# albertgassol1/vf-nerf

Hardware: AMD Instinct MI355X
Metric: rays/sec (4096-ray chunk, 128 samples/ray) + PSNR vs ref (higher is better)
Workload: dtype f16x3+f32acc

## Files before the change

### vf_nerf_amd/csrc/vfn_common.h

```cpp
#pragma once
#include <hip/hip_runtime.h>
#include <stdarg.h>
#include <stdio.h>
#include "../../include/vfn.h"

void vfn_set_error(const char* fmt, ...);

#define VFN_REQUIRE(cond, ...)                 \
    do {                                       \
        if (!(cond)) {                         \
            vfn_set_error(__VA_ARGS__);        \
            return VFN_ERR_INVALID;            \
        }                                      \
    } while (0)

static inline int vfn_check_launch(const char* what) {
    hipError_t e = hipGetLastError();
    if (e != hipSuccess) {
        vfn_set_error("%s: HIP launch failed: %s", what, hipGetErrorString(e));
        return VFN_ERR_LAUNCH;
    }
    return VFN_OK;
}

__device__ __forceinline__ double vfn_pair_sqdist(double qx, double qy, double qz, double tx, double ty, double tz) {
    const double dx = qx - tx, dy = qy - ty, dz = qz - tz;
    return (dx * dx + dy * dy) + dz * dz;
}

int vfn_internal_raygen(const vfn_raygen_params* p, const float* uv, const float* pose, const float* intrinsics, const float* k_sign,
                        const float* t_vals, const float* far_per_ray, const float* u_coarse, int gen_u, long long u_base, uint64_t seed,
                        uint64_t offset, float* directions, float* ray_dirs, float* cam_loc, float* z_vals, float* points, void* stream);
int vfn_internal_density_fine(const vfn_density_params* dp, const float* normals_c, const float* ray_dirs, const float* z_c,
                              const float* density_scalars, const vfn_fine_params* fp, const float* directions, const float* cam_loc,
                              const float* far_per_ray, const float* u_fine, const float* u_add, int gen_fine, int gen_add,
                              long long fine_base, long long add_base, uint64_t seed, uint64_t offset, float* z_vals, float* points,
                              int32_t* src, float* new_points, int32_t* dst, int64_t new_row0, void* stream);
int vfn_internal_composite_gather(const vfn_density_params* dp, float* normals, const float* ray_dirs, const float* z_vals,
                                  const float* density_scalars, float* colors, const int32_t* src, const float* normals_c,
                                  const float* colors_c, int64_t n_stored_c, float* weights, float* rgb, float* depth, void* stream);

int vfn_internal_weight_grad_frag_batch(int32_t shape, int32_t dy_form, int32_t x_form, int32_t n, const void* const* dy, const void* const* x,
                                        float* const* dw_part, float* const* db_part, int64_t n_points, int32_t groups, void* stream);
int vfn_internal_weight_grad_frag_batch_dev(int32_t shape, int32_t dy_form, int32_t x_form, int32_t n, const void* const* dy, const void* const* x,
                                            float* const* dw_part, float* const* db_part, int64_t n_points, const int32_t* n_dev, int32_t groups,
                                            void* stream);

int vfn_internal_fused16_fwd_train_at(const vfn_net_geom* vf_geom, const void* vf_packed16, const vfn_net_geom* rn_geom,
                                      const void* rn_packed16, const float* points, const float* ray_dirs, int64_t n_points,
                                      const int32_t* n_dev, int32_t samples_per_ray, float* normals, float* colors, float* saved,
                                      float* save_aux_vf, float* save_aux_rn, uint32_t* save_masks, int32_t save_f16, int64_t ws_first,
                                      int64_t ws_points, int32_t colour_products, void* stream);
int vfn_internal_bwd_chain_bf16_ws_at(const vfn_net_geom* vf_geom, const void* vf_packed_bwd16, const float* vf_head_w,
                                      const vfn_net_geom* rn_geom, const void* rn_packed_bwd16, const float* rn_head_w,
                                      const float* feats, const uint32_t* masks, void* dy, int32_t dy_flags, const float* d_colors,
                                      const float* colors, const float* d_vec, const float* vec, const float* d_feats,
                                      int32_t vec_stride, int64_t n_points, const int32_t* n_dev, float* dz_rgb, float* dz_vec,
                                      int64_t ws_first, int64_t ws_points, void* stream);
int vfn_internal_net_weight_grads_frag_part(int32_t net_kind, const vfn_net_geom* geom, const vfn_wgrad_layer* layers, const void* saved,
                                            const void* dy, int64_t slot_bytes, int32_t dy_form, int32_t x_form, const float* feats,
                                            const float* aux, const float* dz_head, int64_t n_points, const int32_t* n_dev, uint32_t parts,
                                            int32_t accumulate, void* scratch, void* stream, int32_t stages = 3);

int vfn_internal_select_positive(const float* weights, const float* sigma, const float* z_vals, int n_rays, int n_samples, const float* points,
                                 const float* ray_dirs, int32_t* cnt, int32_t* off, int32_t* k_dev, int32_t* sel_sorted, float* pts_sel,
                                 float* dirs_sel, void* stream);
int vfn_internal_rows3_by_index(const float* a, const int32_t* index, const int32_t* k_dev, int64_t capacity, float* out, int gather, void* stream);
int vfn_internal_fused16_products_dev(const vfn_net_geom* vf_geom, const void* vf_packed16, const vfn_net_geom* rn_geom, const void* rn_packed16,
                                      const float* points, const float* ray_dirs, int64_t n_points, const int32_t* n_dev, int32_t samples_per_ray,
                                      const int32_t* out_index, int32_t colour_products, float* normals, float* colors, void* stream);
uint32_t* vfn_internal_f16x3_status();
struct VfnReportScope {
    VfnReportScope(uint32_t* status_word, uint64_t* clock_stamps, int64_t clock_slots);
    ~VfnReportScope();
    VfnReportScope(const VfnReportScope&) = delete;
    VfnReportScope& operator=(const VfnReportScope&) = delete;
    uint32_t* old_status; unsigned long long* old_clock; long long old_slots;
};
```

### vf_nerf_amd/csrc/vfn_mlp16.hip

```cpp
#include <string.h>
#include <utility>
#include "vfn_common.h"
#include "vfn_plan.h"

typedef _Float16 half8 __attribute__((ext_vector_type(8)));
typedef _Float16 half2v __attribute__((ext_vector_type(2)));
typedef float float2v __attribute__((ext_vector_type(2)));
typedef float f32x16 __attribute__((ext_vector_type(16)));
typedef float f32x4v __attribute__((ext_vector_type(4)));

constexpr float VFN16_WSCALE = 64.0f;
constexpr float VFN16_INV_WSCALE = 0.015625f;
constexpr float VFN16_XSCALE = 64.0f;
constexpr int VFN16_SAVE_AUX = 2;
constexpr int VFN16_HANDOVER_NUM = 8;
constexpr int VFN16_DMA_STEPS = 16;
constexpr int VFN16_EPI_PER_MFMA = 6;
constexpr int VFN16_EPI_PER_MFMA2 = 9;
#define VFN16_MAX_CHUNK_KB 39
#define VFN16_STATS_WORDS 64

struct Plan16 {
    int32_t n_hidden;
    int32_t feat_layer;
    int32_t multires;
    uint32_t total_kb;
    uint32_t head_off_kb;
    uint32_t off_kb[VFN_MAX_LAYERS];
    uint8_t act16[VFN_MAX_LAYERS];
    uint8_t aux16[VFN_MAX_LAYERS];
    uint8_t n_tiles[VFN_MAX_LAYERS];
};

static int make_plan16(int kind, const vfn_net_geom* g, VfnNetPlan* p32, Plan16* p, const char* what) {
    char err[256] = {0};
    int rc = vfn_make_plan(kind, g, p32, err, sizeof(err));
    if (rc != VFN_OK) { vfn_set_error("%s: %s", what, err); return rc; }
    memset(p, 0, sizeof(*p));
    p->n_hidden = p32->n_hidden; p->feat_layer = p32->feat_layer; p->multires = p32->multires;
    uint32_t off = 0;
    for (int h = 0; h < p32->n_hidden; ++h) {
        const VfnLayerPlan& lp = p32->hidden[h];
        if (lp.nkb_act % 2) { vfn_set_error("%s: act width not a multiple of 16", what); return VFN_ERR_UNSUPPORTED; }
        p->act16[h] = (uint8_t)(lp.nkb_act / 2);
        p->aux16[h] = lp.nkb_aux ? 3 : 0;
        p->n_tiles[h] = (uint8_t)lp.n_tiles;
        p->off_kb[h] = off;
        off += lp.n_tiles * (2u * (p->act16[h] + p->aux16[h]) + 1u);
    }
    p->head_off_kb = off;
    off += 2u * 16u + 1u;
    p->total_kb = off;
    return VFN_OK;
}

struct Pack16Entry {
    const float* w; const float* b; const float* bn_w; const float* bn_b; const float* bn_mean; const float* bn_var;
    uint32_t off_kb, n_chunks, act16, aux16;
    int32_t in_dim, row_off, n_rows, act_col_off, act_valid, aux_col_off, aux_valid;
    float scale;
};
struct Pack16Args {
    Pack16Entry e[VFN_MAX_LAYERS + 2];
    int32_t n_entries;
    uint32_t total_words;
    uint32_t* out;
    uint32_t* stats;
};

__device__ __forceinline__ float folded_weight(const Pack16Entry& e, int n, int col) {
    if (n >= e.n_rows || col < 0) return 0.f;
    const int row = e.row_off + n;
    float w = e.w[(size_t)row * e.in_dim + col];
    if (e.bn_w) w *= e.bn_w[row] / sqrtf(e.bn_var[row] + 1e-5f);
    return w * e.scale;
}

#define VFN16_STAT_WGS 32
__device__ __forceinline__ void pack16_entry_stats(const Pack16Args& a, int ei, int share) {
    __shared__ float s_max[4];
    const Pack16Entry& e = a.e[ei];
    const int ncol = e.act_valid + e.aux_valid;
    float m = 0.f;
    for (int n = share; n < e.n_rows; n += VFN16_STAT_WGS)
        for (int c = (int)threadIdx.x; c < ncol; c += (int)blockDim.x)
            m = fmaxf(m, fabsf(folded_weight(e, n, c < e.act_valid ? e.act_col_off + c : e.aux_col_off + (c - e.act_valid))));
#pragma unroll
    for (int o = 32; o > 0; o >>= 1) m = fmaxf(m, __shfl_xor(m, o, 64));
    if ((threadIdx.x & 63) == 0) s_max[threadIdx.x >> 6] = m;
    __syncthreads();
    if (threadIdx.x == 0) {
        const float wm = fmaxf(fmaxf(s_max[0], s_max[1]), fmaxf(s_max[2], s_max[3]));
        if (wm > 0.f) atomicMax(a.stats + ei, __builtin_bit_cast(uint32_t, wm));
    }
}

__global__ __launch_bounds__(256) void vfn_pack16_kernel(Pack16Args a) {
    if (blockIdx.x * blockDim.x >= a.total_words) {
        const int sidx = (int)(blockIdx.x - a.total_words / blockDim.x);
        if (a.stats) pack16_entry_stats(a, sidx / VFN16_STAT_WGS, sidx % VFN16_STAT_WGS);
        return;
    }
    const uint32_t idx = blockIdx.x * blockDim.x + threadIdx.x;
    int ei = 0;
    for (int i = 1; i < a.n_entries; ++i)
        if (idx >= a.e[i].off_kb * 256u) ei = i;
    const Pack16Entry& e = a.e[ei];
    const uint32_t nkb = e.act16 + e.aux16;
    const uint32_t wblocks = nkb * 2u;
    const uint32_t chunk_words = (wblocks + 1u) * 256u;
    const uint32_t local = idx - e.off_kb * 256u;
    const uint32_t ck = local / chunk_words, cw = local % chunk_words;
    uint32_t word = 0;
    if (cw < wblocks * 256u) {
        const uint32_t blk = cw >> 8, lane = (cw >> 2) & 63u, jp = cw & 3u;
        const uint32_t part = blk & 1u, kb = blk >> 1;
        const int g = (int)(lane >> 5);
        const int n = (int)(32u * ck + (lane & 31u));
        _Float16 halves[2];
        for (int q = 0; q < 2; ++q) {
            const int j = (int)(2u * jp) + q;
            int col = -1;
            if (kb < e.act16) {
                const int k = 16 * (int)kb + 8 * (j >> 2) + 4 * g + (j & 3);
                if (k < e.act_valid) col = e.act_col_off + k;
            } else {
                const int k = 16 * (int)(kb - e.act16) + 8 * g + j;
                if (k < e.aux_valid) col = e.aux_col_off + k;
            }
            const float w = folded_weight(e, n, col);
            const _Float16 hi = (_Float16)w;
            halves[q] = part ? (_Float16)(w - (float)hi) : hi;
        }
        word = (uint32_t)__builtin_bit_cast(unsigned short, halves[0]) |
               ((uint32_t)__builtin_bit_cast(unsigned short, halves[1]) << 16);
    } else {
        const uint32_t bi = cw - wblocks * 256u;
        if (bi < 32u) {
            const int hl = (int)(bi >> 4), r = (int)(bi & 15u);
            const int n = (int)(32u * ck) + (r & 3) + 8 * (r >> 2) + 4 * hl;
            float b = 0.f;
            if (n < e.n_rows) {
                const int row = e.row_off + n;
                b = e.b[row];
                if (e.bn_w) b = (b - e.bn_mean[row]) * (e.bn_w[row] / sqrtf(e.bn_var[row] + 1e-5f)) + e.bn_b[row];
            }
            word = __builtin_bit_cast(uint32_t, b * VFN16_WSCALE);
        }
    }
    a.out[idx] = word;
}

static int check_kind16(int net_kind, const Plan16& p, const char* what);

extern "C" int64_t vfn_pack16_size(int32_t net_kind, const vfn_net_geom* geom) {
    VfnNetPlan p32; Plan16 p;
    int rc = make_plan16(net_kind, geom, &p32, &p, "vfn_pack16_size");
    if (rc != VFN_OK) return rc;
    rc = check_kind16(net_kind, p, "vfn_pack16_size");
    if (rc != VFN_OK) return rc;
    return (int64_t)p.total_kb * 1024 + VFN16_STATS_WORDS * 4;
}

extern "C" int vfn_pack16_weights(int32_t net_kind, const vfn_net_geom* geom, const vfn_layer_params* layers,
                                   void* packed16, void* stream) {
    VfnNetPlan p32; Plan16 p;
    int rc = make_plan16(net_kind, geom, &p32, &p, "vfn_pack16_weights");
    if (rc != VFN_OK) return rc;
    rc = check_kind16(net_kind, p, "vfn_pack16_weights");
    if (rc != VFN_OK) return rc;
    VFN_REQUIRE(layers && packed16, "vfn_pack16_weights: NULL argument");
    Pack16Args a;
    memset(&a, 0, sizeof(a));
    const int L = geom->n_layers, pe_dim = p32.pe_dim, F = geom->feature_dims;
    auto fill = [&](Pack16Entry& e, int i) -> int {
        const vfn_layer_params& q = layers[i];
        VFN_REQUIRE(q.weight && q.bias, "vfn_pack16_weights: layer %d has NULL weight/bias", i);
        e.w = q.weight; e.b = q.bias;
        if (geom->has_bn[i]) {
            VFN_REQUIRE(q.bn_weight && q.bn_bias && q.bn_mean && q.bn_var, "vfn_pack16_weights: layer %d BatchNorm pointer NULL", i);
            e.bn_w = q.bn_weight; e.bn_b = q.bn_bias; e.bn_mean = q.bn_mean; e.bn_var = q.bn_var;
        }
        e.in_dim = geom->in_dims[i]; e.scale = 1.0f;
        return VFN_OK;
    };
    for (int h = 0; h < p.n_hidden; ++h) {
        const int i = p32.hidden[h].ref_layer;
        Pack16Entry& e = a.e[a.n_entries++];
        rc = fill(e, i);
        if (rc != VFN_OK) return rc;
        e.off_kb = p.off_kb[h]; e.n_chunks = p.n_tiles[h]; e.act16 = p.act16[h]; e.aux16 = p.aux16[h];
        const bool feat = p.feat_layer && h == p.n_hidden - 1;
        e.row_off = feat ? 3 : 0;
        e.n_rows = feat ? F : geom->out_dims[i];
        if (net_kind == VFN_NET_VF) {
            if (i == 0) { e.act_valid = 0; e.aux_col_off = 0; e.aux_valid = pe_dim; }
            else if (i == geom->skip_layer) {
                e.act_col_off = 0; e.act_valid = geom->out_dims[i - 1];
                e.aux_col_off = geom->out_dims[i - 1]; e.aux_valid = pe_dim;
                e.scale = 0.70710678118654752440f;
            } else { e.act_col_off = 0; e.act_valid = VFN_HIDDEN; }
        } else {
            if (i == 0) { e.act_col_off = 6 + pe_dim; e.act_valid = F; e.aux_col_off = 0; e.aux_valid = 6 + pe_dim; }
            else { e.act_col_off = 0; e.act_valid = VFN_HIDDEN; }
        }
    }
    {
        Pack16Entry& e = a.e[a.n_entries++];
        rc = fill(e, L - 1);
        if (rc != VFN_OK) return rc;
        e.off_kb = p.head_off_kb; e.n_chunks = 1; e.act16 = 16; e.aux16 = 0;
        e.row_off = 0; e.n_rows = 3; e.act_col_off = 0; e.act_valid = VFN_HIDDEN;
    }
    a.total_words = p.total_kb * 256u;
    a.out = (uint32_t*)packed16;
    a.stats = a.out + a.total_words;
    if (hipMemsetAsync(a.stats, 0, VFN16_STATS_WORDS * 4, (hipStream_t)stream) != hipSuccess) {
        vfn_set_error("vfn_pack16_weights: hipMemsetAsync failed");
        return VFN_ERR_LAUNCH;
    }
    hipLaunchKernelGGL(vfn_pack16_kernel, dim3(a.total_words / 256 + VFN16_STAT_WGS * a.n_entries), dim3(256), 0, (hipStream_t)stream, a);
    return vfn_check_launch("vfn_pack16_weights");
}

namespace {

enum : int { EPI_RELU = 0, EPI_TANH = 1, EPI_HEAD_TANH = 2, EPI_HEAD_SIGMOID = 3 };
enum : int { M16_FEAT = 1, M16_RENDER = 2, M16_TRAIN = 4, M16_BLKOUT = 8, M16_BLKIN = 16, M16_C2 = 32, M16_P1 = 64, M16_SF16 = 128,
             M16_VF_VEC = 0, M16_FUSED = M16_FEAT | M16_RENDER, M16_VF_BLK = M16_FEAT | M16_BLKOUT, M16_RN_BLK = M16_RENDER | M16_BLKIN,
             M16_VF_VEC_TRAIN = M16_TRAIN, M16_VF_FULL_TRAIN = M16_FEAT | M16_TRAIN, M16_FUSED_TRAIN = M16_FUSED | M16_TRAIN };

constexpr int VFN16_FDEPTH = 2;
#define VFN16_SLOT (VFN16_MAX_CHUNK_KB * 64)
#define VFN16_WAVES 4
#define VFN16_PTS 128

typedef __attribute__((address_space(3))) void lds_void;

constexpr int VF_ACT[9] = {0, 16, 16, 16, 14, 16, 16, 16, 16};
constexpr int VF_AUX[9] = {3, 0, 0, 0, 3, 0, 0, 0, 0};
constexpr int VF_TILES[9] = {8, 8, 8, 7, 8, 8, 8, 8, 8};
constexpr int RN_ACT[4] = {16, 16, 16, 16};
constexpr int RN_AUX[4] = {3, 0, 0, 0};
constexpr int RN_TILES[4] = {8, 8, 8, 8};
constexpr int HEAD_KB = 2 * 16 + 1;
constexpr int chunk_kb(int act, int aux) { return 2 * (act + aux) + 1; }
constexpr int vf_off_kb(int h) { int o = 0; for (int i = 0; i < h; ++i) o += VF_TILES[i] * chunk_kb(VF_ACT[i], VF_AUX[i]); return o; }
constexpr int rn_off_kb(int h) { int o = 0; for (int i = 0; i < h; ++i) o += RN_TILES[i] * chunk_kb(RN_ACT[i], RN_AUX[i]); return o; }

struct ChunkD { int net, off_kb, kb, aux; };
constexpr ChunkD chunk_of(int mode, int c) {
    if (!(mode & M16_BLKIN)) {
        const int vf_layers = (mode & M16_FEAT) ? 9 : 8;
        for (int h = 0; h < vf_layers; ++h) {
            if (c < VF_TILES[h]) return {0, vf_off_kb(h) + c * chunk_kb(VF_ACT[h], VF_AUX[h]), chunk_kb(VF_ACT[h], VF_AUX[h]), VF_AUX[h]};
            c -= VF_TILES[h];
        }
        if (c == 0) return {0, vf_off_kb(9), HEAD_KB, 0};
        c -= 1;
    }
    if (mode & M16_RENDER) {
        for (int h = 0; h < 4; ++h) {
            if (c < RN_TILES[h]) return {1, rn_off_kb(h) + c * chunk_kb(RN_ACT[h], RN_AUX[h]), chunk_kb(RN_ACT[h], RN_AUX[h]), RN_AUX[h]};
            c -= RN_TILES[h];
        }
        if (c == 0) return {1, rn_off_kb(4), HEAD_KB, 0};
    }
    return {0, 0, 0, 0};
}

constexpr int rn_first_chunk(int mode) { return (mode & M16_BLKIN) ? 0 : 72; }
constexpr bool chunk_two(int mode, int c) { return (mode & M16_C2) && !(mode & M16_BLKIN) && c >= 63 && c != 71; }
constexpr bool mode_one(int mode) { return (mode & M16_P1) != 0; }
constexpr int VFN16_P1_RING = 5;
#define VFN16_P1_SLOT_KB 20
constexpr int ring_of(int mode) { return mode_one(mode) ? VFN16_P1_RING : 3; }
constexpr int slot_u4(int mode) { return mode_one(mode) ? VFN16_P1_SLOT_KB * 64 : VFN16_MAX_CHUNK_KB * 64; }
constexpr int slot_base(int mode, int c) { return (c % ring_of(mode)) * slot_u4(mode); }
static_assert(VFN16_P1_RING * VFN16_P1_SLOT_KB <= 3 * VFN16_MAX_CHUNK_KB, "the single-product ring must fit into the split modes' ring");
constexpr int stores_of(int mode, int c) { return (c == 0 || ((mode & M16_RENDER) && c == rn_first_chunk(mode))) ? 0 : 4; }
constexpr int young_ops(int mode, int c) {
    const int ring = ring_of(mode);
    int n = 0;
    for (int k = (c - ring + 2 > 0 ? c - ring + 2 : 0); k < c; ++k) n += stores_of(mode, k);
    for (int j = 2; j <= ring - 2; ++j)
        if (c + j >= ring - 1 && chunk_of(mode, c + j).kb > 0) n += (((chunk_of(mode, c + j).kb - 1) / 2 + 1) / VFN16_WAVES);
    return n;
}

struct Mlp16Args {
    const uint4* vf_w;
    const uint4* rn_w;
    const float* points;
    const float* ray_dirs;
    float* out_vec;
    float* out_colors;
    long long n_points;
    int dirs_div;
    int vf_multires, rn_multires;
    uint32_t vf_bytes, rn_bytes;
    float* saved;
    float* save_aux_vf;
    float* save_aux_rn;
    uint32_t* save_masks;
    int save_f16;
    uint4* blk_out;
    const uint4* blk_in;
    const float* vec_in;
    const int* src;
    const int* out_index;
    long long ws_first, ws_points;
    uint32_t* status;
    const int* n_dev;
    unsigned long long* clock;
    long long clock_slots;
};

#define VFN16_CLAMP 60000.0f
constexpr int VFN16_CLAMP_BITS = 0x476a6000;
static_assert(__builtin_bit_cast(int, VFN16_CLAMP) == VFN16_CLAMP_BITS, "VFN16_CLAMP_BITS is VFN16_CLAMP as an integer");

struct X16 { half8 hi[16]; half8 lo[16]; };
struct A16 { half8 hi[3]; half8 lo[3]; };

struct Pipe16 {
    uint4* lds;
    __amdgpu_buffer_rsrc_t vf_w;
    __amdgpu_buffer_rsrc_t rn_w;
    float* saved;
    long long slot_floats;
    uint32_t slot_bytes;
    uint32_t save_voff;
    uint32_t save_voff16;
    uint32_t feat_voff;
    uint32_t st_tile, st_q;
    int save16;
    uint32_t* masks;
    uint32_t mask_bytes;
    uint32_t mask_voff;
    uint4* blk_out;
    uint32_t blk_bytes, blk_voff;
};

struct Carry16 {
    f32x16 pend;
    f32x16 bias;
    half8 fh0, fl0;
    uint32_t lm[4];
    unsigned long long sat;
};

template <int N, typename F, int... I>
__device__ __forceinline__ void static_for_impl(F&& f, std::integer_sequence<int, I...>) { (f(std::integral_constant<int, I>{}), ...); }
template <int N, typename F>
__device__ __forceinline__ void static_for(F&& f) { static_for_impl<N>(f, std::make_integer_sequence<int, N>{}); }

__device__ __forceinline__ void split2(float a, float b, _Float16& h0, _Float16& h1, _Float16& l0, _Float16& l1) {
    const float2v v = {a, b};
    const half2v hi = __builtin_convertvector(v, half2v);
    h0 = hi[0]; h1 = hi[1];
    const uint32_t hp = __builtin_bit_cast(uint32_t, hi);
    float r0, r1;
    asm("v_fma_mix_f32 %0, %1, -1.0, %2 op_sel_hi:[1,0,0]" : "=v"(r0) : "v"(hp), "v"(a));
    asm("v_fma_mix_f32 %0, %1, -1.0, %2 op_sel:[1,0,0] op_sel_hi:[1,0,0]" : "=v"(r1) : "v"(hp), "v"(b));
    const float2v r = {r0, r1};
    const half2v lo = __builtin_convertvector(r, half2v);
    l0 = lo[0]; l1 = lo[1];
}

__device__ __forceinline__ float tanh_exp(float v) { return 1.0f - 2.0f / (1.0f + expf(2.0f * v)); }

template <int NET, int OFF_KB, int LDS_U4>
__device__ __forceinline__ void dma_piece(const Pipe16& p, int blk, int lane, int dst_blk = -1) {
    __builtin_amdgcn_raw_ptr_buffer_load_lds(NET ? p.rn_w : p.vf_w, (lds_void*)(p.lds + LDS_U4 + (dst_blk < 0 ? blk : dst_blk) * 64), 16,
                                             lane * 16, (OFF_KB + blk) * 1024, 0, 0);
}
template <int MODE, int C>
__device__ __forceinline__ void dma_chunk(const Pipe16& p, int wave, int lane) {
    constexpr ChunkD d = chunk_of(MODE, C);
    if constexpr (mode_one(MODE)) {
        constexpr int NKB = (d.kb - 1) / 2;
#pragma unroll
        for (int i = 0; i * VFN16_WAVES < NKB + 1; ++i)
            if (wave + VFN16_WAVES * i < NKB + 1) dma_piece<d.net, d.off_kb, slot_base(MODE, C)>(p, 2 * (wave + VFN16_WAVES * i), lane, wave + VFN16_WAVES * i);
    } else {
#pragma unroll
    for (int i = 0; i * VFN16_WAVES < d.kb; ++i)
        if (wave + VFN16_WAVES * i < d.kb) dma_piece<d.net, d.off_kb, slot_base(MODE, C)>(p, wave + VFN16_WAVES * i, lane);
    }
}

template <int MODE, int C>
__device__ __forceinline__ void prefetch_chunk(Carry16& cy, const Pipe16& p, int lane) {
    constexpr ChunkD d = chunk_of(MODE, C);
    const uint4* cb = p.lds + slot_base(MODE, C);
    const f32x4v* bb = reinterpret_cast<const f32x4v*>(cb + (mode_one(MODE) ? (d.kb - 1) / 2 : d.kb - 1) * 64) + (lane >> 5) * 4;
    const f32x4v b0 = bb[0], b1 = bb[1], b2 = bb[2], b3 = bb[3];
#pragma unroll
    for (int q = 0; q < 4; ++q) { cy.bias[q] = b0[q]; cy.bias[4 + q] = b1[q]; cy.bias[8 + q] = b2[q]; cy.bias[12 + q] = b3[q]; }
    cy.fh0 = __builtin_bit_cast(half8, cb[0 * 64 + lane]);
    if (!chunk_two(MODE, C) && !mode_one(MODE)) cy.fl0 = __builtin_bit_cast(half8, cb[1 * 64 + lane]);
}

template <int EPI, bool KEEP, bool LO = true>
__device__ __forceinline__ void epi_pair(f32x16& pend, int& gmax, int pr, half8& hi, half8& lo, int j) {
    float v0 = pend[2 * pr], v1 = pend[2 * pr + 1];
    if (EPI != EPI_RELU) { v0 *= VFN16_INV_WSCALE; v1 *= VFN16_INV_WSCALE; }
    if (EPI == EPI_RELU) {
        const int b0 = __builtin_bit_cast(int, v0), b1 = __builtin_bit_cast(int, v1);
        gmax = pr == 0 ? max(b0, b1) : max(max(gmax, b0), b1);
        v0 = __builtin_amdgcn_fmed3f(v0, 0.f, VFN16_CLAMP); v1 = __builtin_amdgcn_fmed3f(v1, 0.f, VFN16_CLAMP);
    }
    else { v0 = tanh_exp(v0) * VFN16_XSCALE; v1 = tanh_exp(v1) * VFN16_XSCALE; }
    if constexpr (LO) {
        _Float16 h0, h1, l0, l1;
        split2(v0, v1, h0, h1, l0, l1);
        hi[j] = h0; hi[j + 1] = h1; lo[j] = l0; lo[j + 1] = l1;
    } else {
        const float2v v = {v0, v1};
        const half2v h = __builtin_convertvector(v, half2v);
        hi[j] = h[0]; hi[j + 1] = h[1];
    }
    if (KEEP) { pend[2 * pr] = v0 * (1.0f / VFN16_XSCALE); pend[2 * pr + 1] = v1 * (1.0f / VFN16_XSCALE); }
}

template <int SLOT, int TILE, bool SF16 = false>
__device__ __forceinline__ void save_group(const Pipe16& p, const f32x16& v, int q) {
    typedef unsigned int u32x4 __attribute__((ext_vector_type(4)));
    const __amdgpu_buffer_rsrc_t rs = __builtin_amdgcn_make_buffer_rsrc(p.saved + (long long)SLOT * p.slot_floats, 0,
                                                                        (int)p.slot_bytes, 0x00020000);
    const f32x4v g = {v[4 * q], v[4 * q + 1], v[4 * q + 2], v[4 * q + 3]};
    if constexpr (SF16 && SLOT != 8) {
        typedef _Float16 half4 __attribute__((ext_vector_type(4)));
        typedef unsigned int u32x2 __attribute__((ext_vector_type(2)));
        const half4 h = __builtin_convertvector(g, half4);
        __builtin_amdgcn_raw_buffer_store_b64(__builtin_bit_cast(u32x2, h), rs, (int)p.save_voff16, (TILE * 4096 + q * 1024) / 2, VFN16_SAVE_AUX);
        return;
    }
    if (SLOT == 8) {
        __builtin_amdgcn_raw_buffer_store_b128(__builtin_bit_cast(u32x4, g), rs, (int)p.feat_voff, (32 * TILE + 8 * q) * 4, 0);
    } else if (p.save16) {
        typedef _Float16 half4 __attribute__((ext_vector_type(4)));
        typedef unsigned int u32x2 __attribute__((ext_vector_type(2)));
        const half4 h = __builtin_convertvector(g, half4);
        if (p.st_q == 1024u) __builtin_amdgcn_raw_buffer_store_b64(__builtin_bit_cast(u32x2, h), rs, (int)p.save_voff16, (int)((TILE * p.st_tile + q * p.st_q) >> 1), VFN16_SAVE_AUX);
        else __builtin_amdgcn_raw_buffer_store_b64(__builtin_bit_cast(u32x2, h), rs, (int)p.save_voff16, (int)((TILE * p.st_tile + q * p.st_q) >> 1), 0);
    } else {
        if (p.st_q == 1024u) __builtin_amdgcn_raw_buffer_store_b128(__builtin_bit_cast(u32x4, g), rs, (int)p.save_voff, (int)(TILE * p.st_tile + q * p.st_q), VFN16_SAVE_AUX);
        else __builtin_amdgcn_raw_buffer_store_b128(__builtin_bit_cast(u32x4, g), rs, (int)p.save_voff, (int)(TILE * p.st_tile + q * p.st_q), 0);
    }
}

template <int TILE, int EPI>
__device__ __forceinline__ void collect_mask(Carry16& cy) {
    if constexpr (EPI == EPI_RELU) {
        typedef unsigned int u32x16 __attribute__((ext_vector_type(16)));
        const u32x16 u = __builtin_bit_cast(u32x16, cy.pend);
        unsigned b = 0;
#pragma unroll
        for (int r = 15; r >= 0; --r) b = __builtin_amdgcn_alignbit(b, u[r] + 0x7fffffffu, 31);
        cy.lm[TILE >> 1] |= b << (16 * (TILE & 1));
    }
}
template <int TILE, int EPI, int PART, int PARTS>
__device__ __forceinline__ void collect_mask_part(Carry16& cy, unsigned& b) {
    if constexpr (EPI == EPI_RELU) {
        typedef unsigned int u32x16 __attribute__((ext_vector_type(16)));
        const u32x16 u = __builtin_bit_cast(u32x16, cy.pend);
        constexpr int N = 16 / PARTS;
        if constexpr (PART == 0) b = 0;
#pragma unroll
        for (int r = 15 - PART * N; r > 15 - (PART + 1) * N; --r) b = __builtin_amdgcn_alignbit(b, u[r] + 0x7fffffffu, 31);
        if constexpr (PART == PARTS - 1) cy.lm[TILE >> 1] |= b << (16 * (TILE & 1));
    }
}
template <int SLOT>
__device__ __forceinline__ void store_mask(const Pipe16& p, Carry16& cy) {
    typedef unsigned int u32x4 __attribute__((ext_vector_type(4)));
    const __amdgpu_buffer_rsrc_t rs = __builtin_amdgcn_make_buffer_rsrc(
        reinterpret_cast<unsigned char*>(p.masks) + (size_t)SLOT * p.mask_bytes, 0, (int)p.mask_bytes, 0x00020000);
    const u32x4 w = {cy.lm[0], cy.lm[1], cy.lm[2], cy.lm[3]};
    __builtin_amdgcn_raw_buffer_store_b128(w, rs, (int)p.mask_voff, 0, 0);
    cy.lm[0] = 0; cy.lm[1] = 0; cy.lm[2] = 0; cy.lm[3] = 0;
}

template <int TILE>
__device__ __forceinline__ void store_blocks(const Pipe16& p, const X16& x) {
    typedef unsigned int u32x4 __attribute__((ext_vector_type(4)));
    const __amdgpu_buffer_rsrc_t rs = __builtin_amdgcn_make_buffer_rsrc(p.blk_out, 0, (int)p.blk_bytes, 0x00020000);
#pragma unroll
    for (int s = 0; s < 2; ++s) {
        __builtin_amdgcn_raw_buffer_store_b128(__builtin_bit_cast(u32x4, x.hi[2 * TILE + s]), rs, (int)p.blk_voff, (2 * TILE + s) * 2048, 0);
        __builtin_amdgcn_raw_buffer_store_b128(__builtin_bit_cast(u32x4, x.lo[2 * TILE + s]), rs, (int)p.blk_voff, (2 * TILE + s) * 2048 + 1024, 0);
    }
}

template <int MODE, int C0, int ACT, int AUX, int NCH, int EPI, int PEPI, int PKB, int SLOT = -1, int PSLOT = -1, bool BLK = false,
          bool PBLK = false>
__device__ __forceinline__ void layer16(const X16& xin, const A16& aux, X16& xout, X16& xpend, Carry16& cy, float (&head)[3],
                                       const Pipe16& p, int wave, int lane) {
    constexpr int NKB = ACT + AUX;
    constexpr int E = NKB / 2 > 0 ? NKB / 2 : 1;
    constexpr int H = NKB * VFN16_HANDOVER_NUM / 16 > 0 ? NKB * VFN16_HANDOVER_NUM / 16 : 1;
    constexpr int PMAX = (VFN16_MAX_CHUNK_KB + VFN16_WAVES - 1) / VFN16_WAVES;
    constexpr int DSPAN = NKB - H > 0 ? NKB - H : 1;
    constexpr int DSTEPS = DSPAN < VFN16_DMA_STEPS ? DSPAN : VFN16_DMA_STEPS;
    static_assert(PEPI < 0 || PKB >= E, "the pending tile must be complete before it is read");
    constexpr bool TRAIN = (MODE & M16_TRAIN) != 0;
    constexpr int DEND = NKB - 4 > H + 1 ? NKB - 4 : (H + 1 < NKB ? H + 1 : NKB - 1);
    constexpr int SSTEPS = NKB - DEND > 0 ? NKB - DEND : 1;
    constexpr int DST = TRAIN ? (DEND - H > 0 ? DEND - H : 1) : DSTEPS;
    constexpr int MPARTS = (TRAIN && E <= H) ? (DEND - H >= 4 ? 4 : (DEND - H >= 2 ? 2 : (DEND - H >= 1 ? 1 : 0))) : 0;
    static_for<NCH>([&](auto ich) {
        constexpr int ch = decltype(ich)::value;
        constexpr int C = C0 + ch;
        constexpr int RING = ring_of(MODE);
        constexpr ChunkD dcur = chunk_of(MODE, C), dnext = chunk_of(MODE, C + 1), ddma = chunk_of(MODE, C + RING - 1);
        static_assert(dcur.kb == 2 * NKB + 1, "layer shape and chunk table disagree");
        constexpr bool P1 = mode_one(MODE);
        constexpr bool W2 = chunk_two(MODE, C);
        constexpr bool D2 = chunk_two(MODE, C + RING - 1) || P1;
        constexpr int DNKB = (ddma.kb - 1) / 2;
        constexpr int DPIECES = P1 ? DNKB + 1 : (D2 ? DNKB + ddma.aux + 1 : ddma.kb);
        auto piece_blk = [&](int idx) -> int {
            if (P1) return idx < DNKB ? 2 * idx : 2 * DNKB;
            if (!D2) return idx;
            if (ddma.aux == 0) return 2 * idx;
            return idx < DNKB ? 2 * idx : (idx < DNKB + ddma.aux ? 2 * (idx - ddma.aux) + 1 : 2 * DNKB);
        };
        constexpr int PM = D2 ? (DPIECES + VFN16_WAVES - 1) / VFN16_WAVES : PMAX;
        const uint4* cb = p.lds + slot_base(MODE, C);
        constexpr int FB = P1 ? 1 : 2;
        f32x16 acc = cy.bias;
        half8 fh[VFN16_FDEPTH], fl[VFN16_FDEPTH];
        fh[0] = cy.fh0;
        if (!P1 && (!W2 || ACT == 0)) fl[0] = cy.fl0;
        half8 ehi[2], elo[2];
        [[maybe_unused]] int gmax = 0;
        [[maybe_unused]] unsigned mbits = 0;
#pragma unroll
        for (int st = 0; st < NKB; ++st) {
            constexpr int AHEAD = VFN16_FDEPTH - 1;
            if (st + AHEAD < NKB) {
                fh[(st + AHEAD) % VFN16_FDEPTH] = __builtin_bit_cast(half8, cb[(FB * (st + AHEAD)) * 64 + lane]);
                if (!P1 && (!W2 || st + AHEAD >= ACT)) fl[(st + AHEAD) % VFN16_FDEPTH] = __builtin_bit_cast(half8, cb[(2 * (st + AHEAD) + 1) * 64 + lane]);
            }
            const half8 a_hi = fh[st % VFN16_FDEPTH];
            const half8 x_hi = st < ACT ? xin.hi[st < ACT ? st : 0] : aux.hi[st >= ACT ? st - ACT : 0];
            const half8 x_lo = st < ACT ? xin.lo[st < ACT ? st : 0] : aux.lo[st >= ACT ? st - ACT : 0];
            acc = __builtin_amdgcn_mfma_f32_32x32x16_f16(a_hi, x_hi, acc, 0, 0, 0);
            if constexpr (!P1) {
                acc = __builtin_amdgcn_mfma_f32_32x32x16_f16(a_hi, x_lo, acc, 0, 0, 0);
                if (!W2 || st >= ACT) acc = __builtin_amdgcn_mfma_f32_32x32x16_f16(fl[st % VFN16_FDEPTH], x_hi, acc, 0, 0, 0);
            }
            if (st < E && (ch > 0 || PEPI >= 0)) {
#pragma unroll
                for (int pr = st * 8 / E; pr < (st + 1) * 8 / E; ++pr) {
                    const int sblk = pr >> 2, j = (pr & 3) * 2;
                    if (ch > 0) epi_pair<EPI, TRAIN, !P1>(cy.pend, gmax, pr, ehi[sblk], elo[sblk], j);
                    else epi_pair<(PEPI >= 0 ? PEPI : 0), TRAIN, !P1>(cy.pend, gmax, pr, ehi[sblk], elo[sblk], j);
                    if (pr == 7 && (ch > 0 ? EPI : PEPI) == EPI_RELU) cy.sat |= __builtin_amdgcn_ballot_w64(gmax >= VFN16_CLAMP_BITS);
                    if ((pr & 3) == 3) {
                        asm volatile("" : "+a"(ehi[sblk]));
                        if constexpr (!P1) asm volatile("" : "+a"(elo[sblk]));
                        if (ch > 0) { xout.hi[2 * (ch > 0 ? ch - 1 : 0) + sblk] = ehi[sblk]; if constexpr (!P1) xout.lo[2 * (ch > 0 ? ch - 1 : 0) + sblk] = elo[sblk]; }
                        else { xpend.hi[PKB + sblk] = ehi[sblk]; if constexpr (!P1) xpend.lo[PKB + sblk] = elo[sblk]; }
                    }
                }
                if constexpr (!P1) {
                __builtin_amdgcn_sched_group_barrier(0x100, W2 ? 1 : 2, 0);
                __builtin_amdgcn_sched_group_barrier(0x008, 1, 0);
                __builtin_amdgcn_sched_group_barrier(0x002, W2 ? VFN16_EPI_PER_MFMA2 : VFN16_EPI_PER_MFMA, 0);
                __builtin_amdgcn_sched_group_barrier(0x008, 1, 0);
                __builtin_amdgcn_sched_group_barrier(0x002, W2 ? VFN16_EPI_PER_MFMA2 : VFN16_EPI_PER_MFMA, 0);
                if (!W2) {
                    __builtin_amdgcn_sched_group_barrier(0x008, 1, 0);
                    __builtin_amdgcn_sched_group_barrier(0x002, VFN16_EPI_PER_MFMA, 0);
                }
                }
            }
            if (st == H - 1 && dnext.kb > 0) {
                if constexpr (P1 && TRAIN) {
                    constexpr int young = young_ops(MODE, C);
                    static_assert(young < 64, "vmcnt is a 6-bit field");
                    if constexpr (young == 0) asm volatile("s_waitcnt vmcnt(0)" ::: "memory");
                    else asm volatile("s_waitcnt vmcnt(%0)" :: "n"(young) : "memory");
                } else
                if (TRAIN && C > 0 && (ch == 0 || ch > 1 || PEPI >= 0)) asm volatile("s_waitcnt vmcnt(4)" ::: "memory");
                else asm volatile("s_waitcnt vmcnt(0)" ::: "memory");
                __builtin_amdgcn_s_barrier();
            }
            if (st >= H && st < H + DST && ddma.kb > 0) {
#pragma unroll
                for (int i = (st - H) * PM / DST; i < (st - H + 1) * PM / DST; ++i) {
                    if (VFN16_WAVES * i + VFN16_WAVES <= DPIECES) dma_piece<ddma.net, ddma.off_kb, slot_base(MODE, C + RING - 1)>(p, piece_blk(wave + VFN16_WAVES * i), lane, P1 ? wave + VFN16_WAVES * i : -1);
                    else if (VFN16_WAVES * i < DPIECES) {
                        const int idx = min(wave + VFN16_WAVES * i, DPIECES - 1);
                        dma_piece<ddma.net, ddma.off_kb, slot_base(MODE, C + RING - 1)>(p, piece_blk(idx), lane, P1 ? idx : -1);
                    }
                }
            }
            if (TRAIN && MPARTS > 0 && st >= H && st < H + MPARTS && (ch > 0 || PEPI >= 0)) {
                static_for<MPARTS>([&](auto ip) {
                    constexpr int part = decltype(ip)::value;
                    if (st - H == part) {
                        if (ch > 0) collect_mask_part<(ch > 0 ? ch - 1 : 0), EPI, part, (MPARTS > 0 ? MPARTS : 1)>(cy, mbits);
                        else collect_mask_part<PKB / 2, (PEPI >= 0 ? PEPI : 0), part, (MPARTS > 0 ? MPARTS : 1)>(cy, mbits);
                    }
                });
            }
            if (TRAIN && st >= DEND && st < DEND + SSTEPS && (ch > 0 || PEPI >= 0)) {
                if (st == DEND) {
                    if constexpr (MPARTS > 0) {
                        if (ch == 0) store_mask<(PSLOT >= 0 ? PSLOT : 0)>(p, cy);
                    } else {
                        if (ch > 0) collect_mask<(ch > 0 ? ch - 1 : 0), EPI>(cy);
                        else { collect_mask<PKB / 2, (PEPI >= 0 ? PEPI : 0)>(cy); store_mask<(PSLOT >= 0 ? PSLOT : 0)>(p, cy); }
                    }
                }
#pragma unroll
                for (int q = (st - DEND) * 4 / SSTEPS; q < (st - DEND + 1) * 4 / SSTEPS; ++q) {
                    if (ch > 0) save_group<(SLOT >= 0 ? SLOT : 0), (ch > 0 ? ch - 1 : 0), (MODE & M16_SF16) != 0>(p, cy.pend, q);
                    else save_group<(PSLOT >= 0 ? PSLOT : 0), PKB / 2, (MODE & M16_SF16) != 0>(p, cy.pend, q);
                }
            }
            if (st == H && ((BLK && ch > 0) || (PBLK && ch == 0))) {
                if (ch > 0) store_blocks<(ch > 0 ? ch - 1 : 0)>(p, xout);
                else store_blocks<PKB / 2>(p, xpend);
            }
            if (st == NKB - 1 && dnext.kb > 0) prefetch_chunk<MODE, (dnext.kb > 0 ? C + 1 : C)>(cy, p, lane);
            __builtin_amdgcn_sched_barrier(0);
        }
        if (EPI == EPI_RELU || EPI == EPI_TANH) {
            cy.pend = acc;
        } else {
#pragma unroll
            for (int c = 0; c < 3; ++c) {
                const float v = acc[c] * VFN16_INV_WSCALE;
                head[c] = (EPI == EPI_HEAD_TANH) ? tanh_exp(v) : 1.0f / (1.0f + expf(-v));
            }
        }
    });
}

__device__ __forceinline__ float enc_value(const float (&x)[3], const float (&sn)[18], const float (&cs)[18], int multires, int k) {
    if (k < 3) return x[k];
    const int idx = k - 3, oct = idx / 6, rem = idx - 6 * oct;
    if (oct >= multires) return 0.f;
    return rem < 3 ? sn[3 * oct + rem] : cs[3 * oct + rem - 3];
}

template <typename F>
__device__ __forceinline__ void build_aux(A16& aux, int g, F col, float& ain) {
#pragma unroll
    for (int s = 0; s < 3; ++s) {
        half8 hi, lo;
#pragma unroll
        for (int j = 0; j < 8; j += 2) {
            float v0, v1;
            if (g == 0) { v0 = col(16 * s + j); v1 = col(16 * s + j + 1); }
            else { v0 = col(16 * s + 8 + j); v1 = col(16 * s + 8 + j + 1); }
            v0 *= VFN16_XSCALE; v1 *= VFN16_XSCALE;
            v0 = fminf(fmaxf(v0, -VFN16_CLAMP), VFN16_CLAMP); v1 = fminf(fmaxf(v1, -VFN16_CLAMP), VFN16_CLAMP);
            ain = fmaxf(ain, fmaxf(fabsf(v0), fabsf(v1)));
            _Float16 h0, h1, l0, l1;
            split2(v0, v1, h0, h1, l0, l1);
            hi[j] = h0; hi[j + 1] = h1; lo[j] = l0; lo[j + 1] = l1;
        }
        aux.hi[s] = hi; aux.lo[s] = lo;
    }
}

template <typename F>
__device__ __forceinline__ void save_aux(float* dst, long long m, int g, F col) {
#pragma unroll
    for (int s = 0; s < 3; ++s)
#pragma unroll
        for (int h = 0; h < 2; ++h) {
            const int c0 = 16 * s + 8 * g + 4 * h;
            if (c0 + 4 <= VFN_AUX_K) {
                f32x4v v;
                if (g == 0) { v = f32x4v{col(16 * s + 4 * h), col(16 * s + 4 * h + 1), col(16 * s + 4 * h + 2), col(16 * s + 4 * h + 3)}; }
                else { v = f32x4v{col(16 * s + 8 + 4 * h), col(16 * s + 8 + 4 * h + 1), col(16 * s + 8 + 4 * h + 2), col(16 * s + 8 + 4 * h + 3)}; }
                *reinterpret_cast<f32x4v*>(dst + m * VFN_AUX_K + c0) = v;
            }
        }
}

__device__ __forceinline__ void load_aux(A16& ax, const float* park) {
    const half8* pk = reinterpret_cast<const half8*>(park + 8);
#pragma unroll
    for (int q = 0; q < 3; ++q) { ax.hi[q] = pk[2 * q]; ax.lo[q] = pk[2 * q + 1]; }
}

__device__ __forceinline__ void encode_sincos(const float (&x)[3], int multires, int g, float (&sn)[18], float (&cs)[18]) {
#pragma unroll
    for (int j = 0; j < 3; ++j)
#pragma unroll
        for (int c = 0; c < 3; ++c) {
            float s = 0.f, k = 0.f;
            if (2 * j < multires) {
                sincosf(x[c] * (g ? (float)(2 << (2 * j)) : (float)(1 << (2 * j))), &s, &k);
                if (2 * j + g >= multires) { s = 0.f; k = 0.f; }
            }
            const float so = __shfl_xor(s, 32, 64), ko = __shfl_xor(k, 32, 64);
            sn[6 * j + c] = g ? so : s;          cs[6 * j + c] = g ? ko : k;
            sn[6 * j + 3 + c] = g ? s : so;      cs[6 * j + 3 + c] = g ? k : ko;
        }
}

template <int MODE>
__device__ __forceinline__ void render_aux(const Mlp16Args& a, A16& aux, const float (&xr)[3], const float (&dr)[3], const float (&nrm)[3],
                                           long long m, bool in, int g, float& ain) {
    const int rn_multires = a.rn_multires;
    float sn[18], cs[18];
    encode_sincos(dr, rn_multires, g, sn, cs);
    const int ncol = 6 + 6 * rn_multires;
    auto rn_col = [&](int k) -> float {
        if (k < 3) return xr[k];
        if (k >= ncol) return k < ncol + 3 ? nrm[k - ncol] : 0.f;
        return enc_value(dr, sn, cs, rn_multires, k - 3);
    };
    build_aux(aux, g, rn_col, ain);
    if ((MODE & M16_TRAIN) && in) save_aux(a.save_aux_rn, m, g, rn_col);
}

template <int MODE>
__device__ __forceinline__ void render_tail(const Mlp16Args& a, const Pipe16& p, Carry16& cy, X16& xa, X16& xb, const A16& aux,
                                            const float (&nrm)[3], long long m, bool in, int wave, int lane) {
    constexpr int R = EPI_RELU, NONE = -1;
    constexpr int C0 = rn_first_chunk(MODE);
    float rgb[3] = {0.f, 0.f, 0.f};
    layer16<MODE, C0 + 0, 16, 3, 8, R, NONE, 0, 9, -1>(xb, aux, xa, xb, cy, rgb, p, wave, lane);
    layer16<MODE, C0 + 8, 16, 0, 8, R, R, 14, 10, 9>(xa, aux, xb, xa, cy, rgb, p, wave, lane);
    layer16<MODE, C0 + 16, 16, 0, 8, R, R, 14, 11, 10>(xb, aux, xa, xb, cy, rgb, p, wave, lane);
    layer16<MODE, C0 + 24, 16, 0, 8, R, R, 14, 12, 11>(xa, aux, xb, xa, cy, rgb, p, wave, lane);
    layer16<MODE, C0 + 32, 16, 0, 1, EPI_HEAD_SIGMOID, R, 14, -1, 12>(xb, aux, xa, xb, cy, rgb, p, wave, lane);
    const long long mo = m;
    if (in && (threadIdx.x & 32) == 0) {
        a.out_vec[mo * 3 + 0] = nrm[0]; a.out_vec[mo * 3 + 1] = nrm[1]; a.out_vec[mo * 3 + 2] = nrm[2];
        a.out_colors[mo * 3 + 0] = rgb[0]; a.out_colors[mo * 3 + 1] = rgb[1]; a.out_colors[mo * 3 + 2] = rgb[2];
    }
}

__device__ __forceinline__ void report_range(const Mlp16Args& a, unsigned long long sat, float ain) {
    if (a.status) {
        const unsigned bits = (sat != 0ull ? 1u : 0u) | (ain >= VFN16_CLAMP ? 2u : 0u);
        if (bits) atomicOr(a.status, bits);
    }
}

template <int MODE>
__global__ __launch_bounds__(256, 1) void vfn_mlp16_kernel(const Mlp16Args a) {
    __shared__ __attribute__((aligned(16))) uint4 s_ring[3 * VFN16_SLOT + 256 * 8];
    float* s_park = reinterpret_cast<float*>(s_ring + 3 * VFN16_SLOT) + threadIdx.x * 32;
    const int tid = threadIdx.x;
    const int lane = tid & 63;
    const int wave = __builtin_amdgcn_readfirstlane(tid >> 6);
    const int g = lane >> 5;
    unsigned long long ck_t0 = 0ull, ck_r0 = 0ull;
    if constexpr ((MODE & M16_RENDER) != 0 && (MODE & M16_BLKIN) == 0 && (MODE & M16_TRAIN) == 0) {
        if (a.clock) { ck_t0 = __builtin_amdgcn_s_memtime(); ck_r0 = __builtin_amdgcn_s_memrealtime(); }
    }
    const long long m = (long long)blockIdx.x * VFN16_PTS + wave * 32 + (lane & 31);
    long long n_live = a.n_points;
    if (a.n_dev) {
        const long long nd = (long long)*a.n_dev;
        n_live = nd < n_live ? nd : n_live;
        if ((long long)blockIdx.x * VFN16_PTS >= n_live) return;
    }
    const bool in = m < n_live;

    if constexpr ((MODE & M16_BLKIN) != 0) {
        const int dpos = in ? a.src[m] : -1;
        const bool live = dpos >= 0;
        float xr[3] = {0.f, 0.f, 0.f}, dr[3] = {0.f, 0.f, 0.f}, nrm[3] = {0.f, 0.f, 0.f};
        if (live) {
            const long long di = dpos / a.dirs_div;
#pragma unroll
            for (int c = 0; c < 3; ++c) { xr[c] = a.points[(long long)dpos * 3 + c]; dr[c] = a.ray_dirs[di * 3 + c]; nrm[c] = a.vec_in[m * 3 + c]; }
        }
        Pipe16 p;
        p.lds = s_ring;
        p.vf_w = __builtin_amdgcn_make_buffer_rsrc(const_cast<uint4*>(a.rn_w), 0, (int)a.rn_bytes, 0x00020000);
        p.rn_w = p.vf_w;
        p.saved = nullptr; p.slot_floats = 0; p.slot_bytes = 0; p.save_voff = 0; p.blk_out = nullptr; p.blk_bytes = 0; p.blk_voff = 0;
        p.masks = nullptr; p.mask_bytes = 0; p.mask_voff = 0; p.save16 = 0; p.save_voff16 = 0; p.feat_voff = 0; p.st_tile = 0; p.st_q = 0;
        dma_chunk<MODE, 0>(p, wave, lane);
        dma_chunk<MODE, 1>(p, wave, lane);
        X16 xa, xb;
        A16 aux;
        float ain_blk = 0.f;
        {
            typedef unsigned int u32x4 __attribute__((ext_vector_type(4)));
            const __amdgpu_buffer_rsrc_t rs_blk = __builtin_amdgcn_make_buffer_rsrc(
                const_cast<uint4*>(a.blk_in), 0, (int)(((a.n_points + 31) & ~31ll) * 1024), 0x00020000);
            const unsigned goff = in ? (unsigned)((m >> 5) * 32768 + lane * 16) : 0xfffffff0u;
            u32x4 q[32];
#pragma unroll
            for (int i = 0; i < 32; ++i) q[i] = __builtin_amdgcn_raw_buffer_load_b128(rs_blk, goff, i * 1024, 0);
            render_aux<MODE>(a, aux, xr, dr, nrm, -1, false, g, ain_blk);
#pragma unroll
            for (int t = 0; t < 8; ++t) {
                half8 h0 = __builtin_bit_cast(half8, q[4 * t + 0]), l0 = __builtin_bit_cast(half8, q[4 * t + 1]);
                half8 h1 = __builtin_bit_cast(half8, q[4 * t + 2]), l1 = __builtin_bit_cast(half8, q[4 * t + 3]);
                asm volatile("" : "+a"(h0)); asm volatile("" : "+a"(l0)); asm volatile("" : "+a"(h1)); asm volatile("" : "+a"(l1));
                xb.hi[2 * t] = h0; xb.lo[2 * t] = l0; xb.hi[2 * t + 1] = h1; xb.lo[2 * t + 1] = l1;
            }
        }
        asm volatile("s_waitcnt vmcnt(0)" ::: "memory");
        __builtin_amdgcn_s_barrier();
        Carry16 cy;
#pragma unroll
        for (int q = 0; q < 16; ++q) cy.pend[q] = 0.f;
        cy.lm[0] = 0; cy.lm[1] = 0; cy.lm[2] = 0; cy.lm[3] = 0; cy.sat = 0ull;
        prefetch_chunk<MODE, 0>(cy, p, lane);
        render_tail<MODE>(a, p, cy, xa, xb, aux, nrm, live ? (long long)dpos : -1, live, wave, lane);
        report_range(a, cy.sat, ain_blk);
    } else {
    float x[3] = {0.f, 0.f, 0.f};
    if (in) { x[0] = a.points[m * 3 + 0]; x[1] = a.points[m * 3 + 1]; x[2] = a.points[m * 3 + 2]; }
    float d[3] = {0.f, 0.f, 0.f};
    int out_row = -1;
    if ((MODE & M16_RENDER) && in) {
        const long long di = m / a.dirs_div;
        d[0] = a.ray_dirs[di * 3 + 0]; d[1] = a.ray_dirs[di * 3 + 1]; d[2] = a.ray_dirs[di * 3 + 2];
        if (a.out_index) out_row = a.out_index[m];
    }
    asm volatile("s_waitcnt vmcnt(0)" ::: "memory");
    if (MODE & M16_RENDER) {
        s_park[0] = x[0]; s_park[1] = x[1]; s_park[2] = x[2];
        s_park[4] = d[0]; s_park[5] = d[1]; s_park[6] = d[2];
    }

    Pipe16 p;
    p.lds = s_ring;
    p.vf_w = __builtin_amdgcn_make_buffer_rsrc(const_cast<uint4*>(a.vf_w), 0, (int)a.vf_bytes, 0x00020000);
    p.rn_w = __builtin_amdgcn_make_buffer_rsrc(const_cast<uint4*>((MODE & M16_RENDER) ? a.rn_w : a.vf_w), 0,
                                               (int)((MODE & M16_RENDER) ? a.rn_bytes : a.vf_bytes), 0x00020000);
    const bool frag = (a.save_f16 & 2) != 0;
    const long long mw = m + a.ws_first;
    p.slot_floats = frag ? ((a.ws_points + 31) >> 5) * 8192 : a.ws_points * 256;
    p.saved = a.saved + a.ws_first * 256;
    {
        const long long left = p.slot_floats * 4 - a.ws_first * 1024;
        p.slot_bytes = (uint32_t)(left < 0x7fffffffll ? left : 0x7fffffffll);
    }
    p.save_voff = !in ? (frag ? 0xc0000000u : 0xfffffff0u) : (frag ? (uint32_t)((m >> 5) * 32768 + lane * 16) : (uint32_t)(m * 1024 + g * 16));
    p.save_voff16 = !in ? (frag ? 0xc0000000u : 0xfffffff0u) : (frag ? (uint32_t)((m >> 5) * 32768 + lane * 8) : (uint32_t)(m * 1024 + g * 8));
    p.feat_voff = in ? (uint32_t)(m * 1024 + g * 16) : 0xfffffff0u;
    p.st_tile = frag ? 4096u : 128u; p.st_q = frag ? 1024u : 32u;
    p.masks = a.save_masks; p.mask_bytes = (uint32_t)(a.ws_points * 32); p.mask_voff = in ? (uint32_t)((2 * mw + g) * 16) : 0xfffffff0u;
    p.save16 = a.save_f16 & 1;
    p.blk_out = a.blk_out; p.blk_bytes = (uint32_t)(((a.n_points + 31) & ~31ll) * 1024);
    p.blk_voff = (uint32_t)((m >> 5) * 32768 + lane * 16);
    dma_chunk<MODE, 0>(p, wave, lane);
    dma_chunk<MODE, 1>(p, wave, lane);
    if constexpr (mode_one(MODE)) static_for<VFN16_P1_RING - 3>([&](auto ic) { dma_chunk<MODE, 2 + decltype(ic)::value>(p, wave, lane); });

    const int vf_multires = a.vf_multires;
    A16 aux;
    float ain = 0.f;
    {
        float sn[18], cs[18];
        encode_sincos(x, vf_multires, g, sn, cs);
        build_aux(aux, g, [&](int k) { return enc_value(x, sn, cs, vf_multires, k); }, ain);
        if ((MODE & M16_TRAIN) && in) save_aux(a.save_aux_vf, mw, g, [&](int k) { return enc_value(x, sn, cs, vf_multires, k); });
        half8* pk = reinterpret_cast<half8*>(s_park + 8);
#pragma unroll
        for (int q = 0; q < 3; ++q) { pk[2 * q] = aux.hi[q]; pk[2 * q + 1] = aux.lo[q]; }
    }
    asm volatile("s_waitcnt vmcnt(0)" ::: "memory");
    __builtin_amdgcn_s_barrier();
    Carry16 cy;
#pragma unroll
    for (int q = 0; q < 16; ++q) cy.pend[q] = 0.f;
    cy.lm[0] = 0; cy.lm[1] = 0; cy.lm[2] = 0; cy.lm[3] = 0; cy.sat = 0ull;
    prefetch_chunk<MODE, 0>(cy, p, lane);

    X16 xa, xb;
    float vec[3] = {0.f, 0.f, 0.f};
    constexpr int R = EPI_RELU, T = EPI_TANH, NONE = -1;
    layer16<MODE, 0, 0, 3, 8, R, NONE, 0, 0, -1>(xa, aux, xb, xb, cy, vec, p, wave, lane);
    layer16<MODE, 8, 16, 0, 8, R, R, 14, 1, 0>(xb, aux, xa, xb, cy, vec, p, wave, lane);
    layer16<MODE, 16, 16, 0, 8, R, R, 14, 2, 1>(xa, aux, xb, xa, cy, vec, p, wave, lane);
    layer16<MODE, 24, 16, 0, 7, R, R, 14, 3, 2>(xb, aux, xa, xb, cy, vec, p, wave, lane);
    { A16 ax; load_aux(ax, s_park); layer16<MODE, 31, 14, 3, 8, R, R, 12, 4, 3>(xa, ax, xb, xa, cy, vec, p, wave, lane); }
    layer16<MODE, 39, 16, 0, 8, R, R, 14, 5, 4>(xb, aux, xa, xb, cy, vec, p, wave, lane);
    layer16<MODE, 47, 16, 0, 8, R, R, 14, 6, 5>(xa, aux, xb, xa, cy, vec, p, wave, lane);
    layer16<MODE, 55, 16, 0, 8, R, R, 14, 7, 6>(xb, aux, xa, xb, cy, vec, p, wave, lane);
    if constexpr (!(MODE & M16_FEAT)) {
        layer16<MODE, 63, 16, 0, 1, EPI_HEAD_TANH, R, 14, -1, 7>(xa, aux, xb, xa, cy, vec, p, wave, lane);
        if (in && g == 0) { a.out_vec[m * 3 + 0] = vec[0]; a.out_vec[m * 3 + 1] = vec[1]; a.out_vec[m * 3 + 2] = vec[2]; }
        report_range(a, cy.sat, ain);
    } else {
    constexpr bool BO = (MODE & M16_BLKOUT) != 0;
    layer16<MODE, 63, 16, 0, 8, T, R, 14, 8, 7, BO, false>(xa, aux, xb, xa, cy, vec, p, wave, lane);
    layer16<MODE, 71, 16, 0, 1, EPI_HEAD_TANH, T, 14, -1, 8, false, BO>(xa, aux, xb, xb, cy, vec, p, wave, lane);
    if constexpr (!(MODE & M16_RENDER)) {
        if (in && g == 0) { a.out_vec[m * 3 + 0] = vec[0]; a.out_vec[m * 3 + 1] = vec[1]; a.out_vec[m * 3 + 2] = vec[2]; }
        report_range(a, cy.sat, ain);
    } else {
    float nrm[3];
#pragma unroll
    for (int c = 0; c < 3; ++c) nrm[c] = __shfl(vec[c], lane & 31, 64);
    const float xr[3] = {s_park[0], s_park[1], s_park[2]};
    const float dr[3] = {s_park[4], s_park[5], s_park[6]};
    A16 raux;
    render_aux<MODE>(a, raux, xr, dr, nrm, (MODE & M16_TRAIN) ? mw : m, in, g, ain);
    render_tail<MODE>(a, p, cy, xa, xb, raux, nrm, a.out_index ? (long long)out_row : m, a.out_index ? out_row >= 0 : in, wave, lane);
    report_range(a, cy.sat, ain);
    if constexpr ((MODE & M16_TRAIN) == 0) {
        if (a.clock && threadIdx.x == 0 && (long long)blockIdx.x < a.clock_slots) {
            const unsigned long long t1 = __builtin_amdgcn_s_memtime(), r1 = __builtin_amdgcn_s_memrealtime();
            a.clock[2 * blockIdx.x] = t1 - ck_t0; a.clock[2 * blockIdx.x + 1] = r1 - ck_r0;
        }
    }
    }
    }
    }
}

int check_vf16(const Plan16& vf, const char* what) {
    bool ok = vf.feat_layer == 1 && vf.n_hidden == 9 && (int)vf.head_off_kb == vf_off_kb(9);
    for (int h = 0; ok && h < 9; ++h)
        ok = vf.act16[h] == VF_ACT[h] && vf.aux16[h] == VF_AUX[h] && vf.n_tiles[h] == VF_TILES[h] && (int)vf.off_kb[h] == vf_off_kb(h);
    if (!ok) { vfn_set_error("%s: the f16x3 kernels are specialised for the shipped vector-field network shape", what); return VFN_ERR_UNSUPPORTED; }
    return VFN_OK;
}
int check_rn16(const Plan16& rn, const char* what) {
    bool ok = rn.n_hidden == 4 && (int)rn.head_off_kb == rn_off_kb(4);
    for (int h = 0; ok && h < 4; ++h)
        ok = rn.act16[h] == RN_ACT[h] && rn.aux16[h] == RN_AUX[h] && rn.n_tiles[h] == RN_TILES[h] && (int)rn.off_kb[h] == rn_off_kb(h);
    if (!ok) { vfn_set_error("%s: the f16x3 kernels are specialised for the shipped rendering network shape", what); return VFN_ERR_UNSUPPORTED; }
    return VFN_OK;
}

}

static int check_kind16(int net_kind, const Plan16& p, const char* what) {
    return net_kind == VFN_NET_VF ? check_vf16(p, what) : check_rn16(p, what);
}

static thread_local uint32_t* t_status_word = nullptr;

uint32_t* vfn_internal_f16x3_status() { return t_status_word; }

extern "C" int vfn_f16x3_set_status(uint32_t* status_word) {
    t_status_word = status_word;
    return VFN_OK;
}

static thread_local unsigned long long* t_clock_probe = nullptr;
static thread_local long long t_clock_slots = 0;

extern "C" int vfn_f16x3_set_clock_probe(uint64_t* stamps, int64_t slots) {
    VFN_REQUIRE(slots >= 0 && (stamps || slots == 0), "vfn_f16x3_set_clock_probe: %lld slots without a buffer", (long long)slots);
    t_clock_probe = reinterpret_cast<unsigned long long*>(stamps);
    t_clock_slots = stamps ? slots : 0;
    return VFN_OK;
}

VfnReportScope::VfnReportScope(uint32_t* status_word, uint64_t* clock_stamps, int64_t clock_slots)
    : old_status(t_status_word), old_clock(t_clock_probe), old_slots(t_clock_slots) {
    if (status_word) t_status_word = status_word;
    if (clock_stamps && clock_slots > 0) { t_clock_probe = reinterpret_cast<unsigned long long*>(clock_stamps); t_clock_slots = clock_slots; }
}
VfnReportScope::~VfnReportScope() { t_status_word = old_status; t_clock_probe = old_clock; t_clock_slots = old_slots; }

extern "C" int vfn_vf_mlp16_fwd(const vfn_net_geom* geom, const void* packed16, const float* points, int64_t n_points,
                                 float* out_vec, void* stream) {
    Mlp16Args a = {};
    VfnNetPlan p32; Plan16 vf;
    int rc = make_plan16(VFN_NET_VF, geom, &p32, &vf, "vfn_vf_mlp16_fwd");
    if (rc != VFN_OK) return rc;
    rc = check_vf16(vf, "vfn_vf_mlp16_fwd");
    if (rc != VFN_OK) return rc;
    if (n_points <= 0) return VFN_OK;
    VFN_REQUIRE(packed16 && points && out_vec, "vfn_vf_mlp16_fwd: NULL argument");
    a.vf_w = (const uint4*)packed16; a.points = points; a.out_vec = out_vec; a.n_points = n_points; a.dirs_div = 1;
    a.vf_multires = vf.multires; a.vf_bytes = vf.total_kb * 1024u;
    a.status = t_status_word;
    a.clock = t_clock_probe; a.clock_slots = t_clock_slots;
    const long long blocks = (n_points + VFN16_PTS - 1) / VFN16_PTS;
    hipLaunchKernelGGL(vfn_mlp16_kernel<M16_VF_VEC>, dim3((unsigned)blocks), dim3(256), 0, (hipStream_t)stream, a);
    return vfn_check_launch("vfn_vf_mlp16_fwd");
}

static int launch_fused16(const char* what, const vfn_net_geom* vf_geom, const void* vf_packed16, const vfn_net_geom* rn_geom,
                          const void* rn_packed16, const float* points, const float* ray_dirs, int64_t n_points,
                          int32_t samples_per_ray, const int32_t* out_index, bool scatter, int32_t colour_products, float* normals,
                          float* colors, void* stream, const int32_t* n_dev = nullptr) {
    Mlp16Args a = {};
    a.n_dev = n_dev;
    VfnNetPlan p32; Plan16 vf, rn;
    VFN_REQUIRE(vf_geom && rn_geom, "%s: NULL argument", what);
    int rc = make_plan16(VFN_NET_VF, vf_geom, &p32, &vf, what);
    if (rc != VFN_OK) return rc;
    rc = make_plan16(VFN_NET_RENDER, rn_geom, &p32, &rn, what);
    if (rc != VFN_OK) return rc;
    rc = check_vf16(vf, what);
    if (rc != VFN_OK) return rc;
    rc = check_rn16(rn, what);
    if (rc != VFN_OK) return rc;
    VFN_REQUIRE(vf_geom->feature_dims == VFN_HIDDEN && rn_geom->feature_dims == VFN_HIDDEN, "%s: both nets need feature_dims == %d", what, VFN_HIDDEN);
    VFN_REQUIRE(colour_products == 2 || colour_products == 3, "%s: colour_products must be 2 or 3 (got %d)", what, colour_products);
    if (n_points <= 0) return VFN_OK;
    VFN_REQUIRE(vf_packed16 && rn_packed16 && points && ray_dirs && normals && colors && (out_index || !scatter), "%s: NULL argument", what);
    VFN_REQUIRE(samples_per_ray > 0, "%s: samples_per_ray must be > 0", what);
    a.vf_w = (const uint4*)vf_packed16; a.rn_w = (const uint4*)rn_packed16; a.points = points; a.ray_dirs = ray_dirs;
    a.out_vec = normals; a.out_colors = colors; a.out_index = out_index; a.n_points = n_points; a.dirs_div = samples_per_ray;
    a.vf_multires = vf.multires; a.rn_multires = rn.multires; a.vf_bytes = vf.total_kb * 1024u; a.rn_bytes = rn.total_kb * 1024u;
    a.status = t_status_word;
    a.clock = t_clock_probe; a.clock_slots = t_clock_slots;
    const long long blocks = (n_points + VFN16_PTS - 1) / VFN16_PTS;
    if (colour_products == 2) hipLaunchKernelGGL(vfn_mlp16_kernel<M16_FUSED | M16_C2>, dim3((unsigned)blocks), dim3(256), 0, (hipStream_t)stream, a);
    else hipLaunchKernelGGL(vfn_mlp16_kernel<M16_FUSED>, dim3((unsigned)blocks), dim3(256), 0, (hipStream_t)stream, a);
    return vfn_check_launch(what);
}

extern "C" int vfn_vf_render_fused16_fwd(const vfn_net_geom* vf_geom, const void* vf_packed16, const vfn_net_geom* rn_geom,
                                          const void* rn_packed16, const float* points, const float* ray_dirs,
                                          int64_t n_points, int32_t samples_per_ray, float* normals, float* colors,
                                          void* stream) {
    return launch_fused16("vfn_vf_render_fused16_fwd", vf_geom, vf_packed16, rn_geom, rn_packed16, points, ray_dirs, n_points, samples_per_ray,
                          nullptr, false, 3, normals, colors, stream);
}

extern "C" int vfn_vf_render_fused16_scatter(const vfn_net_geom* vf_geom, const void* vf_packed16, const vfn_net_geom* rn_geom,
                                          const void* rn_packed16, const float* points, const float* ray_dirs,
                                          int64_t n_points, int32_t samples_per_ray, const int32_t* out_index, float* normals,
                                          float* colors, void* stream) {
    return launch_fused16("vfn_vf_render_fused16_scatter", vf_geom, vf_packed16, rn_geom, rn_packed16, points, ray_dirs, n_points,
                          samples_per_ray, out_index, true, 3, normals, colors, stream);
}

extern "C" int vfn_vf_render_fused16_products(const vfn_net_geom* vf_geom, const void* vf_packed16, const vfn_net_geom* rn_geom,
                                              const void* rn_packed16, const float* points, const float* ray_dirs, int64_t n_points,
                                              int32_t samples_per_ray, const int32_t* out_index, int32_t colour_products,
                                              float* normals, float* colors, void* stream) {
    return launch_fused16("vfn_vf_render_fused16_products", vf_geom, vf_packed16, rn_geom, rn_packed16, points, ray_dirs, n_points,
                          samples_per_ray, out_index, false, colour_products, normals, colors, stream);
}

int vfn_internal_fused16_products_dev(const vfn_net_geom* vf_geom, const void* vf_packed16, const vfn_net_geom* rn_geom, const void* rn_packed16,
                                      const float* points, const float* ray_dirs, int64_t n_points, const int32_t* n_dev, int32_t samples_per_ray,
                                      const int32_t* out_index, int32_t colour_products, float* normals, float* colors, void* stream) {
    return launch_fused16("vfn_render_fwd (colour branch on the selected samples)", vf_geom, vf_packed16, rn_geom, rn_packed16, points, ray_dirs,
                          n_points, samples_per_ray, out_index, false, colour_products, normals, colors, stream, n_dev);
}

extern "C" int vfn_vf_feat16_fwd(const vfn_net_geom* geom, const void* packed16, const float* points, int64_t n_points,
                                 float* out_vec, void* out_blocks, void* stream) {
    Mlp16Args a = {};
    VfnNetPlan p32; Plan16 vf;
    int rc = make_plan16(VFN_NET_VF, geom, &p32, &vf, "vfn_vf_feat16_fwd");
    if (rc != VFN_OK) return rc;
    rc = check_vf16(vf, "vfn_vf_feat16_fwd");
    if (rc != VFN_OK) return rc;
    if (n_points <= 0) return VFN_OK;
    VFN_REQUIRE(packed16 && points && out_vec && out_blocks, "vfn_vf_feat16_fwd: NULL argument");
    VFN_REQUIRE(n_points < (1ll << 22), "vfn_vf_feat16_fwd: at most 4194303 points per launch (32-bit block offsets)");
    a.vf_w = (const uint4*)packed16; a.points = points; a.out_vec = out_vec; a.n_points = n_points; a.dirs_div = 1;
    a.vf_multires = vf.multires; a.vf_bytes = vf.total_kb * 1024u; a.blk_out = (uint4*)out_blocks;
    a.status = t_status_word;
    a.clock = t_clock_probe; a.clock_slots = t_clock_slots;
    const long long blocks = (n_points + VFN16_PTS - 1) / VFN16_PTS;
    hipLaunchKernelGGL(vfn_mlp16_kernel<M16_VF_BLK>, dim3((unsigned)blocks), dim3(256), 0, (hipStream_t)stream, a);
    return vfn_check_launch("vfn_vf_feat16_fwd");
}

extern "C" int vfn_render16_from_blocks(const vfn_net_geom* rn_geom, const void* rn_packed16, const void* blocks, const float* vecs,
                                        const int32_t* dst, const float* points, const float* ray_dirs, int64_t n_points,
                                        int32_t samples_per_ray, float* normals, float* colors, void* stream) {
    Mlp16Args a = {};
    VfnNetPlan p32; Plan16 rn;
    int rc = make_plan16(VFN_NET_RENDER, rn_geom, &p32, &rn, "vfn_render16_from_blocks");
    if (rc != VFN_OK) return rc;
    rc = check_rn16(rn, "vfn_render16_from_blocks");
    if (rc != VFN_OK) return rc;
    VFN_REQUIRE(rn_geom->feature_dims == VFN_HIDDEN, "vfn_render16_from_blocks: feature_dims must be %d", VFN_HIDDEN);
    if (n_points <= 0) return VFN_OK;
    VFN_REQUIRE(rn_packed16 && blocks && vecs && dst && points && ray_dirs && normals && colors, "vfn_render16_from_blocks: NULL argument");
    VFN_REQUIRE(samples_per_ray > 0, "vfn_render16_from_blocks: samples_per_ray must be > 0");
    a.rn_w = (const uint4*)rn_packed16; a.vf_w = a.rn_w; a.points = points; a.ray_dirs = ray_dirs; a.out_vec = normals; a.out_colors = colors;
    a.n_points = n_points; a.dirs_div = samples_per_ray; a.rn_multires = rn.multires; a.rn_bytes = rn.total_kb * 1024u; a.vf_bytes = a.rn_bytes;
    a.blk_in = (const uint4*)blocks; a.vec_in = vecs; a.src = dst;
    a.status = t_status_word;
    a.clock = t_clock_probe; a.clock_slots = t_clock_slots;
    const long long nblocks = (n_points + VFN16_PTS - 1) / VFN16_PTS;
    hipLaunchKernelGGL(vfn_mlp16_kernel<M16_RN_BLK>, dim3((unsigned)nblocks), dim3(256), 0, (hipStream_t)stream, a);
    return vfn_check_launch("vfn_render16_from_blocks");
}

extern "C" int vfn_vf_mlp16_fwd_train(const vfn_net_geom* geom, const void* packed16, const float* points, int64_t n_points,
                                      int32_t with_features, float* out_vec, float* saved, float* save_aux_vf, uint32_t* save_masks,
                                      int32_t save_f16, void* stream) {
    return vfn_vf_mlp16_fwd_train_at(geom, packed16, points, n_points, with_features, out_vec, saved, save_aux_vf, save_masks, save_f16, 0, n_points,
                                     stream);
}

extern "C" int vfn_vf_mlp16_fwd_train_at(const vfn_net_geom* geom, const void* packed16, const float* points, int64_t n_points,
                                         int32_t with_features, float* out_vec, float* saved, float* save_aux_vf, uint32_t* save_masks,
                                         int32_t save_f16, int64_t ws_first, int64_t ws_points, void* stream) {
    Mlp16Args a = {};
    VfnNetPlan p32; Plan16 vf;
    int rc = make_plan16(VFN_NET_VF, geom, &p32, &vf, "vfn_vf_mlp16_fwd_train");
    if (rc != VFN_OK) return rc;
    rc = check_vf16(vf, "vfn_vf_mlp16_fwd_train");
    if (rc != VFN_OK) return rc;
    if (n_points <= 0) return VFN_OK;
    VFN_REQUIRE(packed16 && points && out_vec && saved && save_aux_vf && save_masks, "vfn_vf_mlp16_fwd_train: NULL argument");
    VFN_REQUIRE(ws_first >= 0 && ws_first + n_points <= ws_points, "vfn_vf_mlp16_fwd_train: points %lld .. %lld outside a workspace of %lld",
                (long long)ws_first, (long long)(ws_first + n_points), (long long)ws_points);
    VFN_REQUIRE(!(save_f16 & 2) || ws_first % 32 == 0, "vfn_vf_mlp16_fwd_train: ws_first must be a multiple of 32 in fragment order");
    VFN_REQUIRE(n_points < (1ll << 21) && ws_points < (1ll << 26), "vfn_vf_mlp16_fwd_train: at most 2097151 points per launch (32-bit slot offsets) and 67108863 per "
                "workspace (got %lld in %lld)", (long long)n_points, (long long)ws_points);
    a.vf_w = (const uint4*)packed16; a.points = points; a.out_vec = out_vec; a.n_points = n_points; a.dirs_div = 1;
    a.vf_multires = vf.multires; a.vf_bytes = vf.total_kb * 1024u; a.saved = saved; a.save_aux_vf = save_aux_vf;
    a.save_masks = save_masks; a.save_f16 = save_f16 & 3;
    a.ws_first = ws_first; a.ws_points = ws_points;
    a.status = t_status_word;
    a.clock = t_clock_probe; a.clock_slots = t_clock_slots;
    const long long blocks = (n_points + VFN16_PTS - 1) / VFN16_PTS;
    if (save_f16 & 4) {
        VFN_REQUIRE(!with_features, "vfn_vf_mlp16_fwd_train: the single-product forward computes the vector columns only");
        hipLaunchKernelGGL(vfn_mlp16_kernel<M16_VF_VEC_TRAIN | M16_P1>, dim3((unsigned)blocks), dim3(256), 0, (hipStream_t)stream, a);
    }
    else if (with_features && (save_f16 & 3) == 3) hipLaunchKernelGGL(vfn_mlp16_kernel<M16_VF_FULL_TRAIN | M16_SF16>, dim3((unsigned)blocks), dim3(256), 0, (hipStream_t)stream, a);
    else if (with_features) hipLaunchKernelGGL(vfn_mlp16_kernel<M16_VF_FULL_TRAIN>, dim3((unsigned)blocks), dim3(256), 0, (hipStream_t)stream, a);
    else if ((save_f16 & 3) == 3) hipLaunchKernelGGL(vfn_mlp16_kernel<M16_VF_VEC_TRAIN | M16_SF16>, dim3((unsigned)blocks), dim3(256), 0, (hipStream_t)stream, a);
    else hipLaunchKernelGGL(vfn_mlp16_kernel<M16_VF_VEC_TRAIN>, dim3((unsigned)blocks), dim3(256), 0, (hipStream_t)stream, a);
    return vfn_check_launch("vfn_vf_mlp16_fwd_train");
}

extern "C" int vfn_vf_render_fused16_fwd_train(const vfn_net_geom* vf_geom, const void* vf_packed16, const vfn_net_geom* rn_geom,
                                               const void* rn_packed16, const float* points, const float* ray_dirs,
                                               int64_t n_points, int32_t samples_per_ray, float* normals, float* colors,
                                               float* saved, float* save_aux_vf, float* save_aux_rn, uint32_t* save_masks,
                                               int32_t save_f16, void* stream) {
    return vfn_vf_render_fused16_fwd_train_at(vf_geom, vf_packed16, rn_geom, rn_packed16, points, ray_dirs, n_points, samples_per_ray, normals, colors,
                                              saved, save_aux_vf, save_aux_rn, save_masks, save_f16, 0, n_points, 3, stream);
}

extern "C" int vfn_vf_render_fused16_fwd_train_at(const vfn_net_geom* vf_geom, const void* vf_packed16, const vfn_net_geom* rn_geom,
                                                  const void* rn_packed16, const float* points, const float* ray_dirs,
                                                  int64_t n_points, int32_t samples_per_ray, float* normals, float* colors,
                                                  float* saved, float* save_aux_vf, float* save_aux_rn, uint32_t* save_masks,
                                                  int32_t save_f16, int64_t ws_first, int64_t ws_points, int32_t colour_products,
                                                  void* stream) {
    return vfn_internal_fused16_fwd_train_at(vf_geom, vf_packed16, rn_geom, rn_packed16, points, ray_dirs, n_points, nullptr, samples_per_ray, normals,
                                             colors, saved, save_aux_vf, save_aux_rn, save_masks, save_f16, ws_first, ws_points, colour_products, stream);
}

int vfn_internal_fused16_fwd_train_at(const vfn_net_geom* vf_geom, const void* vf_packed16, const vfn_net_geom* rn_geom,
                                      const void* rn_packed16, const float* points, const float* ray_dirs, int64_t n_points,
                                      const int32_t* n_dev, int32_t samples_per_ray, float* normals, float* colors, float* saved,
                                      float* save_aux_vf, float* save_aux_rn, uint32_t* save_masks, int32_t save_f16, int64_t ws_first,
                                      int64_t ws_points, int32_t colour_products, void* stream) {
    Mlp16Args a = {};
    a.n_dev = n_dev;
    VfnNetPlan p32; Plan16 vf, rn;
    int rc = make_plan16(VFN_NET_VF, vf_geom, &p32, &vf, "vfn_vf_render_fused16_fwd_train");
    if (rc != VFN_OK) return rc;
    rc = make_plan16(VFN_NET_RENDER, rn_geom, &p32, &rn, "vfn_vf_render_fused16_fwd_train");
    if (rc != VFN_OK) return rc;
    rc = check_vf16(vf, "vfn_vf_render_fused16_fwd_train");
    if (rc != VFN_OK) return rc;
    rc = check_rn16(rn, "vfn_vf_render_fused16_fwd_train");
    if (rc != VFN_OK) return rc;
    if (n_points <= 0) return VFN_OK;
    VFN_REQUIRE(vf_packed16 && rn_packed16 && points && ray_dirs && normals && colors && saved && save_aux_vf && save_aux_rn && save_masks,
                "vfn_vf_render_fused16_fwd_train: NULL argument");
    VFN_REQUIRE(samples_per_ray > 0, "vfn_vf_render_fused16_fwd_train: samples_per_ray must be > 0");
    VFN_REQUIRE(ws_first >= 0 && ws_first + n_points <= ws_points, "vfn_vf_render_fused16_fwd_train: points %lld .. %lld outside a workspace of %lld",
                (long long)ws_first, (long long)(ws_first + n_points), (long long)ws_points);
    VFN_REQUIRE(!(save_f16 & 2) || ws_first % 32 == 0, "vfn_vf_render_fused16_fwd_train: ws_first must be a multiple of 32 in fragment order");
    VFN_REQUIRE(n_points < (1ll << 21) && ws_points < (1ll << 26), "vfn_vf_render_fused16_fwd_train: at most 2097151 points per launch (32-bit slot offsets) and 67108863 per "
                "workspace (got %lld in %lld)", (long long)n_points, (long long)ws_points);
    a.ws_first = ws_first; a.ws_points = ws_points;
    a.vf_w = (const uint4*)vf_packed16; a.rn_w = (const uint4*)rn_packed16; a.points = points; a.ray_dirs = ray_dirs;
    a.out_vec = normals; a.out_colors = colors; a.n_points = n_points; a.dirs_div = samples_per_ray;
    a.vf_multires = vf.multires; a.rn_multires = rn.multires; a.vf_bytes = vf.total_kb * 1024u; a.rn_bytes = rn.total_kb * 1024u;
    a.saved = saved; a.save_aux_vf = save_aux_vf; a.save_aux_rn = save_aux_rn; a.save_masks = save_masks; a.save_f16 = save_f16 & 3;
    a.status = t_status_word;
    a.clock = t_clock_probe; a.clock_slots = t_clock_slots;
    const long long blocks = (n_points + VFN16_PTS - 1) / VFN16_PTS;
    VFN_REQUIRE(colour_products >= 1 && colour_products <= 3, "vfn_vf_render_fused16_fwd_train: colour_products must be 1, 2 or 3 (got %d)", colour_products);
    if (colour_products == 1) hipLaunchKernelGGL(vfn_mlp16_kernel<M16_FUSED_TRAIN | M16_P1>, dim3((unsigned)blocks), dim3(256), 0, (hipStream_t)stream, a);
    else if (colour_products == 2) hipLaunchKernelGGL(vfn_mlp16_kernel<M16_FUSED_TRAIN | M16_C2>, dim3((unsigned)blocks), dim3(256), 0, (hipStream_t)stream, a);
    else if ((save_f16 & 3) == 3) hipLaunchKernelGGL(vfn_mlp16_kernel<M16_FUSED_TRAIN | M16_SF16>, dim3((unsigned)blocks), dim3(256), 0, (hipStream_t)stream, a);
    else hipLaunchKernelGGL(vfn_mlp16_kernel<M16_FUSED_TRAIN>, dim3((unsigned)blocks), dim3(256), 0, (hipStream_t)stream, a);
    return vfn_check_launch("vfn_vf_render_fused16_fwd_train");
}
```

### vf_nerf_amd/csrc/vfn_rays.hip

```cpp
#pragma clang fp contract(off)
#include <string.h>
#include "vfn_common.h"

namespace {

__device__ __forceinline__ bool argmax_takes(float ob, int oi, float best, int besti) {
    if (ob != ob) return best == best || oi < besti;
    return best == best && (ob > best || (ob == best && oi < besti));
}

constexpr int WAVE = 64;
constexpr int RAYS_PER_BLOCK = 4;
constexpr int MAX_SAMPLES = 512;

__device__ __forceinline__ float wave_sum(float v) {
#pragma unroll
    for (int o = 32; o > 0; o >>= 1) v += __shfl_xor(v, o, WAVE);
    return v;
}

__device__ __forceinline__ void philox_round(uint32_t (&c)[4], uint32_t (&k)[2]) {
    const uint64_t p0 = (uint64_t)0xD2511F53u * c[0];
    const uint64_t p1 = (uint64_t)0xCD9E8D57u * c[2];
    const uint32_t n0 = (uint32_t)(p1 >> 32) ^ c[1] ^ k[0];
    const uint32_t n1 = (uint32_t)p1;
    const uint32_t n2 = (uint32_t)(p0 >> 32) ^ c[3] ^ k[1];
    const uint32_t n3 = (uint32_t)p0;
    c[0] = n0; c[1] = n1; c[2] = n2; c[3] = n3;
    k[0] += 0x9E3779B9u; k[1] += 0xBB67AE85u;
}

struct PhiloxStream { unsigned long long seed, offset; };
__device__ __forceinline__ float philox_uniform(const PhiloxStream& ps, long long e) {
    const unsigned long long ctr = ps.offset + (unsigned long long)(e >> 2);
    uint32_t c[4] = {(uint32_t)ctr, (uint32_t)(ctr >> 32), 0u, 0u};
    uint32_t k[2] = {(uint32_t)ps.seed, (uint32_t)(ps.seed >> 32)};
#pragma unroll
    for (int r = 0; r < 10; ++r) philox_round(c, k);
    const int i = (int)(e & 3);
    const uint32_t v = i == 0 ? c[0] : (i == 1 ? c[1] : (i == 2 ? c[2] : c[3]));
    return (float)(v >> 8) * (1.0f / 16777216.0f);
}

constexpr int K1_RAYS = 16;

struct RaygenArgs {
    vfn_raygen_params p;
    const float* uv;
    const float* pose;
    const float* K;
    const float* t_vals;
    const float* far_per_ray;
    const float* u;
    float* directions;
    float* ray_dirs;
    float* cam_loc;
    float* z_vals;
    float* points;
    int gen_u;
    long long u_base;
    PhiloxStream ps;
    const float* k_sign;
};

__device__ __forceinline__ float coarse_z(float near, float far, float t) { return near * (1.0f - t) + far * t; }

__global__ __launch_bounds__(256) void vfn_raygen_kernel(const RaygenArgs a) {
    __shared__ float s_ray[K1_RAYS][8];
    const int tid = threadIdx.x;
    const int ray0 = blockIdx.x * K1_RAYS;
    const int n = a.p.n_rays;
    if (tid < K1_RAYS && ray0 + tid < n) {
        const int r = ray0 + tid;
        float P[3][4];
        if (a.p.pose_is_quat) {
            const float* q7 = a.pose + (size_t)r * 7;
            float q0 = q7[0], q1 = q7[1], q2 = q7[2], q3 = q7[3];
            const float nq = fmaxf(sqrtf(q0 * q0 + q1 * q1 + q2 * q2 + q3 * q3), 1e-12f);
            const float qr = q0 / nq, qi = q1 / nq, qj = q2 / nq, qk = q3 / nq;
            P[0][0] = 1 - 2 * (qj * qj + qk * qk); P[0][1] = 2 * (qj * qi - qk * qr); P[0][2] = 2 * (qi * qk + qr * qj);
            P[1][0] = 2 * (qj * qi + qk * qr); P[1][1] = 1 - 2 * (qi * qi + qk * qk); P[1][2] = 2 * (qj * qk - qi * qr);
            P[2][0] = 2 * (qk * qi - qj * qr); P[2][1] = 2 * (qj * qk + qi * qr); P[2][2] = 1 - 2 * (qi * qi + qj * qj);
            P[0][3] = q7[4]; P[1][3] = q7[5]; P[2][3] = q7[6];
        } else {
            const float* m = a.pose + (size_t)r * 16;
#pragma unroll
            for (int i = 0; i < 3; ++i)
#pragma unroll
                for (int j = 0; j < 4; ++j) P[i][j] = m[i * 4 + j];
        }
        const float* Kr = a.K + (size_t)r * 16;
        const float fx = Kr[0], sk = Kr[1], cx = Kr[2], fy = Kr[5], cy = Kr[6];
        const float fy0 = (a.k_sign ? a.k_sign : a.K)[5];
        const float zs = (fy0 > 0.f) ? 1.f : ((fy0 < 0.f) ? -1.f : 0.f);
        const float u = a.uv[(size_t)r * 2 + 0], v = a.uv[(size_t)r * 2 + 1];
        const float za = fabsf(zs);
        const float x = (u - cx + cy * sk / fy - sk * v / fy) / fx * za;
        const float y = (v - cy) / fy * za;
        float w[3];
#pragma unroll
        for (int i = 0; i < 3; ++i) w[i] = ((P[i][0] * x + P[i][1] * y) + P[i][2] * zs) + P[i][3];
        const float cam[3] = {P[0][3], P[1][3], P[2][3]};
        float d[3] = {w[0] - cam[0], w[1] - cam[1], w[2] - cam[2]};
        const float nd = fmaxf(sqrtf(d[0] * d[0] + d[1] * d[1] + d[2] * d[2]), 1e-12f);
#pragma unroll
        for (int i = 0; i < 3; ++i) {
            a.directions[(size_t)r * 3 + i] = d[i];
            a.ray_dirs[(size_t)r * 3 + i] = d[i] / nd;
            a.cam_loc[(size_t)r * 3 + i] = cam[i];
            s_ray[tid][i] = d[i];
            s_ray[tid][3 + i] = cam[i];
        }
        s_ray[tid][6] = a.far_per_ray ? a.far_per_ray[r] : a.p.far;
    }
    __syncthreads();
    const int S = a.p.n_samples;
    const int total = K1_RAYS * S;
    for (int idx = tid; idx < total; idx += blockDim.x) {
        const int lr = idx / S, s = idx - lr * S;
        const int r = ray0 + lr;
        if (r >= n) break;
        const float near = a.p.near, far = s_ray[lr][6];
        float z = coarse_z(near, far, a.t_vals[s]);
        if (a.u || a.gen_u) {
            const float zl = (s > 0) ? coarse_z(near, far, a.t_vals[s - 1]) : z;
            const float zu = (s < S - 1) ? coarse_z(near, far, a.t_vals[s + 1]) : z;
            const float upper = (s < S - 1) ? 0.5f * (zu + z) : z;
            const float lower = (s > 0) ? 0.5f * (z + zl) : z;
            z = lower + (upper - lower) * (a.gen_u ? philox_uniform(a.ps, a.u_base + (long long)r * S + s) : a.u[(size_t)r * S + s]);
        }
        const size_t o = (size_t)r * S + s;
        a.z_vals[o] = z;
        a.points[o * 3 + 0] = s_ray[lr][3] + z * s_ray[lr][0];
        a.points[o * 3 + 1] = s_ray[lr][4] + z * s_ray[lr][1];
        a.points[o * 3 + 2] = s_ray[lr][5] + z * s_ray[lr][2];
    }
}

struct DensityArgs {
    vfn_density_params p;
    const float* normals;
    const float* ray_dirs;
    const float* z_vals;
    const float* scalars;
    const float* colors;
    float* sigma;
    float* weights;
    long long* argmax;
    float* rgb;
    float* depth;
    const int* src;
    const float* normals_c;
    const float* colors_c;
    int n_stored_c;
};

__device__ __forceinline__ float laplace_cdf(float x, float beta, float scale, float mean) {
    const float a = x - mean;
    const float sg = (a > 0.f) ? 1.f : ((a < 0.f) ? -1.f : 0.f);
    const float t = 1.0f - expf(-fabsf(a) / beta);
    return scale * (0.5f + (0.5f * sg) * t);
}

__device__ __forceinline__ float dot3(const float* a, const float* b) { return (a[0] * b[0] + a[1] * b[1]) + a[2] * b[2]; }

__device__ __forceinline__ int density_ray(const DensityArgs& a, float* su, int ray, int lane) {
    const int S = a.p.n_samples;
    float* sz = su + (size_t)S * 3;
    float* se = sz + S;

    const float* nrm = a.normals + (size_t)ray * S * 3;
    for (int j = lane; j < S; j += WAVE) {
        if (a.src) {
            const int row = a.src[(size_t)ray * S + j];
            if (row < a.n_stored_c) {
                float* no = const_cast<float*>(nrm) + j * 3;
                float* co = const_cast<float*>(a.colors) + ((size_t)ray * S + j) * 3;
#pragma unroll
                for (int c = 0; c < 3; ++c) { no[c] = a.normals_c[(size_t)row * 3 + c]; co[c] = a.colors_c[(size_t)row * 3 + c]; }
            }
        }
        const float x = nrm[j * 3 + 0], y = nrm[j * 3 + 1], z = nrm[j * 3 + 2];
        const float nn = fmaxf(sqrtf((x * x + y * y) + z * z), 1e-8f);
        su[j * 3 + 0] = x / nn; su[j * 3 + 1] = y / nn; su[j * 3 + 2] = z / nn;
        sz[j] = a.z_vals[(size_t)ray * S + j];
    }
    float d[3] = {a.ray_dirs[(size_t)ray * 3 + 0], a.ray_dirs[(size_t)ray * 3 + 1], a.ray_dirs[(size_t)ray * 3 + 2]};
    {
        const float nd = fmaxf(sqrtf((d[0] * d[0] + d[1] * d[1]) + d[2] * d[2]), 1e-8f);
        d[0] /= nd; d[1] /= nd; d[2] /= nd;
    }
    const float beta = fminf(fmaxf(a.scalars[0], a.p.beta_min), a.p.beta_max);
    const float mean = fminf(fmaxf(a.scalars[1], a.p.mean_min), a.p.mean_max);
    const float scale = fmaxf(fabsf(a.scalars[2]), a.p.scale_min);
    const float cdf_cut = laplace_cdf(a.p.cutoff, beta, scale, mean);
    __builtin_amdgcn_wave_barrier();
    __builtin_amdgcn_fence(__ATOMIC_RELEASE, "wavefront");

    const int W = a.p.n_window;
    const int start = (int)((W + 1) / 2.0 + 1);
    const float wgt = 1.0f / (float)W;
    float wnorm = 0.f;
    for (int i = 0; i < W; ++i) wnorm += fabsf(wgt);
    const int L = S - 1;
    const int lo = start, hi = L - start;

    for (int j = lane; j < S; j += WAVE) {
        float sg = 0.f;
        if (j < L) {
            const float* uj = su + j * 3;
            float c = dot3(uj, su + (j + 1) * 3);
            if (j >= lo && j < hi) {
                c = c * wgt / wnorm;
                for (int i = 1; i < start - 1; ++i) {
                    const float f = dot3(uj, su + (j + 1 + i) * 3);
                    const float b = dot3(uj, su + (j - i) * 3);
                    c = (c + f * wgt / wnorm) + b * wgt / wnorm;
                }
            }
            const float c_ray = dot3(uj, d);
            sg = fmaxf(laplace_cdf(-c, beta, scale, mean) - cdf_cut, 0.f);
            if (c_ray < a.p.dir_to_normal_th && c < 0.f) sg = 0.f;
        }
        if (a.sigma) a.sigma[(size_t)ray * S + j] = sg;
        const float delta = (j < L) ? (sz[j + 1] - sz[j]) : 1e10f;
        se[j] = delta * sg;
    }
    __builtin_amdgcn_wave_barrier();
    __builtin_amdgcn_fence(__ATOMIC_ACQ_REL, "wavefront");

    const int C = (S + WAVE - 1) / WAVE;
    const int j0 = lane * C;
    double tot = 0.0;
    for (int i = 0; i < C; ++i) { const int j = j0 + i; if (j < S) tot += (double)se[j]; }
    double incl = tot;
#pragma unroll
    for (int o = 1; o < WAVE; o <<= 1) {
        const double up = __shfl_up(incl, o, WAVE);
        if (lane >= o) incl += up;
    }
    double run = incl - tot;
    float wsum_l = 0.f;
    for (int i = 0; i < C; ++i) {
        const int j = j0 + i;
        if (j < S) {
            const float e = se[j];
            const float T = expf(-(float)run);
            const float w = (1.0f - expf(-e)) * T;
            run += (double)e;
            se[j] = w;
            wsum_l += w;
        }
    }
    const float wsum = wave_sum(wsum_l);
    const float den = wsum + 1e-5f;
    __builtin_amdgcn_wave_barrier();
    __builtin_amdgcn_fence(__ATOMIC_ACQ_REL, "wavefront");

    float best = -INFINITY;
    int besti = 0x7fffffff;
    float acc[4] = {0.f, 0.f, 0.f, 0.f};
    const float* col = a.colors ? a.colors + (size_t)ray * S * 3 : nullptr;
    for (int j = lane; j < S; j += WAVE) {
        float w = se[j];
        if (a.p.normalize) w = w / den;
        if (a.weights) a.weights[(size_t)ray * S + j] = w;
        if (argmax_takes(w, j, best, besti)) { best = w; besti = j; }
        if (col) {
            acc[0] += w * col[j * 3 + 0]; acc[1] += w * col[j * 3 + 1]; acc[2] += w * col[j * 3 + 2];
            acc[3] += w * sz[j];
        }
    }
#pragma unroll
    for (int o = 32; o > 0; o >>= 1) {
        const float ob = __shfl_xor(best, o, WAVE);
        const int oi = __shfl_xor(besti, o, WAVE);
        if (argmax_takes(ob, oi, best, besti)) { best = ob; besti = oi; }
    }
    besti = (besti == 0x7fffffff) ? 0 : besti;
    if (a.argmax && lane == 0) a.argmax[ray] = besti;
    if (col) {
#pragma unroll
        for (int c = 0; c < 4; ++c) acc[c] = wave_sum(acc[c]);
        if (lane == 0) {
            a.rgb[(size_t)ray * 3 + 0] = acc[0]; a.rgb[(size_t)ray * 3 + 1] = acc[1]; a.rgb[(size_t)ray * 3 + 2] = acc[2];
            a.depth[ray] = acc[3];
        }
    }
    return besti;
}

__global__ __launch_bounds__(256) void vfn_density_kernel(const DensityArgs a) {
    extern __shared__ __attribute__((aligned(16))) float dsm[];
    const int wv = threadIdx.x >> 6, lane = threadIdx.x & 63;
    const int ray = blockIdx.x * RAYS_PER_BLOCK + wv;
    if (ray >= a.p.n_rays) return;
    (void)density_ray(a, dsm + (size_t)wv * a.p.n_samples * 5, ray, lane);
}

constexpr int MAX_SAMPLES_BWD = 256;

struct DensityBwdArgs {
    vfn_density_params p;
    const float* normals;
    const float* ray_dirs;
    const float* z_vals;
    const float* scalars;
    const float* colors;
    const float* d_rgb;
    const float* d_depth;
    const float* d_weights;
    const float* d_sigma;
    float* d_normals;
    float* d_colors;
    float* d_scalars;
};

__device__ __forceinline__ double wave_excl_scan_d(double v, int lane) {
    double incl = v;
#pragma unroll
    for (int o = 1; o < WAVE; o <<= 1) {
        const double up = __shfl_up(incl, o, WAVE);
        if (lane >= o) incl += up;
    }
    return incl - v;
}

__device__ __forceinline__ void density_bwd_ray(const DensityBwdArgs& a, float* bsm, int wv, int lane, int ray, float& gb_out, float& gm_out,
                                                float& gs_out) {
    const int S = a.p.n_samples;
    float* su = bsm + (size_t)wv * S * 12;
    float* sinv = su + (size_t)S * 3;
    float* sz = sinv + S;
    float* sc = sz + S;
    float* se = sc + S;
    float* sT = se + S;
    float* sw = sT + S;
    float* sg = sw + S;
    float* sact = sg + S;
    float* sdl = sact + S;

    const float* nrm = a.normals + (size_t)ray * S * 3;
    for (int j = lane; j < S; j += WAVE) {
        const float x = nrm[j * 3 + 0], y = nrm[j * 3 + 1], z = nrm[j * 3 + 2];
        const float nn = fmaxf(sqrtf((x * x + y * y) + z * z), 1e-8f);
        su[j * 3 + 0] = x / nn; su[j * 3 + 1] = y / nn; su[j * 3 + 2] = z / nn;
        sinv[j] = 1.0f / nn;
        sz[j] = a.z_vals[(size_t)ray * S + j];
    }
    float d[3] = {a.ray_dirs[(size_t)ray * 3 + 0], a.ray_dirs[(size_t)ray * 3 + 1], a.ray_dirs[(size_t)ray * 3 + 2]};
    {
        const float nd = fmaxf(sqrtf((d[0] * d[0] + d[1] * d[1]) + d[2] * d[2]), 1e-8f);
        d[0] /= nd; d[1] /= nd; d[2] /= nd;
    }
    const float braw = a.scalars[0], mraw = a.scalars[1], sraw = a.scalars[2];
    const float beta = fminf(fmaxf(braw, a.p.beta_min), a.p.beta_max);
    const float mean = fminf(fmaxf(mraw, a.p.mean_min), a.p.mean_max);
    const float scale = fmaxf(fabsf(sraw), a.p.scale_min);
    const float cdf_cut = laplace_cdf(a.p.cutoff, beta, scale, mean);
    __builtin_amdgcn_wave_barrier();

    const int W = a.p.n_window;
    const int start = (int)((W + 1) / 2.0 + 1);
    const float wgt = 1.0f / (float)W;
    float wnorm = 0.f;
    for (int i = 0; i < W; ++i) wnorm += fabsf(wgt);
    const float coef = wgt / wnorm;
    const int L = S - 1;
    const int lo = start, hi = L - start;

    for (int j = lane; j < S; j += WAVE) {
        float sgm = 0.f, c = 1.f, act = 0.f;
        if (j < L) {
            const float* uj = su + j * 3;
            c = dot3(uj, su + (j + 1) * 3);
            if (j >= lo && j < hi) {
                c = c * wgt / wnorm;
                for (int i = 1; i < start - 1; ++i) {
                    const float f = dot3(uj, su + (j + 1 + i) * 3);
                    const float b = dot3(uj, su + (j - i) * 3);
                    c = (c + f * wgt / wnorm) + b * wgt / wnorm;
                }
            }
            const float c_ray = dot3(uj, d);
            const float raw = laplace_cdf(-c, beta, scale, mean) - cdf_cut;
            const bool masked = (c_ray < a.p.dir_to_normal_th && c < 0.f);
            if (raw > 0.f && !masked) { sgm = raw; act = 1.f; }
        }
        sc[j] = c;
        sact[j] = act;
        const float delta = (j < L) ? (sz[j + 1] - sz[j]) : 1e10f;
        sdl[j] = delta;
        se[j] = delta * sgm;
    }
    __builtin_amdgcn_wave_barrier();

    const int C = (S + WAVE - 1) / WAVE;
    const int j0 = lane * C;
    double tot = 0.0;
    for (int i = 0; i < C; ++i) { const int j = j0 + i; if (j < S) tot += (double)se[j]; }
    double run = wave_excl_scan_d(tot, lane);
    float wsum_l = 0.f;
    for (int i = 0; i < C; ++i) {
        const int j = j0 + i;
        if (j < S) {
            const float e = se[j];
            const float T = expf(-(float)run);
            const float w = (1.0f - expf(-e)) * T;
            run += (double)e;
            sT[j] = T; sw[j] = w;
            wsum_l += w;
        }
    }
    const float wsum = wave_sum(wsum_l);
    const float den = a.p.normalize ? (wsum + 1e-5f) : 1.0f;
    __builtin_amdgcn_wave_barrier();

    float drgb[3] = {0.f, 0.f, 0.f}, ddep = 0.f;
    if (a.d_rgb) { drgb[0] = a.d_rgb[(size_t)ray * 3 + 0]; drgb[1] = a.d_rgb[(size_t)ray * 3 + 1]; drgb[2] = a.d_rgb[(size_t)ray * 3 + 2]; }
    if (a.d_depth) ddep = a.d_depth[ray];
    const float* col = a.colors ? a.colors + (size_t)ray * S * 3 : nullptr;
    float dot_l = 0.f;
    for (int j = lane; j < S; j += WAVE) {
        const float w = sw[j] / den;
        float g = ddep * sz[j];
        if (col) g += (drgb[0] * col[j * 3 + 0] + drgb[1] * col[j * 3 + 1]) + drgb[2] * col[j * 3 + 2];
        if (a.d_weights) g += a.d_weights[(size_t)ray * S + j];
        if (a.d_colors) {
            float* dc = a.d_colors + ((size_t)ray * S + j) * 3;
            dc[0] = w * drgb[0]; dc[1] = w * drgb[1]; dc[2] = w * drgb[2];
        }
        sg[j] = g;
        dot_l += g * w;
    }
    const float gdot = wave_sum(dot_l);
    __builtin_amdgcn_wave_barrier();
    double qtot = 0.0;
    for (int i = 0; i < C; ++i) {
        const int j = j0 + i;
        if (j < S) {
            const float gh = a.p.normalize ? (sg[j] - gdot) / den : sg[j];
            sg[j] = gh;
            qtot += (double)(gh * sw[j]);
        }
    }
    const double qpre = wave_excl_scan_d(qtot, lane);
    double qall = qtot;
#pragma unroll
    for (int o = 32; o > 0; o >>= 1) qall += __shfl_xor(qall, o, WAVE);
    double qrun = qpre;
    float gb = 0.f, gm = 0.f, gs = 0.f;
    const float Ec = expf(-fabsf(a.p.cutoff - mean) / beta);
    const float ac = a.p.cutoff - mean;
    const float Fcut = cdf_cut / scale;
    for (int i = 0; i < C; ++i) {
        const int j = j0 + i;
        if (j < S) {
            const float gh = sg[j];
            qrun += (double)(gh * sw[j]);
            const float suffix = (float)(qall - qrun);
            float gc = 0.f;
            if (j < L && sact[j] != 0.f) {
                const float e = se[j];
                const float de = gh * sT[j] * expf(-e) - suffix;
                const float dsig = sdl[j] * de + (a.d_sigma ? a.d_sigma[(size_t)ray * S + j] : 0.f);
                const float x = -sc[j];
                const float ax = x - mean;
                const float E = expf(-fabsf(ax) / beta);
                const float sgx = (ax > 0.f) ? 1.f : ((ax < 0.f) ? -1.f : 0.f);
                const float Fx = 0.5f + 0.5f * sgx * (1.0f - E);
                gc = -dsig * scale * 0.5f * E / beta;
                gs += dsig * (Fx - Fcut);
                gm += dsig * scale * (-0.5f * E / beta + 0.5f * Ec / beta);
                gb += dsig * scale * (-0.5f * ax * E + 0.5f * ac * Ec) / (beta * beta);
            }
            sg[j] = gc;
        }
    }
    __builtin_amdgcn_wave_barrier();
    gb_out = wave_sum(gb); gm_out = wave_sum(gm); gs_out = wave_sum(gs);
    for (int j = lane; j < S; j += WAVE) {
        float du[3] = {0.f, 0.f, 0.f};
        if (j < L) {
            const float gcj = sg[j];
            if (gcj != 0.f) {
                if (j >= lo && j < hi) {
                    for (int t = 1; t <= start - 1; ++t) { const float* un = su + (j + t) * 3; du[0] += coef * gcj * un[0]; du[1] += coef * gcj * un[1]; du[2] += coef * gcj * un[2]; }
                    for (int t = 1; t <= start - 2; ++t) { const float* un = su + (j - t) * 3; du[0] += coef * gcj * un[0]; du[1] += coef * gcj * un[1]; du[2] += coef * gcj * un[2]; }
                } else {
                    const float* un = su + (j + 1) * 3;
                    du[0] += gcj * un[0]; du[1] += gcj * un[1]; du[2] += gcj * un[2];
                }
            }
        }
        for (int i = max(0, j - (start - 1)); i <= min(L - 1, j + (start - 2)); ++i) {
            if (i == j) continue;
            const float gci = sg[i];
            if (gci == 0.f) continue;
            const bool interior = (i >= lo && i < hi);
            const int off = j - i;
            float wgt_ij = 0.f;
            if (interior) { if ((off >= 1 && off <= start - 1) || (off <= -1 && off >= -(start - 2))) wgt_ij = coef; }
            else if (off == 1) wgt_ij = 1.f;
            if (wgt_ij != 0.f) { const float* ui = su + i * 3; du[0] += wgt_ij * gci * ui[0]; du[1] += wgt_ij * gci * ui[1]; du[2] += wgt_ij * gci * ui[2]; }
        }
        const float* uj = su + j * 3;
        const float inv = sinv[j];
        float dn[3];
        if (inv >= 1e8f * 0.999f) {
            dn[0] = du[0] * inv; dn[1] = du[1] * inv; dn[2] = du[2] * inv;
        } else {
            const float pr = (du[0] * uj[0] + du[1] * uj[1]) + du[2] * uj[2];
            dn[0] = (du[0] - pr * uj[0]) * inv; dn[1] = (du[1] - pr * uj[1]) * inv; dn[2] = (du[2] - pr * uj[2]) * inv;
        }
        float* o = a.d_normals + ((size_t)ray * S + j) * 3;
        o[0] += dn[0]; o[1] += dn[1]; o[2] += dn[2];
    }
}

__global__ __launch_bounds__(1024) void vfn_density_bwd_kernel(const DensityBwdArgs a) {
    extern __shared__ __attribute__((aligned(16))) float bsm[];
    __shared__ float s_red[16][3];
    const int wv = threadIdx.x >> 6, lane = threadIdx.x & 63, waves = blockDim.x >> 6;
    const int ray = blockIdx.x * waves + wv;
    float gb = 0.f, gm = 0.f, gs = 0.f;
    if (ray < a.p.n_rays) density_bwd_ray(a, bsm, wv, lane, ray, gb, gm, gs);
    if (!a.d_scalars) return;
    if (lane == 0) { s_red[wv][0] = gb; s_red[wv][1] = gm; s_red[wv][2] = gs; }
    __syncthreads();
    if (threadIdx.x < 3) {
        float v = 0.f;
        for (int w = 0; w < waves; ++w) v += s_red[w][threadIdx.x];
        const float braw = a.scalars[0], mraw = a.scalars[1], sraw = a.scalars[2];
        if (threadIdx.x == 0 && braw >= a.p.beta_min && braw <= a.p.beta_max) atomicAdd(a.d_scalars + 0, v);
        if (threadIdx.x == 1 && mraw >= a.p.mean_min && mraw <= a.p.mean_max) atomicAdd(a.d_scalars + 1, v);
        if (threadIdx.x == 2 && fabsf(sraw) >= a.p.scale_min) atomicAdd(a.d_scalars + 2, (sraw >= 0.f) ? v : -v);
    }
}

struct FineArgs {
    vfn_fine_params p;
    const float* z_coarse;
    const long long* argmax;
    const float* directions;
    const float* cam_loc;
    const float* far_per_ray;
    const float* u_fine;
    const float* u_add;
    float* z_vals;
    float* points;
    int* src;
    float* new_points;
    int* dst;
    int new_row0;
    int gen_fine, gen_add;
    long long fine_base, add_base;
    PhiloxStream ps;
};

__device__ __forceinline__ void fine_ray(const FineArgs& a, float* sv, int ray, int lane, long long imax) {
    const int Sc = a.p.n_coarse, Nf = a.p.n_fine, St = Sc + Nf;
    float* so = sv + St;
    const float* zc = a.z_coarse + (size_t)ray * Sc;
    for (int j = lane; j < Sc; j += WAVE) sv[j] = zc[j];
    const float near = a.p.near;
    const float far = a.far_per_ray ? a.far_per_ray[ray] : a.p.far;
    if (imax > 0) {
        const float zstar = zc[imax];
        const float base = zstar - a.p.half_range;
        const float step = a.p.window_step;
        for (int k = lane; k < Nf; k += WAVE) {
            float z = base + step * (float)k;
            if (a.u_fine || a.gen_fine) {
                const float zl = base + step * (float)(k - 1);
                const float zu = base + step * (float)(k + 1);
                const float upper = (k < Nf - 1) ? 0.5f * (zu + z) : z;
                const float lower = (k > 0) ? 0.5f * (z + zl) : z;
                z = lower + (upper - lower) * (a.gen_fine ? philox_uniform(a.ps, a.fine_base + (long long)ray * Nf + k) : a.u_fine[(size_t)ray * Nf + k]);
            }
            sv[Sc + k] = z;
        }
    } else {
        const float span = a.far_per_ray ? (far - near) : a.p.span;
        for (int k = lane; k < Nf; k += WAVE)
            sv[Sc + k] = (a.gen_add ? philox_uniform(a.ps, a.add_base + (long long)ray * Nf + k) : a.u_add[(size_t)ray * Nf + k]) * span + near;
    }
    __builtin_amdgcn_wave_barrier();
    __builtin_amdgcn_fence(__ATOMIC_ACQ_REL, "wavefront");
    for (int i = lane; i < St; i += WAVE) {
        const float v = sv[i];
        int rank = 0;
        for (int j = 0; j < St; ++j) {
            const float o = sv[j];
            rank += (o < v || (o == v && j < i)) ? 1 : 0;
        }
        so[rank] = v;
        const int row = i < Sc ? ray * Sc + i : a.new_row0 + ray * Nf + (i - Sc);
        if (a.src) a.src[(size_t)ray * St + rank] = row;
        if (a.dst) a.dst[row] = ray * St + rank;
    }
    __builtin_amdgcn_wave_barrier();
    __builtin_amdgcn_fence(__ATOMIC_ACQ_REL, "wavefront");
    const float dx = a.directions[(size_t)ray * 3 + 0], dy = a.directions[(size_t)ray * 3 + 1], dz = a.directions[(size_t)ray * 3 + 2];
    const float ox = a.cam_loc[(size_t)ray * 3 + 0], oy = a.cam_loc[(size_t)ray * 3 + 1], oz = a.cam_loc[(size_t)ray * 3 + 2];
    for (int j = lane; j < St; j += WAVE) {
        const float z = so[j];
        const size_t o = (size_t)ray * St + j;
        a.z_vals[o] = z;
        a.points[o * 3 + 0] = ox + z * dx;
        a.points[o * 3 + 1] = oy + z * dy;
        a.points[o * 3 + 2] = oz + z * dz;
    }
    if (a.new_points) {
        for (int k = lane; k < Nf; k += WAVE) {
            const float z = sv[Sc + k];
            const size_t o = (size_t)ray * Nf + k;
            a.new_points[o * 3 + 0] = ox + z * dx;
            a.new_points[o * 3 + 1] = oy + z * dy;
            a.new_points[o * 3 + 2] = oz + z * dz;
        }
    }
}

__global__ __launch_bounds__(256) void vfn_fine_kernel(const FineArgs a) {
    extern __shared__ __attribute__((aligned(16))) float fsm[];
    const int wv = threadIdx.x >> 6, lane = threadIdx.x & 63;
    const int ray = blockIdx.x * RAYS_PER_BLOCK + wv;
    if (ray >= a.p.n_rays) return;
    fine_ray(a, fsm + (size_t)wv * (a.p.n_coarse + a.p.n_fine) * 2, ray, lane, a.argmax[ray]);
}

__global__ __launch_bounds__(256) void vfn_density_fine_kernel(const DensityArgs d, const FineArgs f) {
    extern __shared__ __attribute__((aligned(16))) float dfm[];
    const int wv = threadIdx.x >> 6, lane = threadIdx.x & 63;
    const int ray = blockIdx.x * RAYS_PER_BLOCK + wv;
    if (ray >= d.p.n_rays) return;
    const int per_wave = max(d.p.n_samples * 5, (f.p.n_coarse + f.p.n_fine) * 2);
    float* lds = dfm + (size_t)wv * per_wave;
    const int imax = density_ray(d, lds, ray, lane);
    __builtin_amdgcn_wave_barrier();
    __builtin_amdgcn_fence(__ATOMIC_ACQ_REL, "wavefront");
    fine_ray(f, lds, ray, lane, (long long)imax);
}

__global__ void vfn_uniform_kernel(float* out, long long n, unsigned long long seed, unsigned long long offset) {
    const long long g = (long long)blockIdx.x * blockDim.x + threadIdx.x;
    const long long base = g * 4;
    if (base >= n) return;
    const unsigned long long ctr = offset + (unsigned long long)g;
    uint32_t c[4] = {(uint32_t)ctr, (uint32_t)(ctr >> 32), 0u, 0u};
    uint32_t k[2] = {(uint32_t)seed, (uint32_t)(seed >> 32)};
#pragma unroll
    for (int r = 0; r < 10; ++r) philox_round(c, k);
#pragma unroll
    for (int i = 0; i < 4; ++i)
        if (base + i < n) out[base + i] = (float)(c[i] >> 8) * (1.0f / 16777216.0f);
}

struct ShellArgs {
    const float* u;
    const float* centroid;
    float* points;
    float* gt;
    long long n;
    float r_min, r_max;
    int inward;
    unsigned long long seed, offset;
};

__global__ void vfn_sphere_shell_kernel(const ShellArgs a) {
    const long long i = (long long)blockIdx.x * blockDim.x + threadIdx.x;
    if (i >= a.n) return;
    float u0, u1, u2;
    if (a.u) { u0 = a.u[i * 3 + 0]; u1 = a.u[i * 3 + 1]; u2 = a.u[i * 3 + 2]; }
    else {
        const unsigned long long ctr = a.offset + (unsigned long long)i;
        uint32_t c[4] = {(uint32_t)ctr, (uint32_t)(ctr >> 32), 0u, 0u};
        uint32_t k[2] = {(uint32_t)a.seed, (uint32_t)(a.seed >> 32)};
#pragma unroll
        for (int r = 0; r < 10; ++r) philox_round(c, k);
        u0 = (float)(c[0] >> 8) * (1.0f / 16777216.0f);
        u1 = (float)(c[1] >> 8) * (1.0f / 16777216.0f);
        u2 = (float)(c[2] >> 8) * (1.0f / 16777216.0f);
    }
    const float phi = 6.283185307179586f * u0;
    const float ct = 2.0f * u1 - 1.0f;
    const float st = sqrtf(fmaxf(0.f, 1.0f - ct * ct));
    const float r = cbrtf(u2) * (a.r_max - a.r_min) + a.r_min;
    float sp, cp;
    sincosf(phi, &sp, &cp);
    const float cx = a.centroid[0], cy = a.centroid[1], cz = a.centroid[2];
    const float px = r * st * cp + cx, py = r * st * sp + cy, pz = r * ct + cz;
    a.points[i * 3 + 0] = px; a.points[i * 3 + 1] = py; a.points[i * 3 + 2] = pz;
    float dx = px - cx, dy = py - cy, dz = pz - cz;
    if (a.inward) { dx = -dx; dy = -dy; dz = -dz; }
    const float inv = 1.0f / fmaxf(sqrtf(dx * dx + dy * dy + dz * dz), 1e-12f);
    a.gt[i * 3 + 0] = dx * inv; a.gt[i * 3 + 1] = dy * inv; a.gt[i * 3 + 2] = dz * inv;
}


__global__ __launch_bounds__(256) void vfn_scatter_rows3_kernel(const float* a, const float* b, const int* index, long long n,
                                                                 float* out_a, float* out_b) {
    const long long r = (long long)blockIdx.x * 256 + threadIdx.x;
    if (r >= n) return;
    const int d = index[r];
    if (d < 0) return;
#pragma unroll
    for (int c = 0; c < 3; ++c) {
        out_a[(long long)d * 3 + c] = a[r * 3 + c];
        if (b) out_b[(long long)d * 3 + c] = b[r * 3 + c];
    }
}

struct UniformSampleArgs {
    const float* directions;
    const float* cam_loc;
    const float* t_vals;
    const float* far_per_ray;
    const float* u;
    float* z_vals;
    float* points;
    int n_rays, n_samples;
    float near, far;
};

__global__ __launch_bounds__(256) void vfn_uniform_sample_kernel(const UniformSampleArgs a) {
    const long long idx = (long long)blockIdx.x * blockDim.x + threadIdx.x;
    const int S = a.n_samples;
    if (idx >= (long long)a.n_rays * S) return;
    const int r = (int)(idx / S), s = (int)(idx - (long long)r * S);
    const float near = a.near, far = a.far_per_ray ? a.far_per_ray[r] : a.far;
    float z = coarse_z(near, far, a.t_vals[s]);
    if (a.u) {
        const float zl = (s > 0) ? coarse_z(near, far, a.t_vals[s - 1]) : z;
        const float zu = (s < S - 1) ? coarse_z(near, far, a.t_vals[s + 1]) : z;
        const float upper = (s < S - 1) ? 0.5f * (zu + z) : z;
        const float lower = (s > 0) ? 0.5f * (z + zl) : z;
        z = lower + (upper - lower) * a.u[idx];
    }
    a.z_vals[idx] = z;
    if (a.points) {
        a.points[idx * 3 + 0] = a.cam_loc[(size_t)r * 3 + 0] + z * a.directions[(size_t)r * 3 + 0];
        a.points[idx * 3 + 1] = a.cam_loc[(size_t)r * 3 + 1] + z * a.directions[(size_t)r * 3 + 1];
        a.points[idx * 3 + 2] = a.cam_loc[(size_t)r * 3 + 2] + z * a.directions[(size_t)r * 3 + 2];
    }
}

__global__ __launch_bounds__(256) void vfn_rows_argmax_kernel(const float* w, int n_rows, int n_cols, long long* out) {
    const int wv = threadIdx.x >> 6, lane = threadIdx.x & 63;
    const int row = blockIdx.x * RAYS_PER_BLOCK + wv;
    if (row >= n_rows) return;
    float best = -INFINITY;
    int besti = 0x7fffffff;
    for (int j = lane; j < n_cols; j += WAVE) {
        const float v = w[(size_t)row * n_cols + j];
        if (argmax_takes(v, j, best, besti)) { best = v; besti = j; }
    }
#pragma unroll
    for (int o = 32; o > 0; o >>= 1) {
        const float ob = __shfl_xor(best, o, WAVE);
        const int oi = __shfl_xor(besti, o, WAVE);
        if (argmax_takes(ob, oi, best, besti)) { best = ob; besti = oi; }
    }
    if (lane == 0) out[row] = (besti == 0x7fffffff) ? 0 : besti;
}

__global__ __launch_bounds__(256) void vfn_merge_sort_depths_kernel(const float* z, const float* extra, int n_rays, int s, int e, int p2,
                                                                    const float* directions, const float* cam_loc, float* z_out, float* points) {
    extern __shared__ float sbuf[];
    const int wv = threadIdx.x >> 6, lane = threadIdx.x & 63;
    const int ray = blockIdx.x * RAYS_PER_BLOCK + wv;
    const bool live = ray < n_rays;
    float* buf = sbuf + wv * p2;
    const int tot = s + e;
    for (int i = lane; i < p2; i += WAVE)
        buf[i] = !live || i >= tot ? __builtin_nanf("") : (i < s ? z[(size_t)ray * s + i] : extra[(size_t)ray * e + (i - s)]);
    __syncthreads();
    for (int k = 2; k <= p2; k <<= 1)
        for (int j = k >> 1; j > 0; j >>= 1) {
            for (int i = lane; i < p2; i += WAVE) {
                const int q = i ^ j;
                if (q > i) {
                    const float a = buf[i], b = buf[q];
                    const bool a_gt_b = (a != a && b == b) || a > b;
                    const bool up = (i & k) == 0;
                    if (a_gt_b == up && (a_gt_b || (b != b && a == a) || b > a)) { buf[i] = b; buf[q] = a; }
                }
            }
            __syncthreads();
        }
    if (!live) return;
    for (int i = lane; i < tot; i += WAVE) {
        const float zz = buf[i];
        const size_t idx = (size_t)ray * tot + i;
        z_out[idx] = zz;
        if (points) {
            points[idx * 3 + 0] = cam_loc[(size_t)ray * 3 + 0] + zz * directions[(size_t)ray * 3 + 0];
            points[idx * 3 + 1] = cam_loc[(size_t)ray * 3 + 1] + zz * directions[(size_t)ray * 3 + 1];
            points[idx * 3 + 2] = cam_loc[(size_t)ray * 3 + 2] + zz * directions[(size_t)ray * 3 + 2];
        }
    }
}

}

extern "C" int vfn_uniform_sample(int32_t n_rays, int32_t n_samples, float near, float far, const float* directions,
                                  const float* cam_loc, const float* t_vals, const float* far_per_ray, const float* u,
                                  float* z_vals, float* points, void* stream) {
    if (n_rays == 0) return VFN_OK;
    VFN_REQUIRE(n_rays > 0 && n_samples >= 1, "vfn_uniform_sample: bad sizes (n_rays=%d, n_samples=%d)", n_rays, n_samples);
    VFN_REQUIRE(t_vals && z_vals && (!points || (directions && cam_loc)), "vfn_uniform_sample: NULL argument");
    UniformSampleArgs a{directions, cam_loc, t_vals, far_per_ray, u, z_vals, points, n_rays, n_samples, near, far};
    const long long total = (long long)n_rays * n_samples;
    hipLaunchKernelGGL(vfn_uniform_sample_kernel, dim3((unsigned)((total + 255) / 256)), dim3(256), 0, (hipStream_t)stream, a);
    return vfn_check_launch("vfn_uniform_sample");
}

extern "C" int vfn_merge_sort_depths(const float* z_vals, const float* extra, int32_t n_rays, int32_t n_samples, int32_t n_extra,
                                     const float* directions, const float* cam_loc, float* z_out, float* points, void* stream) {
    if (n_rays == 0) return VFN_OK;
    VFN_REQUIRE(n_rays > 0 && n_samples >= 0 && n_extra >= 0 && n_samples + n_extra >= 1 && n_samples + n_extra <= 2048,
                "vfn_merge_sort_depths: bad sizes (n_rays=%d, n_samples=%d, n_extra=%d; at most 2048 depths per ray)", n_rays, n_samples, n_extra);
    VFN_REQUIRE((z_vals || n_samples == 0) && (extra || n_extra == 0) && z_out && (!points || (directions && cam_loc)),
                "vfn_merge_sort_depths: NULL argument");
    int p2 = 2;
    while (p2 < n_samples + n_extra) p2 <<= 1;
    hipLaunchKernelGGL(vfn_merge_sort_depths_kernel, dim3((unsigned)((n_rays + RAYS_PER_BLOCK - 1) / RAYS_PER_BLOCK)), dim3(256),
                       (size_t)RAYS_PER_BLOCK * p2 * sizeof(float), (hipStream_t)stream, z_vals, extra, (int)n_rays, (int)n_samples, (int)n_extra, p2,
                       directions, cam_loc, z_out, points);
    return vfn_check_launch("vfn_merge_sort_depths");
}

extern "C" int vfn_rows_argmax(const float* w, int32_t n_rows, int32_t n_cols, int64_t* out, void* stream) {
    if (n_rows == 0) return VFN_OK;
    VFN_REQUIRE(w && out && n_rows > 0 && n_cols >= 1, "vfn_rows_argmax: bad argument");
    hipLaunchKernelGGL(vfn_rows_argmax_kernel, dim3((unsigned)((n_rows + RAYS_PER_BLOCK - 1) / RAYS_PER_BLOCK)), dim3(256), 0,
                       (hipStream_t)stream, w, (int)n_rows, (int)n_cols, (long long*)out);
    return vfn_check_launch("vfn_rows_argmax");
}

extern "C" int vfn_raygen_uniform(const vfn_raygen_params* p, const float* uv, const float* pose, const float* intrinsics,
                                  const float* t_vals, const float* far_per_ray, const float* u_coarse, float* directions,
                                  float* ray_dirs, float* cam_loc, float* z_vals, float* points, void* stream) {
    if (p && p->n_rays == 0) return VFN_OK;
    VFN_REQUIRE(p && uv && pose && intrinsics && t_vals && directions && ray_dirs && cam_loc && z_vals && points,
                "vfn_raygen_uniform: NULL argument");
    VFN_REQUIRE(p->n_rays >= 0 && p->n_samples >= 1, "vfn_raygen_uniform: bad sizes (n_rays=%d, n_samples=%d)", p->n_rays,
                p->n_samples);
    if (p->n_rays == 0) return VFN_OK;
    RaygenArgs a{*p, uv, pose, intrinsics, t_vals, far_per_ray, u_coarse, directions, ray_dirs, cam_loc, z_vals, points};
    const unsigned blocks = (unsigned)((p->n_rays + K1_RAYS - 1) / K1_RAYS);
    hipLaunchKernelGGL(vfn_raygen_kernel, dim3(blocks), dim3(256), 0, (hipStream_t)stream, a);
    return vfn_check_launch("vfn_raygen_uniform");
}

extern "C" int vfn_ray_density_weights(const vfn_density_params* p, const float* normals, const float* ray_dirs,
                                       const float* z_vals, const float* density_scalars, const float* colors, float* sigma,
                                       float* weights, int64_t* argmax, float* rgb, float* depth, void* stream) {
    if (p && p->n_rays <= 0) return VFN_OK;
    VFN_REQUIRE(p && normals && ray_dirs && z_vals && density_scalars, "vfn_ray_density_weights: NULL argument");
    VFN_REQUIRE(p->n_samples >= 2 && p->n_samples <= MAX_SAMPLES, "vfn_ray_density_weights: n_samples=%d outside [2,%d]",
                p->n_samples, MAX_SAMPLES);
    VFN_REQUIRE(p->n_window >= 1, "vfn_ray_density_weights: n_window must be >= 1");
    VFN_REQUIRE(!colors || (rgb && depth), "vfn_ray_density_weights: colors given but rgb/depth NULL");
    if (p->n_rays <= 0) return VFN_OK;
    DensityArgs a{*p, normals, ray_dirs, z_vals, density_scalars, colors, sigma, weights, (long long*)argmax, rgb, depth};
    const unsigned blocks = (unsigned)((p->n_rays + RAYS_PER_BLOCK - 1) / RAYS_PER_BLOCK);
    const size_t shmem = (size_t)RAYS_PER_BLOCK * p->n_samples * 5 * sizeof(float);
    hipLaunchKernelGGL(vfn_density_kernel, dim3(blocks), dim3(256), shmem, (hipStream_t)stream, a);
    return vfn_check_launch("vfn_ray_density_weights");
}

extern "C" int vfn_range_fine_sample(const vfn_fine_params* p, const float* z_coarse, const int64_t* argmax,
                                     const float* directions, const float* cam_loc, const float* far_per_ray,
                                     const float* u_fine, const float* u_add, float* z_vals, float* points, void* stream) {
    return vfn_range_fine_sample_indexed(p, z_coarse, argmax, directions, cam_loc, far_per_ray, u_fine, u_add, z_vals, points,
                                         nullptr, nullptr, nullptr, p ? (int64_t)p->n_rays * p->n_coarse : 0, stream);
}

extern "C" int vfn_range_fine_sample_indexed(const vfn_fine_params* p, const float* z_coarse, const int64_t* argmax,
                                             const float* directions, const float* cam_loc, const float* far_per_ray,
                                             const float* u_fine, const float* u_add, float* z_vals, float* points,
                                             int32_t* src, float* new_points, int32_t* dst, int64_t new_row0, void* stream) {
    if (p && p->n_rays <= 0) return VFN_OK;
    VFN_REQUIRE(p && z_coarse && argmax && directions && cam_loc && u_add && z_vals && points,
                "vfn_range_fine_sample: NULL argument (u_add is always required, ray_sampler.py:292)");
    VFN_REQUIRE(p->n_coarse >= 1 && p->n_fine >= 2 && p->n_coarse + p->n_fine <= MAX_SAMPLES,
                "vfn_range_fine_sample: bad sizes (n_coarse=%d, n_fine=%d)", p->n_coarse, p->n_fine);
    VFN_REQUIRE((long long)p->n_rays * (p->n_coarse + p->n_fine) < (1ll << 31), "vfn_range_fine_sample: more than 2^31 samples");
    VFN_REQUIRE(new_row0 >= (long long)p->n_rays * p->n_coarse && new_row0 + (long long)p->n_rays * p->n_fine < (1ll << 31),
                "vfn_range_fine_sample_indexed: new_row0=%lld must not overlap the proposal rows", (long long)new_row0);
    FineArgs a{*p, z_coarse, (const long long*)argmax, directions, cam_loc, far_per_ray, u_fine, u_add, z_vals, points, src, new_points,
               dst, (int)new_row0};
    const unsigned blocks = (unsigned)((p->n_rays + RAYS_PER_BLOCK - 1) / RAYS_PER_BLOCK);
    const size_t shmem = (size_t)RAYS_PER_BLOCK * (p->n_coarse + p->n_fine) * 2 * sizeof(float);
    hipLaunchKernelGGL(vfn_fine_kernel, dim3(blocks), dim3(256), shmem, (hipStream_t)stream, a);
    return vfn_check_launch("vfn_range_fine_sample");
}

int vfn_internal_raygen(const vfn_raygen_params* p, const float* uv, const float* pose, const float* intrinsics, const float* k_sign,
                        const float* t_vals, const float* far_per_ray, const float* u_coarse, int gen_u, long long u_base, uint64_t seed,
                        uint64_t offset, float* directions, float* ray_dirs, float* cam_loc, float* z_vals, float* points, void* stream) {
    RaygenArgs a{*p, uv, pose, intrinsics, t_vals, far_per_ray, u_coarse, directions, ray_dirs, cam_loc, z_vals, points};
    a.gen_u = gen_u; a.u_base = u_base; a.ps = PhiloxStream{seed, offset}; a.k_sign = k_sign;
    const unsigned blocks = (unsigned)((p->n_rays + K1_RAYS - 1) / K1_RAYS);
    hipLaunchKernelGGL(vfn_raygen_kernel, dim3(blocks), dim3(256), 0, (hipStream_t)stream, a);
    return vfn_check_launch("vfn_render_fwd (rays)");
}

int vfn_internal_density_fine(const vfn_density_params* dp, const float* normals_c, const float* ray_dirs, const float* z_c,
                              const float* density_scalars, const vfn_fine_params* fp, const float* directions, const float* cam_loc,
                              const float* far_per_ray, const float* u_fine, const float* u_add, int gen_fine, int gen_add,
                              long long fine_base, long long add_base, uint64_t seed, uint64_t offset, float* z_vals, float* points,
                              int32_t* src, float* new_points, int32_t* dst, int64_t new_row0, void* stream) {
    VFN_REQUIRE(dp->n_samples >= 2 && dp->n_samples <= MAX_SAMPLES && fp->n_coarse + fp->n_fine <= MAX_SAMPLES && fp->n_fine >= 2 &&
                dp->n_window >= 1, "vfn_render_fwd: sample counts outside what the per-ray kernels support (n_coarse=%d, n_fine=%d)",
                fp->n_coarse, fp->n_fine);
    VFN_REQUIRE((long long)fp->n_rays * (fp->n_coarse + fp->n_fine) < (1ll << 31), "vfn_render_fwd: more than 2^31 samples");
    DensityArgs d{*dp, normals_c, ray_dirs, z_c, density_scalars, nullptr, nullptr, nullptr, nullptr, nullptr, nullptr};
    FineArgs f{*fp, z_c, nullptr, directions, cam_loc, far_per_ray, u_fine, u_add, z_vals, points, src, new_points, dst, (int)new_row0};
    f.gen_fine = gen_fine; f.gen_add = gen_add; f.fine_base = fine_base; f.add_base = add_base; f.ps = PhiloxStream{seed, offset};
    const unsigned blocks = (unsigned)((dp->n_rays + RAYS_PER_BLOCK - 1) / RAYS_PER_BLOCK);
    const int per_wave = dp->n_samples * 5 > (fp->n_coarse + fp->n_fine) * 2 ? dp->n_samples * 5 : (fp->n_coarse + fp->n_fine) * 2;
    hipLaunchKernelGGL(vfn_density_fine_kernel, dim3(blocks), dim3(256), (size_t)RAYS_PER_BLOCK * per_wave * sizeof(float),
                       (hipStream_t)stream, d, f);
    return vfn_check_launch("vfn_render_fwd (proposal weights + fine sampler)");
}

int vfn_internal_composite_gather(const vfn_density_params* dp, float* normals, const float* ray_dirs, const float* z_vals,
                                  const float* density_scalars, float* colors, const int32_t* src, const float* normals_c,
                                  const float* colors_c, int64_t n_stored_c, float* weights, float* rgb, float* depth, void* stream) {
    VFN_REQUIRE(dp->n_samples >= 2 && dp->n_samples <= MAX_SAMPLES, "vfn_render_fwd: n_samples=%d outside [2,%d]", dp->n_samples, MAX_SAMPLES);
    DensityArgs a{*dp, normals, ray_dirs, z_vals, density_scalars, colors, nullptr, weights, nullptr, rgb, depth};
    a.src = src; a.normals_c = normals_c; a.colors_c = colors_c; a.n_stored_c = (int)n_stored_c;
    const unsigned blocks = (unsigned)((dp->n_rays + RAYS_PER_BLOCK - 1) / RAYS_PER_BLOCK);
    hipLaunchKernelGGL(vfn_density_kernel, dim3(blocks), dim3(256), (size_t)RAYS_PER_BLOCK * dp->n_samples * 5 * sizeof(float),
                       (hipStream_t)stream, a);
    return vfn_check_launch("vfn_render_fwd (composite)");
}

namespace {
__device__ __forceinline__ bool sel_predicate(const float* w, const float* sigma, const float* z, int ray, int S, int j, int lane, double& carry) {
    const size_t i = (size_t)ray * S + j;
    const bool in = j < S;
    const bool pos = in && w[i] > 0.f;
    if (!sigma) return pos;
    const float sg = in ? sigma[i] : 0.f;
    const float delta = !in ? 0.f : (j < S - 1 ? z[i + 1] - z[i] : 1e10f);
    const double e = (double)(sg * delta);
    double incl = e;
#pragma unroll
    for (int o = 1; o < 64; o <<= 1) {
        const double up = __shfl_up(incl, o, 64);
        if (lane >= o) incl += up;
    }
    const double before = carry + (incl - e);
    carry += __shfl(incl, 63, 64);
    return pos || (in && sg > 0.f && delta > 0.f && before < 110.0);
}

__global__ void vfn_sel_count_kernel(const float* w, const float* sigma, const float* z, int n_rays, int S, int32_t* cnt) {
    const int ray = blockIdx.x * 4 + (threadIdx.x >> 6), lane = threadIdx.x & 63;
    if (ray >= n_rays) return;
    int c = 0;
    double carry = 0.0;
    for (int j0 = 0; j0 < S; j0 += 64) c += sel_predicate(w, sigma, z, ray, S, j0 + lane, lane, carry) ? 1 : 0;
#pragma unroll
    for (int o = 32; o > 0; o >>= 1) c += __shfl_xor(c, o, 64);
    if (lane == 0) cnt[ray] = c;
}

__global__ __launch_bounds__(256) void vfn_sel_scan_kernel(const int32_t* cnt, int n, int32_t* off, int32_t* k_dev) {
    __shared__ int s_sum[256];
    const int t = threadIdx.x;
    const int per = (n + 255) / 256, lo = t * per, hi = min(n, lo + per);
    int sum = 0;
    for (int i = lo; i < hi; ++i) sum += cnt[i];
    s_sum[t] = sum;
    __syncthreads();
    for (int o = 1; o < 256; o <<= 1) {
        const int v = t >= o ? s_sum[t - o] : 0;
        __syncthreads();
        s_sum[t] += v;
        __syncthreads();
    }
    int run = s_sum[t] - sum;
    for (int i = lo; i < hi; ++i) { off[i] = run; run += cnt[i]; }
    if (t == 255) k_dev[0] = s_sum[255];
}

__global__ void vfn_sel_compact_kernel(const float* w, const float* sigma, const float* z, int n_rays, int S, const int32_t* off, const float* points,
                                       const float* ray_dirs, int32_t* sel_sorted, float* pts_sel, float* dirs_sel) {
    const int ray = blockIdx.x * 4 + (threadIdx.x >> 6), lane = threadIdx.x & 63;
    if (ray >= n_rays) return;
    int base = off[ray];
    const float dx = ray_dirs[(size_t)ray * 3 + 0], dy = ray_dirs[(size_t)ray * 3 + 1], dz = ray_dirs[(size_t)ray * 3 + 2];
    double carry = 0.0;
    for (int j0 = 0; j0 < S; j0 += 64) {
        const int j = j0 + lane;
        const bool sel = sel_predicate(w, sigma, z, ray, S, j, lane, carry);
        const unsigned long long mask = __ballot(sel);
        if (sel) {
            const int k = base + __popcll(mask & ((1ull << lane) - 1ull));
            const size_t i = (size_t)ray * S + j;
            sel_sorted[k] = (int32_t)i;
            pts_sel[(size_t)k * 3 + 0] = points[i * 3 + 0]; pts_sel[(size_t)k * 3 + 1] = points[i * 3 + 1]; pts_sel[(size_t)k * 3 + 2] = points[i * 3 + 2];
            dirs_sel[(size_t)k * 3 + 0] = dx; dirs_sel[(size_t)k * 3 + 1] = dy; dirs_sel[(size_t)k * 3 + 2] = dz;
        }
        base += __popcll(mask);
    }
}

__global__ void vfn_sel_rows3_kernel(const float* a, const int32_t* index, const int32_t* k_dev, float* out, int gather) {
    const long long k = (long long)blockIdx.x * blockDim.x + threadIdx.x;
    if (k >= (long long)*k_dev) return;
    const size_t i = (size_t)index[k];
    const size_t from = gather ? i : (size_t)k, to = gather ? (size_t)k : i;
    out[to * 3 + 0] = a[from * 3 + 0]; out[to * 3 + 1] = a[from * 3 + 1]; out[to * 3 + 2] = a[from * 3 + 2];
}

}

int vfn_internal_select_positive(const float* weights, const float* sigma, const float* z_vals, int n_rays, int n_samples, const float* points,
                                 const float* ray_dirs, int32_t* cnt, int32_t* off, int32_t* k_dev, int32_t* sel_sorted, float* pts_sel,
                                 float* dirs_sel, void* stream) {
    VFN_REQUIRE((sigma == nullptr) == (z_vals == nullptr), "vfn_internal_select_positive: sigma and z_vals come together");
    VFN_REQUIRE(weights && points && ray_dirs && cnt && off && k_dev && sel_sorted && pts_sel && dirs_sel && n_rays > 0 && n_samples > 0,
                "vfn_internal_select_positive: bad argument");
    hipStream_t s = (hipStream_t)stream;
    const unsigned blocks = (unsigned)((n_rays + 3) / 4);
    hipLaunchKernelGGL(vfn_sel_count_kernel, dim3(blocks), dim3(256), 0, s, weights, sigma, z_vals, n_rays, n_samples, cnt);
    hipLaunchKernelGGL(vfn_sel_scan_kernel, dim3(1), dim3(256), 0, s, cnt, n_rays, off, k_dev);
    hipLaunchKernelGGL(vfn_sel_compact_kernel, dim3(blocks), dim3(256), 0, s, weights, sigma, z_vals, n_rays, n_samples, off, points, ray_dirs,
                       sel_sorted, pts_sel, dirs_sel);
    return vfn_check_launch("sample selection (w > 0)");
}

extern "C" int vfn_select_samples(const float* weights, const float* sigma, const float* z_vals, int32_t n_rays, int32_t n_samples, const float* points,
                                  const float* ray_dirs, int32_t* scratch, int32_t* count, int32_t* index, float* points_sel, float* dirs_sel,
                                  void* stream) {
    VFN_REQUIRE(scratch && count, "vfn_select_samples: NULL scratch / count");
    return vfn_internal_select_positive(weights, sigma, z_vals, n_rays, n_samples, points, ray_dirs, scratch, scratch + n_rays, count, index, points_sel,
                                        dirs_sel, stream);
}

int vfn_internal_rows3_by_index(const float* a, const int32_t* index, const int32_t* k_dev, int64_t capacity, float* out, int gather, void* stream) {
    VFN_REQUIRE(a && index && k_dev && out && capacity >= 0, "vfn_internal_rows3_by_index: bad argument");
    if (capacity == 0) return VFN_OK;
    hipLaunchKernelGGL(vfn_sel_rows3_kernel, dim3((unsigned)((capacity + 255) / 256)), dim3(256), 0, (hipStream_t)stream, a, index, k_dev, out, gather);
    return vfn_check_launch("selected rows scatter / gather");
}

extern "C" int vfn_scatter_rows3(const float* a, const float* b, const int32_t* index, int64_t n_rows, float* out_a, float* out_b,
                                 void* stream) {
    VFN_REQUIRE(n_rows >= 0 && (n_rows == 0 || (a && index && out_a && (!b || out_b))), "vfn_scatter_rows3: NULL argument");
    if (n_rows == 0) return VFN_OK;
    hipLaunchKernelGGL(vfn_scatter_rows3_kernel, dim3((unsigned)((n_rows + 255) / 256)), dim3(256), 0, (hipStream_t)stream, a, b, index,
                       (long long)n_rows, out_a, out_b);
    return vfn_check_launch("vfn_scatter_rows3");
}

extern "C" int vfn_fill_uniform(float* out, int64_t n, uint64_t seed, uint64_t offset, void* stream) {
    VFN_REQUIRE(out || n == 0, "vfn_fill_uniform: NULL output");
    if (n <= 0) return VFN_OK;
    const long long groups = (n + 3) / 4;
    const unsigned blocks = (unsigned)((groups + 255) / 256);
    hipLaunchKernelGGL(vfn_uniform_kernel, dim3(blocks), dim3(256), 0, (hipStream_t)stream, out, (long long)n,
                       (unsigned long long)seed, (unsigned long long)offset);
    return vfn_check_launch("vfn_fill_uniform");
}

static int bwd_rays_per_block(int n_samples) {
    int rpb = 16;
    while (rpb > 1 && (size_t)rpb * n_samples * 12 * sizeof(float) > 60 * 1024) rpb >>= 1;
    return rpb;
}

extern "C" int vfn_ray_density_weights_bwd(const vfn_density_params* p, const float* normals, const float* ray_dirs,
                                           const float* z_vals, const float* density_scalars, const float* colors,
                                           const float* d_rgb, const float* d_depth, const float* d_weights,
                                           float* d_normals, float* d_colors, float* d_scalars, void* stream) {
    if (p && p->n_rays <= 0) return VFN_OK;
    VFN_REQUIRE(p && normals && ray_dirs && z_vals && density_scalars && d_normals, "vfn_ray_density_weights_bwd: NULL argument");
    VFN_REQUIRE(p->n_samples >= 2 && p->n_samples <= MAX_SAMPLES_BWD,
                "vfn_ray_density_weights_bwd: n_samples=%d outside [2,%d]", p->n_samples, MAX_SAMPLES_BWD);
    VFN_REQUIRE(p->n_window >= 1, "vfn_ray_density_weights_bwd: n_window must be >= 1");
    VFN_REQUIRE(!(d_rgb && !colors), "vfn_ray_density_weights_bwd: d_rgb given without colors");
    if (p->n_rays <= 0) return VFN_OK;
    DensityBwdArgs a{*p, normals, ray_dirs, z_vals, density_scalars, colors, d_rgb, d_depth, d_weights, nullptr, d_normals, d_colors, d_scalars};
    const int rpb = bwd_rays_per_block(p->n_samples);
    const unsigned blocks = (unsigned)((p->n_rays + rpb - 1) / rpb);
    const size_t shmem = (size_t)rpb * p->n_samples * 12 * sizeof(float);
    hipLaunchKernelGGL(vfn_density_bwd_kernel, dim3(blocks), dim3(64 * rpb), shmem, (hipStream_t)stream, a);
    return vfn_check_launch("vfn_ray_density_weights_bwd");
}

extern "C" int vfn_ray_density_sigma_bwd(const vfn_density_params* p, const float* normals, const float* ray_dirs,
                                         const float* z_vals, const float* density_scalars, const float* d_sigma,
                                         float* d_normals, float* d_scalars, void* stream) {
    if (p && p->n_rays <= 0) return VFN_OK;
    VFN_REQUIRE(p && normals && ray_dirs && z_vals && density_scalars && d_sigma && d_normals, "vfn_ray_density_sigma_bwd: NULL argument");
    VFN_REQUIRE(p->n_samples >= 2 && p->n_samples <= MAX_SAMPLES_BWD,
                "vfn_ray_density_sigma_bwd: n_samples=%d outside [2,%d]", p->n_samples, MAX_SAMPLES_BWD);
    VFN_REQUIRE(p->n_window >= 1, "vfn_ray_density_sigma_bwd: n_window must be >= 1");
    DensityBwdArgs a{*p, normals, ray_dirs, z_vals, density_scalars, nullptr, nullptr, nullptr, nullptr, d_sigma, d_normals, nullptr, d_scalars};
    const int rpb = bwd_rays_per_block(p->n_samples);
    const unsigned blocks = (unsigned)((p->n_rays + rpb - 1) / rpb);
    const size_t shmem = (size_t)rpb * p->n_samples * 12 * sizeof(float);
    hipLaunchKernelGGL(vfn_density_bwd_kernel, dim3(blocks), dim3(64 * rpb), shmem, (hipStream_t)stream, a);
    return vfn_check_launch("vfn_ray_density_sigma_bwd");
}

extern "C" int vfn_sample_sphere_shell(int64_t n, float r_min, float r_max, const float* centroid, int32_t inward, const float* u,
                                       uint64_t seed, uint64_t offset, float* points, float* gt, void* stream) {
    if (n <= 0) return VFN_OK;
    VFN_REQUIRE(centroid && points && gt, "vfn_sample_sphere_shell: NULL argument");
    VFN_REQUIRE(r_max >= r_min && r_min >= 0.f, "vfn_sample_sphere_shell: need 0 <= r_min <= r_max (got %g, %g)", (double)r_min, (double)r_max);
    ShellArgs a{u, centroid, points, gt, (long long)n, r_min, r_max, inward ? 1 : 0, (unsigned long long)seed, (unsigned long long)offset};
    hipLaunchKernelGGL(vfn_sphere_shell_kernel, dim3((unsigned)((n + 255) / 256)), dim3(256), 0, (hipStream_t)stream, a);
    return vfn_check_launch("vfn_sample_sphere_shell");
}
```

### vf_nerf_amd/csrc/vfn_render.hip

```cpp
#include <string.h>
#include "vfn_common.h"

namespace {

struct Carve {
    unsigned char* base;
    size_t off;
    template <typename T> T* take(size_t count) {
        T* p = reinterpret_cast<T*>(base ? base + off : nullptr);
        off += ((count * sizeof(T) + 255) / 256) * 256;
        return p;
    }
};

struct Ws {
    float *directions, *cam_loc, *z_c, *pts_c, *normals_c, *colors_c, *new_pts, *u;
    int32_t *dst, *src;
    int64_t* imax;
    int32_t *cnt, *off, *k_dev, *sel_sorted;
    float *pts_sel, *dirs_sel;
    size_t bytes;
};

Ws carve(void* workspace, const vfn_render_params* p) {
    const size_t n = (size_t)p->n_rays, sc = (size_t)p->n_coarse, nf = (size_t)p->n_fine;
    Carve c{static_cast<unsigned char*>(workspace), 0};
    Ws w;
    w.directions = c.take<float>(n * 3);
    w.cam_loc = c.take<float>(n * 3);
    w.z_c = c.take<float>(n * sc);
    w.pts_c = c.take<float>(n * sc * 3);
    w.normals_c = c.take<float>(n * (p->sparse_colours ? sc + nf : sc) * 3);
    w.colors_c = c.take<float>(n * sc * 3);
    w.new_pts = c.take<float>(n * nf * 3);
    w.dst = c.take<int32_t>(n * (sc + nf));
    w.src = c.take<int32_t>(n * (sc + nf));
    w.u = c.take<float>(p->separate_launches ? n * (sc + 2 * nf) + 4 : 0);
    w.imax = c.take<int64_t>(p->separate_launches ? n : 0);
    const size_t cap = p->sparse_colours ? n * (sc + nf) : 0;
    w.cnt = c.take<int32_t>(p->sparse_colours ? n : 0);
    w.off = c.take<int32_t>(p->sparse_colours ? n : 0);
    w.k_dev = c.take<int32_t>(p->sparse_colours ? 4 : 0);
    w.sel_sorted = c.take<int32_t>(cap);
    w.pts_sel = c.take<float>(cap * 3);
    w.dirs_sel = c.take<float>(cap * 3);
    w.bytes = c.off;
    return w;
}

constexpr int MAX_SIDE = 3;
struct Side { hipStream_t s[MAX_SIDE]; hipEvent_t fork, join[MAX_SIDE]; int dev; };
Side* side_streams() {
    static thread_local Side side = {{nullptr, nullptr, nullptr}, nullptr, {nullptr, nullptr, nullptr}, -1};
    int dev = -1;
    if (hipGetDevice(&dev) != hipSuccess) return nullptr;
    if (side.dev != dev) {
        if (side.dev >= 0) {
            for (int i = 0; i < MAX_SIDE; ++i) { (void)hipStreamDestroy(side.s[i]); (void)hipEventDestroy(side.join[i]); }
            (void)hipEventDestroy(side.fork);
            side.dev = -1;
        }
        if (hipEventCreateWithFlags(&side.fork, hipEventDisableTiming) != hipSuccess) return nullptr;
        for (int i = 0; i < MAX_SIDE; ++i)
            if (hipStreamCreateWithFlags(&side.s[i], hipStreamNonBlocking) != hipSuccess ||
                hipEventCreateWithFlags(&side.join[i], hipEventDisableTiming) != hipSuccess) return nullptr;
        side.dev = dev;
    }
    return &side;
}

}

extern "C" int64_t vfn_render_fwd_workspace_bytes(const vfn_render_params* p) {
    if (!p || p->n_rays < 0 || p->n_coarse < 1 || p->n_fine < 2) return VFN_ERR_INVALID;
    return (int64_t)carve(nullptr, p).bytes;
}

extern "C" int vfn_render_fwd(const vfn_render_params* p, const vfn_net_geom* vf_geom, const void* vf_packed16,
                              const vfn_net_geom* rn_geom, const void* rn_packed16, const float* uv, const float* pose,
                              const float* intrinsics, const float* t_vals, const float* far_coarse_per_ray,
                              const float* far_fine_per_ray, const float* density_scalars, const float* u_coarse,
                              const float* u_fine, const float* u_add, void* workspace, float* ray_dirs, float* z_vals,
                              float* points, float* normals, float* colors, float* weights, float* rgb, float* depth,
                              void* stream) {
    VFN_REQUIRE(p && vf_geom && rn_geom, "vfn_render_fwd: NULL argument");
    if (p->n_rays == 0) return VFN_OK;
    VfnReportScope report(p->status_word, p->clock_stamps, p->clock_slots);
    VFN_REQUIRE(p->n_rays > 0 && p->n_coarse >= 1 && p->n_fine >= 2, "vfn_render_fwd: bad sizes (n_rays=%d, n_coarse=%d, n_fine=%d)",
                p->n_rays, p->n_coarse, p->n_fine);
    VFN_REQUIRE(vf_packed16 && rn_packed16 && uv && pose && intrinsics && t_vals && density_scalars && workspace && ray_dirs && z_vals &&
                points && normals && colors && weights && rgb && depth, "vfn_render_fwd: NULL argument");
    const int n = p->n_rays, sc = p->n_coarse, nf = p->n_fine, st = sc + nf;
    VFN_REQUIRE((long long)n * st < (1ll << 22), "vfn_render_fwd: at most 4194303 samples per call");
    VFN_REQUIRE(p->colour_products == 0 || p->colour_products == 2 || p->colour_products == 3, "vfn_render_fwd: colour_products must be 0, 2 or 3");
    const Ws w = carve(workspace, p);
    int rc;
    const int gen_c = p->perturb_coarse && !u_coarse, gen_f = p->perturb_fine && !u_fine, gen_a = !u_add;
    const long long base_f = gen_c ? (long long)n * sc : 0, base_a = base_f + (gen_f ? (long long)n * nf : 0);
    vfn_raygen_params rp = {n, sc, p->pose_is_quat, p->near_coarse, p->far_coarse};
    const int products = p->colour_products == 2 ? 2 : 3;
    if (p->sparse_colours) {
        const float* uc = (p->perturb_coarse && u_coarse) ? u_coarse : nullptr;
        rc = vfn_internal_raygen(&rp, uv, pose, intrinsics, intrinsics, t_vals, far_coarse_per_ray, uc, gen_c, 0, p->seed, p->offset, w.directions, ray_dirs,
                                 w.cam_loc, w.z_c, w.pts_c, stream);
        if (rc != VFN_OK) return rc;
        rc = vfn_vf_mlp16_fwd(vf_geom, vf_packed16, w.pts_c, (int64_t)n * sc, w.normals_c, stream);
        if (rc != VFN_OK) return rc;
        vfn_density_params dq = p->density;
        dq.n_rays = n; dq.n_samples = sc;
        vfn_fine_params fq = {n, sc, nf, p->near_fine, p->far_fine, p->fine_range, p->window_step, p->span};
        rc = vfn_internal_density_fine(&dq, w.normals_c, ray_dirs, w.z_c, density_scalars, &fq, w.directions, w.cam_loc, far_fine_per_ray,
                                       (p->perturb_fine && u_fine) ? u_fine : nullptr, u_add, gen_f, gen_a, base_f, base_a, p->seed, p->offset, z_vals,
                                       points, w.src, w.new_pts, w.dst, (int64_t)n * sc, stream);
        if (rc != VFN_OK) return rc;
        rc = vfn_vf_mlp16_fwd(vf_geom, vf_packed16, w.new_pts, (int64_t)n * nf, w.normals_c + (size_t)n * sc * 3, stream);
        if (rc != VFN_OK) return rc;
        rc = vfn_scatter_rows3(w.normals_c, nullptr, w.dst, (int64_t)n * st, normals, nullptr, stream);
        if (rc != VFN_OK) return rc;
        dq.n_samples = st;
        rc = vfn_ray_density_weights(&dq, normals, ray_dirs, z_vals, density_scalars, nullptr, nullptr, weights, nullptr, nullptr, nullptr, stream);
        if (rc != VFN_OK) return rc;
        rc = vfn_internal_select_positive(weights, nullptr, nullptr, n, st, points, ray_dirs, w.cnt, w.off, w.k_dev, w.sel_sorted, w.pts_sel, w.dirs_sel, stream);
        if (rc != VFN_OK) return rc;
        if (hipMemsetAsync(colors, 0, (size_t)n * st * 3 * sizeof(float), (hipStream_t)stream) != hipSuccess) {
            vfn_set_error("vfn_render_fwd: could not clear the colours");
            return VFN_ERR_LAUNCH;
        }
        if (p->timing_events[0]) (void)hipEventRecord((hipEvent_t)p->timing_events[0], (hipStream_t)stream);
        rc = vfn_internal_fused16_products_dev(vf_geom, vf_packed16, rn_geom, rn_packed16, w.pts_sel, w.dirs_sel, (int64_t)n * st, w.k_dev, 1, w.sel_sorted,
                                               products, normals, colors, stream);
        if (rc != VFN_OK) return rc;
        if (p->timing_events[1]) (void)hipEventRecord((hipEvent_t)p->timing_events[1], (hipStream_t)stream);
        return vfn_ray_density_weights(&dq, normals, ray_dirs, z_vals, density_scalars, colors, nullptr, weights, nullptr, rgb, depth, stream);
    }
    if (p->separate_launches) {
        const float* uc = p->perturb_coarse ? u_coarse : nullptr;
        const float* uf = p->perturb_fine ? u_fine : nullptr;
        const float* ua = u_add;
        if (gen_c) uc = w.u;
        if (gen_f) uf = w.u + base_f;
        if (gen_a) ua = w.u + base_a;
        const long long need = base_a + (gen_a ? (long long)n * nf : 0);
        if (need) { rc = vfn_fill_uniform(w.u, need, p->seed, p->offset, stream); if (rc != VFN_OK) return rc; }
        rc = vfn_raygen_uniform(&rp, uv, pose, intrinsics, t_vals, far_coarse_per_ray, uc, w.directions, ray_dirs, w.cam_loc, w.z_c, w.pts_c, stream);
        if (rc != VFN_OK) return rc;
        rc = vfn_vf_render_fused16_products(vf_geom, vf_packed16, rn_geom, rn_packed16, w.pts_c, ray_dirs, (int64_t)n * sc, sc, nullptr, products,
                                            w.normals_c, w.colors_c, stream);
        if (rc != VFN_OK) return rc;
        vfn_density_params dq = p->density;
        dq.n_rays = n; dq.n_samples = sc;
        rc = vfn_ray_density_weights(&dq, w.normals_c, ray_dirs, w.z_c, density_scalars, nullptr, nullptr, nullptr, w.imax, nullptr, nullptr, stream);
        if (rc != VFN_OK) return rc;
        vfn_fine_params fq = {n, sc, nf, p->near_fine, p->far_fine, p->fine_range, p->window_step, p->span};
        rc = vfn_range_fine_sample_indexed(&fq, w.z_c, w.imax, w.directions, w.cam_loc, far_fine_per_ray, uf, ua, z_vals, points, nullptr, w.new_pts,
                                           w.dst, (int64_t)n * sc, stream);
        if (rc != VFN_OK) return rc;
        rc = vfn_vf_render_fused16_products(vf_geom, vf_packed16, rn_geom, rn_packed16, w.new_pts, ray_dirs, (int64_t)n * nf, nf,
                                            w.dst + (size_t)n * sc, products, normals, colors, stream);
        if (rc != VFN_OK) return rc;
        rc = vfn_scatter_rows3(w.normals_c, w.colors_c, w.dst, (int64_t)n * sc, normals, colors, stream);
        if (rc != VFN_OK) return rc;
        dq.n_samples = st;
        return vfn_ray_density_weights(&dq, normals, ray_dirs, z_vals, density_scalars, colors, nullptr, weights, nullptr, rgb, depth, stream);
    }
    auto stage = [&](int which, int ray0, int nh, hipStream_t s) -> int {
        const size_t r = (size_t)ray0;
        float* dirs_h = ray_dirs + r * 3;
        float* n_c = w.normals_c + r * sc * 3; float* c_c = w.colors_c + r * sc * 3;
        int32_t* dst_h = w.dst + r * st; int32_t* src_h = w.src + r * st;
        vfn_density_params dp = p->density;
        dp.n_rays = nh;
        switch (which) {
        case 0: {
            vfn_raygen_params rq = {nh, sc, p->pose_is_quat, p->near_coarse, p->far_coarse};
            return vfn_internal_raygen(&rq, uv + r * 2, pose + r * (p->pose_is_quat ? 7 : 16), intrinsics + r * 16, intrinsics, t_vals,
                                       far_coarse_per_ray ? far_coarse_per_ray + r : nullptr,
                                       (p->perturb_coarse && u_coarse) ? u_coarse + r * sc : nullptr, gen_c, (long long)r * sc, p->seed, p->offset,
                                       w.directions + r * 3, dirs_h, w.cam_loc + r * 3, w.z_c + r * sc, w.pts_c + r * sc * 3, s);
        }
        case 1:
            return vfn_vf_render_fused16_products(vf_geom, vf_packed16, rn_geom, rn_packed16, w.pts_c + r * sc * 3, dirs_h, (int64_t)nh * sc, sc, nullptr,
                                                  products, n_c, c_c, s);
        case 2: {
            dp.n_samples = sc;
            vfn_fine_params fp = {nh, sc, nf, p->near_fine, p->far_fine, p->fine_range, p->window_step, p->span};
            return vfn_internal_density_fine(&dp, n_c, dirs_h, w.z_c + r * sc, density_scalars, &fp, w.directions + r * 3, w.cam_loc + r * 3,
                                             far_fine_per_ray ? far_fine_per_ray + r : nullptr, (p->perturb_fine && u_fine) ? u_fine + r * nf : nullptr,
                                             u_add ? u_add + r * nf : nullptr, gen_f, gen_a, base_f + (long long)r * nf, base_a + (long long)r * nf,
                                             p->seed, p->offset, z_vals + r * st, points + r * st * 3, src_h, w.new_pts + r * nf * 3, dst_h,
                                             (int64_t)nh * sc, s);
        }
        case 3:
            return vfn_vf_render_fused16_products(vf_geom, vf_packed16, rn_geom, rn_packed16, w.new_pts + r * nf * 3, dirs_h, (int64_t)nh * nf, nf,
                                                  dst_h + (size_t)nh * sc, products, normals + r * st * 3, colors + r * st * 3, s);
        default:
            dp.n_samples = st;
            return vfn_internal_composite_gather(&dp, normals + r * st * 3, dirs_h, z_vals + r * st, density_scalars, colors + r * st * 3, src_h, n_c, c_c,
                                                 (int64_t)nh * sc, weights + r * st, rgb + r * 3, depth + r, s);
        }
    };
    hipStream_t main_s = (hipStream_t)stream;
    auto mark = [&](int slot) {
        if (p->timing_events[slot]) (void)hipEventRecord((hipEvent_t)p->timing_events[slot], main_s);
    };
    int parts = (p->streams >= 2 && p->streams <= MAX_SIDE + 1 && n >= 32 * p->streams) ? p->streams : 1;
    if (p->streams == 0 && n >= 512) {
        const long long wp = ((long long)n * sc + 127) / 128, wq = ((long long)n * nf + 127) / 128;
        const long long waste = (wp + 255) / 256 * 256 - wp + (wq + 255) / 256 * 256 - wq;
        if (20 * waste >= wp + wq) parts = 2;
    }
    Side* side = parts > 1 ? side_streams() : nullptr;
    if (!side) {
        for (int k = 0; k < 5; ++k) {
            if (k == 1 || k == 3) mark(k - 1);
            rc = stage(k, 0, n, main_s);
            if (rc != VFN_OK) return rc;
            if (k == 1 || k == 3) mark(k);
        }
        return VFN_OK;
    }
    int r0[MAX_SIDE + 2];
    for (int i = 0; i <= parts; ++i) r0[i] = i == parts ? n : (int)((long long)n * i / parts + 3) / 4 * 4;
    if (hipEventRecord(side->fork, main_s) != hipSuccess) { vfn_set_error("vfn_render_fwd: could not fork the side streams"); return VFN_ERR_LAUNCH; }
    for (int i = 1; i < parts; ++i)
        if (hipStreamWaitEvent(side->s[i - 1], side->fork, 0) != hipSuccess) { vfn_set_error("vfn_render_fwd: could not fork the side streams"); return VFN_ERR_LAUNCH; }
    rc = VFN_OK;
    for (int k = 0; k < 5 && rc == VFN_OK; ++k)
        for (int i = 0; i < parts && rc == VFN_OK; ++i)
            if (r0[i + 1] > r0[i]) {
                if (i == 0 && (k == 1 || k == 3)) mark(k - 1);
                rc = stage(k, r0[i], r0[i + 1] - r0[i], i == 0 ? main_s : side->s[i - 1]);
                if (i == 0 && (k == 1 || k == 3)) mark(k);
            }
    for (int i = 1; i < parts; ++i)
        if (hipEventRecord(side->join[i - 1], side->s[i - 1]) != hipSuccess || hipStreamWaitEvent(main_s, side->join[i - 1], 0) != hipSuccess) {
            vfn_set_error("vfn_render_fwd: could not join the side streams");
            return VFN_ERR_LAUNCH;
        }
    return rc;
}
```

Measured before the change: 2.034 million.

## Precompute per-ray direction encoding operand rows in raygen, reuse in fused render

Raygen now computes each ray's positional encoding of the view direction once, split into hi/lo f16 pairs, and writes it into a per-ray workspace table. The fused render kernels for the coarse and fine passes load these precomputed operand rows with buffer loads issued before the head layer, and patch in only the per-sample point and normal entries. This is meant to remove the repeated per-sample sincos and split work on direction features. In exchange it adds a workspace table, extra global traffic, and hard-coded insert positions that only hold for rn_multires == 4.

```diff
diff --git a/vf_nerf_amd/csrc/vfn_aux16.h b/vf_nerf_amd/csrc/vfn_aux16.h
--- /dev/null
+++ b/vf_nerf_amd/csrc/vfn_aux16.h
@@ -0,0 +1,88 @@
+#pragma once
+#include <hip/hip_runtime.h>
+#include <stdint.h>
+
+typedef _Float16 half8 __attribute__((ext_vector_type(8)));
+typedef _Float16 half2v __attribute__((ext_vector_type(2)));
+typedef float float2v __attribute__((ext_vector_type(2)));
+
+constexpr float VFN16_XSCALE = 64.0f;
+#define VFN16_CLAMP 60000.0f
+
+struct A16 { half8 hi[3]; half8 lo[3]; };
+
+constexpr int VFN16_DIR_MULTIRES = 4;
+constexpr int VFN16_DIR_ROW_BYTES = 2 * 3 * 2 * 16;
+constexpr int VFN16_DIR_ROW_U4 = VFN16_DIR_ROW_BYTES / 16;
+
+__device__ __forceinline__ void split2(float a, float b, _Float16& h0, _Float16& h1, _Float16& l0, _Float16& l1) {
+    const float2v v = {a, b};
+    const half2v hi = __builtin_convertvector(v, half2v);
+    h0 = hi[0]; h1 = hi[1];
+    const uint32_t hp = __builtin_bit_cast(uint32_t, hi);
+    float r0, r1;
+    asm("v_fma_mix_f32 %0, %1, -1.0, %2 op_sel_hi:[1,0,0]" : "=v"(r0) : "v"(hp), "v"(a));
+    asm("v_fma_mix_f32 %0, %1, -1.0, %2 op_sel:[1,0,0] op_sel_hi:[1,0,0]" : "=v"(r1) : "v"(hp), "v"(b));
+    const float2v r = {r0, r1};
+    const half2v lo = __builtin_convertvector(r, half2v);
+    l0 = lo[0]; l1 = lo[1];
+}
+
+__device__ __forceinline__ float aux_pair(float v0, float v1, _Float16& h0, _Float16& h1, _Float16& l0, _Float16& l1) {
+    v0 *= VFN16_XSCALE; v1 *= VFN16_XSCALE;
+    v0 = fminf(fmaxf(v0, -VFN16_CLAMP), VFN16_CLAMP); v1 = fminf(fmaxf(v1, -VFN16_CLAMP), VFN16_CLAMP);
+    split2(v0, v1, h0, h1, l0, l1);
+    return fmaxf(fabsf(v0), fabsf(v1));
+}
+
+__device__ __forceinline__ float enc_value(const float (&x)[3], const float (&sn)[18], const float (&cs)[18], int multires, int k) {
+    if (k < 3) return x[k];
+    const int idx = k - 3, oct = idx / 6, rem = idx - 6 * oct;
+    if (oct >= multires) return 0.f;
+    return rem < 3 ? sn[3 * oct + rem] : cs[3 * oct + rem - 3];
+}
+
+template <typename F>
+__device__ __forceinline__ void build_aux(A16& aux, int g, F col, float& ain) {
+#pragma unroll
+    for (int s = 0; s < 3; ++s) {
+        half8 hi, lo;
+#pragma unroll
+        for (int j = 0; j < 8; j += 2) {
+            float v0, v1;
+            if (g == 0) { v0 = col(16 * s + j); v1 = col(16 * s + j + 1); }
+            else { v0 = col(16 * s + 8 + j); v1 = col(16 * s + 8 + j + 1); }
+            _Float16 h0, h1, l0, l1;
+            ain = fmaxf(ain, aux_pair(v0, v1, h0, h1, l0, l1));
+            hi[j] = h0; hi[j + 1] = h1; lo[j] = l0; lo[j + 1] = l1;
+        }
+        aux.hi[s] = hi; aux.lo[s] = lo;
+    }
+}
+
+__device__ __forceinline__ void encode_sincos(const float (&x)[3], int multires, int g, float (&sn)[18], float (&cs)[18]) {
+#pragma unroll
+    for (int j = 0; j < 3; ++j)
+#pragma unroll
+        for (int c = 0; c < 3; ++c) {
+            float s = 0.f, k = 0.f;
+            if (2 * j < multires) {
+                sincosf(x[c] * (g ? (float)(2 << (2 * j)) : (float)(1 << (2 * j))), &s, &k);
+                if (2 * j + g >= multires) { s = 0.f; k = 0.f; }
+            }
+            const float so = __shfl_xor(s, 32, 64), ko = __shfl_xor(k, 32, 64);
+            sn[6 * j + c] = g ? so : s;          cs[6 * j + c] = g ? ko : k;
+            sn[6 * j + 3 + c] = g ? s : so;      cs[6 * j + 3 + c] = g ? k : ko;
+        }
+}
+
+__device__ __forceinline__ void dir_operand_row(const float (&d)[3], int g, A16& row) {
+    float sn[18], cs[18];
+    encode_sincos(d, VFN16_DIR_MULTIRES, g, sn, cs);
+    constexpr int ncol = 6 + 6 * VFN16_DIR_MULTIRES;
+    float unused = 0.f;
+    build_aux(row, g, [&](int k) -> float {
+        if (k < 3 || k >= ncol) return 0.f;
+        return enc_value(d, sn, cs, VFN16_DIR_MULTIRES, k - 3);
+    }, unused);
+}
diff --git a/vf_nerf_amd/csrc/vfn_common.h b/vf_nerf_amd/csrc/vfn_common.h
--- a/vf_nerf_amd/csrc/vfn_common.h
+++ b/vf_nerf_amd/csrc/vfn_common.h
@@ -30,7 +30,8 @@
 
 int vfn_internal_raygen(const vfn_raygen_params* p, const float* uv, const float* pose, const float* intrinsics, const float* k_sign,
                         const float* t_vals, const float* far_per_ray, const float* u_coarse, int gen_u, long long u_base, uint64_t seed,
-                        uint64_t offset, float* directions, float* ray_dirs, float* cam_loc, float* z_vals, float* points, void* stream);
+                        uint64_t offset, float* directions, float* ray_dirs, float* cam_loc, float* z_vals, float* points, void* stream,
+                        void* dir_aux = nullptr);
 int vfn_internal_density_fine(const vfn_density_params* dp, const float* normals_c, const float* ray_dirs, const float* z_c,
                               const float* density_scalars, const vfn_fine_params* fp, const float* directions, const float* cam_loc,
                               const float* far_per_ray, const float* u_fine, const float* u_add, int gen_fine, int gen_add,
@@ -69,6 +70,9 @@
 int vfn_internal_fused16_products_dev(const vfn_net_geom* vf_geom, const void* vf_packed16, const vfn_net_geom* rn_geom, const void* rn_packed16,
                                       const float* points, const float* ray_dirs, int64_t n_points, const int32_t* n_dev, int32_t samples_per_ray,
                                       const int32_t* out_index, int32_t colour_products, float* normals, float* colors, void* stream);
+int vfn_internal_fused16_products_table(const vfn_net_geom* vf_geom, const void* vf_packed16, const vfn_net_geom* rn_geom, const void* rn_packed16,
+                                        const float* points, const float* ray_dirs, const void* dir_aux, int64_t n_points, int32_t samples_per_ray,
+                                        const int32_t* out_index, int32_t colour_products, float* normals, float* colors, void* stream);
 uint32_t* vfn_internal_f16x3_status();
 struct VfnReportScope {
     VfnReportScope(uint32_t* status_word, uint64_t* clock_stamps, int64_t clock_slots);
diff --git a/vf_nerf_amd/csrc/vfn_mlp16.hip b/vf_nerf_amd/csrc/vfn_mlp16.hip
--- a/vf_nerf_amd/csrc/vfn_mlp16.hip
+++ b/vf_nerf_amd/csrc/vfn_mlp16.hip
@@ -2,16 +2,14 @@
 #include <utility>
 #include "vfn_common.h"
 #include "vfn_plan.h"
-
-typedef _Float16 half8 __attribute__((ext_vector_type(8)));
-typedef _Float16 half2v __attribute__((ext_vector_type(2)));
-typedef float float2v __attribute__((ext_vector_type(2)));
+#include "vfn_aux16.h"
+
 typedef float f32x16 __attribute__((ext_vector_type(16)));
 typedef float f32x4v __attribute__((ext_vector_type(4)));
+typedef unsigned int u32x4v __attribute__((ext_vector_type(4)));
 
 constexpr float VFN16_WSCALE = 64.0f;
 constexpr float VFN16_INV_WSCALE = 0.015625f;
-constexpr float VFN16_XSCALE = 64.0f;
 constexpr int VFN16_SAVE_AUX = 2;
 constexpr int VFN16_HANDOVER_NUM = 8;
 constexpr int VFN16_DMA_STEPS = 16;
@@ -293,6 +291,8 @@
     const uint4* rn_w;
     const float* points;
     const float* ray_dirs;
+    const uint4* dir_aux;
+    uint32_t dir_bytes;
     float* out_vec;
     float* out_colors;
     long long n_points;
@@ -316,12 +316,10 @@
     long long clock_slots;
 };
 
-#define VFN16_CLAMP 60000.0f
 constexpr int VFN16_CLAMP_BITS = 0x476a6000;
 static_assert(__builtin_bit_cast(int, VFN16_CLAMP) == VFN16_CLAMP_BITS, "VFN16_CLAMP_BITS is VFN16_CLAMP as an integer");
 
 struct X16 { half8 hi[16]; half8 lo[16]; };
-struct A16 { half8 hi[3]; half8 lo[3]; };
 
 struct Pipe16 {
     uint4* lds;
@@ -354,19 +352,6 @@
 __device__ __forceinline__ void static_for_impl(F&& f, std::integer_sequence<int, I...>) { (f(std::integral_constant<int, I>{}), ...); }
 template <int N, typename F>
 __device__ __forceinline__ void static_for(F&& f) { static_for_impl<N>(f, std::make_integer_sequence<int, N>{}); }
-
-__device__ __forceinline__ void split2(float a, float b, _Float16& h0, _Float16& h1, _Float16& l0, _Float16& l1) {
-    const float2v v = {a, b};
-    const half2v hi = __builtin_convertvector(v, half2v);
-    h0 = hi[0]; h1 = hi[1];
-    const uint32_t hp = __builtin_bit_cast(uint32_t, hi);
-    float r0, r1;
-    asm("v_fma_mix_f32 %0, %1, -1.0, %2 op_sel_hi:[1,0,0]" : "=v"(r0) : "v"(hp), "v"(a));
-    asm("v_fma_mix_f32 %0, %1, -1.0, %2 op_sel:[1,0,0] op_sel_hi:[1,0,0]" : "=v"(r1) : "v"(hp), "v"(b));
-    const float2v r = {r0, r1};
-    const half2v lo = __builtin_convertvector(r, half2v);
-    l0 = lo[0]; l1 = lo[1];
-}
 
 __device__ __forceinline__ float tanh_exp(float v) { return 1.0f - 2.0f / (1.0f + expf(2.0f * v)); }
 
@@ -643,34 +628,6 @@
     });
 }
 
-__device__ __forceinline__ float enc_value(const float (&x)[3], const float (&sn)[18], const float (&cs)[18], int multires, int k) {
-    if (k < 3) return x[k];
-    const int idx = k - 3, oct = idx / 6, rem = idx - 6 * oct;
-    if (oct >= multires) return 0.f;
-    return rem < 3 ? sn[3 * oct + rem] : cs[3 * oct + rem - 3];
-}
-
-template <typename F>
-__device__ __forceinline__ void build_aux(A16& aux, int g, F col, float& ain) {
-#pragma unroll
-    for (int s = 0; s < 3; ++s) {
-        half8 hi, lo;
-#pragma unroll
-        for (int j = 0; j < 8; j += 2) {
-            float v0, v1;
-            if (g == 0) { v0 = col(16 * s + j); v1 = col(16 * s + j + 1); }
-            else { v0 = col(16 * s + 8 + j); v1 = col(16 * s + 8 + j + 1); }
-            v0 *= VFN16_XSCALE; v1 *= VFN16_XSCALE;
-            v0 = fminf(fmaxf(v0, -VFN16_CLAMP), VFN16_CLAMP); v1 = fminf(fmaxf(v1, -VFN16_CLAMP), VFN16_CLAMP);
-            ain = fmaxf(ain, fmaxf(fabsf(v0), fabsf(v1)));
-            _Float16 h0, h1, l0, l1;
-            split2(v0, v1, h0, h1, l0, l1);
-            hi[j] = h0; hi[j + 1] = h1; lo[j] = l0; lo[j + 1] = l1;
-        }
-        aux.hi[s] = hi; aux.lo[s] = lo;
-    }
-}
-
 template <typename F>
 __device__ __forceinline__ void save_aux(float* dst, long long m, int g, F col) {
 #pragma unroll
@@ -691,22 +648,6 @@
     const half8* pk = reinterpret_cast<const half8*>(park + 8);
 #pragma unroll
     for (int q = 0; q < 3; ++q) { ax.hi[q] = pk[2 * q]; ax.lo[q] = pk[2 * q + 1]; }
-}
-
-__device__ __forceinline__ void encode_sincos(const float (&x)[3], int multires, int g, float (&sn)[18], float (&cs)[18]) {
-#pragma unroll
-    for (int j = 0; j < 3; ++j)
-#pragma unroll
-        for (int c = 0; c < 3; ++c) {
-            float s = 0.f, k = 0.f;
-            if (2 * j < multires) {
-                sincosf(x[c] * (g ? (float)(2 << (2 * j)) : (float)(1 << (2 * j))), &s, &k);
-                if (2 * j + g >= multires) { s = 0.f; k = 0.f; }
-            }
-            const float so = __shfl_xor(s, 32, 64), ko = __shfl_xor(k, 32, 64);
-            sn[6 * j + c] = g ? so : s;          cs[6 * j + c] = g ? ko : k;
-            sn[6 * j + 3 + c] = g ? s : so;      cs[6 * j + 3 + c] = g ? k : ko;
-        }
 }
 
 template <int MODE>
@@ -822,15 +763,21 @@
     if (in) { x[0] = a.points[m * 3 + 0]; x[1] = a.points[m * 3 + 1]; x[2] = a.points[m * 3 + 2]; }
     float d[3] = {0.f, 0.f, 0.f};
     int out_row = -1;
+    constexpr bool DIR_TABLE = (MODE & M16_RENDER) != 0 && (MODE & M16_TRAIN) == 0;
+    const bool dir_table = DIR_TABLE && a.dir_aux != nullptr;
+    [[maybe_unused]] uint32_t dir_voff = 0;
     if ((MODE & M16_RENDER) && in) {
-        const long long di = m / a.dirs_div;
-        d[0] = a.ray_dirs[di * 3 + 0]; d[1] = a.ray_dirs[di * 3 + 1]; d[2] = a.ray_dirs[di * 3 + 2];
+        if (!dir_table) {
+            const long long di = m / a.dirs_div;
+            d[0] = a.ray_dirs[di * 3 + 0]; d[1] = a.ray_dirs[di * 3 + 1]; d[2] = a.ray_dirs[di * 3 + 2];
+        }
         if (a.out_index) out_row = a.out_index[m];
     }
+    if (dir_table) dir_voff = (uint32_t)m / (uint32_t)a.dirs_div * (uint32_t)VFN16_DIR_ROW_BYTES + (uint32_t)g * (VFN16_DIR_ROW_BYTES / 2);
     asm volatile("s_waitcnt vmcnt(0)" ::: "memory");
     if (MODE & M16_RENDER) {
         s_park[0] = x[0]; s_park[1] = x[1]; s_park[2] = x[2];
-        s_park[4] = d[0]; s_park[5] = d[1]; s_park[6] = d[2];
+        if (!dir_table) { s_park[4] = d[0]; s_park[5] = d[1]; s_park[6] = d[2]; }
     }
 
     Pipe16 p;
@@ -896,6 +843,12 @@
     } else {
     constexpr bool BO = (MODE & M16_BLKOUT) != 0;
     layer16<MODE, 63, 16, 0, 8, T, R, 14, 8, 7, BO, false>(xa, aux, xb, xa, cy, vec, p, wave, lane);
+    [[maybe_unused]] u32x4v dir_q[6];
+    if constexpr (DIR_TABLE) {
+        const __amdgpu_buffer_rsrc_t rs_dir = __builtin_amdgcn_make_buffer_rsrc(const_cast<uint4*>(a.dir_aux), 0, (int)a.dir_bytes, 0x00020000);
+#pragma unroll
+        for (int q = 0; q < 6; ++q) dir_q[q] = __builtin_amdgcn_raw_buffer_load_b128(rs_dir, (int)dir_voff, q * 16, 0);
+    }
     layer16<MODE, 71, 16, 0, 1, EPI_HEAD_TANH, T, 14, -1, 8, false, BO>(xa, aux, xb, xb, cy, vec, p, wave, lane);
     if constexpr (!(MODE & M16_RENDER)) {
         if (in && g == 0) { a.out_vec[m * 3 + 0] = vec[0]; a.out_vec[m * 3 + 1] = vec[1]; a.out_vec[m * 3 + 2] = vec[2]; }
@@ -905,9 +858,25 @@
 #pragma unroll
     for (int c = 0; c < 3; ++c) nrm[c] = __shfl(vec[c], lane & 31, 64);
     const float xr[3] = {s_park[0], s_park[1], s_park[2]};
-    const float dr[3] = {s_park[4], s_park[5], s_park[6]};
     A16 raux;
-    render_aux<MODE>(a, raux, xr, dr, nrm, (MODE & M16_TRAIN) ? mw : m, in, g, ain);
+    if (dir_table) {
+        static_assert(6 + 6 * VFN16_DIR_MULTIRES == 30, "the insert positions below are those of rn_multires == 4");
+#pragma unroll
+        for (int s = 0; s < 3; ++s) { raux.hi[s] = __builtin_bit_cast(half8, dir_q[2 * s]); raux.lo[s] = __builtin_bit_cast(half8, dir_q[2 * s + 1]); }
+        _Float16 h[6], l[6];
+        ain = fmaxf(ain, aux_pair(xr[0], xr[1], h[0], h[1], l[0], l[1]));
+        ain = fmaxf(ain, aux_pair(xr[2], nrm[2], h[2], h[3], l[2], l[3]));
+        ain = fmaxf(ain, aux_pair(nrm[0], nrm[1], h[4], h[5], l[4], l[5]));
+        if (g == 0) {
+            raux.hi[0][0] = h[0]; raux.hi[0][1] = h[1]; raux.hi[0][2] = h[2]; raux.lo[0][0] = l[0]; raux.lo[0][1] = l[1]; raux.lo[0][2] = l[2];
+            raux.hi[2][0] = h[3]; raux.lo[2][0] = l[3];
+        } else {
+            raux.hi[1][6] = h[4]; raux.hi[1][7] = h[5]; raux.lo[1][6] = l[4]; raux.lo[1][7] = l[5];
+        }
+    } else {
+        const float dr[3] = {s_park[4], s_park[5], s_park[6]};
+        render_aux<MODE>(a, raux, xr, dr, nrm, (MODE & M16_TRAIN) ? mw : m, in, g, ain);
+    }
     render_tail<MODE>(a, p, cy, xa, xb, raux, nrm, a.out_index ? (long long)out_row : m, a.out_index ? out_row >= 0 : in, wave, lane);
     report_range(a, cy.sat, ain);
     if constexpr ((MODE & M16_TRAIN) == 0) {
@@ -990,7 +959,7 @@
 static int launch_fused16(const char* what, const vfn_net_geom* vf_geom, const void* vf_packed16, const vfn_net_geom* rn_geom,
                           const void* rn_packed16, const float* points, const float* ray_dirs, int64_t n_points,
                           int32_t samples_per_ray, const int32_t* out_index, bool scatter, int32_t colour_products, float* normals,
-                          float* colors, void* stream, const int32_t* n_dev = nullptr) {
+                          float* colors, void* stream, const int32_t* n_dev = nullptr, const void* dir_aux = nullptr) {
     Mlp16Args a = {};
     a.n_dev = n_dev;
     VfnNetPlan p32; Plan16 vf, rn;
@@ -1011,6 +980,11 @@
     a.vf_w = (const uint4*)vf_packed16; a.rn_w = (const uint4*)rn_packed16; a.points = points; a.ray_dirs = ray_dirs;
     a.out_vec = normals; a.out_colors = colors; a.out_index = out_index; a.n_points = n_points; a.dirs_div = samples_per_ray;
     a.vf_multires = vf.multires; a.rn_multires = rn.multires; a.vf_bytes = vf.total_kb * 1024u; a.rn_bytes = rn.total_kb * 1024u;
+    if (dir_aux && rn.multires == VFN16_DIR_MULTIRES) {
+        VFN_REQUIRE(n_points < (1ll << 22), "%s: a per-ray operand table serves fewer than 2^22 samples", what);
+        a.dir_aux = (const uint4*)dir_aux;
+        a.dir_bytes = (uint32_t)((n_points + samples_per_ray - 1) / samples_per_ray) * (uint32_t)VFN16_DIR_ROW_BYTES;
+    }
     a.status = t_status_word;
     a.clock = t_clock_probe; a.clock_slots = t_clock_slots;
     const long long blocks = (n_points + VFN16_PTS - 1) / VFN16_PTS;
@@ -1048,6 +1022,13 @@
                                       const int32_t* out_index, int32_t colour_products, float* normals, float* colors, void* stream) {
     return launch_fused16("vfn_render_fwd (colour branch on the selected samples)", vf_geom, vf_packed16, rn_geom, rn_packed16, points, ray_dirs,
                           n_points, samples_per_ray, out_index, false, colour_products, normals, colors, stream, n_dev);
+}
+
+int vfn_internal_fused16_products_table(const vfn_net_geom* vf_geom, const void* vf_packed16, const vfn_net_geom* rn_geom, const void* rn_packed16,
+                                        const float* points, const float* ray_dirs, const void* dir_aux, int64_t n_points, int32_t samples_per_ray,
+                                        const int32_t* out_index, int32_t colour_products, float* normals, float* colors, void* stream) {
+    return launch_fused16("vfn_render_fwd (fused launch)", vf_geom, vf_packed16, rn_geom, rn_packed16, points, ray_dirs, n_points, samples_per_ray,
+                          out_index, false, colour_products, normals, colors, stream, nullptr, dir_aux);
 }
 
 extern "C" int vfn_vf_feat16_fwd(const vfn_net_geom* geom, const void* packed16, const float* points, int64_t n_points,
diff --git a/vf_nerf_amd/csrc/vfn_rays.hip b/vf_nerf_amd/csrc/vfn_rays.hip
--- a/vf_nerf_amd/csrc/vfn_rays.hip
+++ b/vf_nerf_amd/csrc/vfn_rays.hip
@@ -1,6 +1,7 @@
 #pragma clang fp contract(off)
 #include <string.h>
 #include "vfn_common.h"
+#include "vfn_aux16.h"
 
 namespace {
 
@@ -60,13 +61,14 @@
     int gen_u;
     long long u_base;
     PhiloxStream ps;
+    uint4* dir_aux;
     const float* k_sign;
 };
 
 __device__ __forceinline__ float coarse_z(float near, float far, float t) { return near * (1.0f - t) + far * t; }
 
 __global__ __launch_bounds__(256) void vfn_raygen_kernel(const RaygenArgs a) {
-    __shared__ float s_ray[K1_RAYS][8];
+    __shared__ float s_ray[K1_RAYS][12];
     const int tid = threadIdx.x;
     const int ray0 = blockIdx.x * K1_RAYS;
     const int n = a.p.n_rays;
@@ -106,14 +108,29 @@
 #pragma unroll
         for (int i = 0; i < 3; ++i) {
             a.directions[(size_t)r * 3 + i] = d[i];
-            a.ray_dirs[(size_t)r * 3 + i] = d[i] / nd;
+            const float dn = d[i] / nd;
+            a.ray_dirs[(size_t)r * 3 + i] = dn;
             a.cam_loc[(size_t)r * 3 + i] = cam[i];
+            s_ray[tid][8 + i] = dn;
             s_ray[tid][i] = d[i];
             s_ray[tid][3 + i] = cam[i];
         }
         s_ray[tid][6] = a.far_per_ray ? a.far_per_ray[r] : a.p.far;
     }
     __syncthreads();
+    if (a.dir_aux && tid < WAVE) {
+        const int lr = tid & 31, g = tid >> 5;
+        const bool live = lr < K1_RAYS && ray0 + lr < n;
+        float dn[3] = {0.f, 0.f, 0.f};
+        if (live) { dn[0] = s_ray[lr][8]; dn[1] = s_ray[lr][9]; dn[2] = s_ray[lr][10]; }
+        A16 row;
+        dir_operand_row(dn, g, row);
+        if (live) {
+            uint4* dst = a.dir_aux + (size_t)(ray0 + lr) * VFN16_DIR_ROW_U4 + g * (VFN16_DIR_ROW_U4 / 2);
+#pragma unroll
+            for (int s = 0; s < 3; ++s) { dst[2 * s] = __builtin_bit_cast(uint4, row.hi[s]); dst[2 * s + 1] = __builtin_bit_cast(uint4, row.lo[s]); }
+        }
+    }
     const int S = a.p.n_samples;
     const int total = K1_RAYS * S;
     for (int idx = tid; idx < total; idx += blockDim.x) {
@@ -900,9 +917,10 @@
 
 int vfn_internal_raygen(const vfn_raygen_params* p, const float* uv, const float* pose, const float* intrinsics, const float* k_sign,
                         const float* t_vals, const float* far_per_ray, const float* u_coarse, int gen_u, long long u_base, uint64_t seed,
-                        uint64_t offset, float* directions, float* ray_dirs, float* cam_loc, float* z_vals, float* points, void* stream) {
+                        uint64_t offset, float* directions, float* ray_dirs, float* cam_loc, float* z_vals, float* points, void* stream,
+                        void* dir_aux) {
     RaygenArgs a{*p, uv, pose, intrinsics, t_vals, far_per_ray, u_coarse, directions, ray_dirs, cam_loc, z_vals, points};
-    a.gen_u = gen_u; a.u_base = u_base; a.ps = PhiloxStream{seed, offset}; a.k_sign = k_sign;
+    a.gen_u = gen_u; a.u_base = u_base; a.ps = PhiloxStream{seed, offset}; a.k_sign = k_sign; a.dir_aux = static_cast<uint4*>(dir_aux);
     const unsigned blocks = (unsigned)((p->n_rays + K1_RAYS - 1) / K1_RAYS);
     hipLaunchKernelGGL(vfn_raygen_kernel, dim3(blocks), dim3(256), 0, (hipStream_t)stream, a);
     return vfn_check_launch("vfn_render_fwd (rays)");
diff --git a/vf_nerf_amd/csrc/vfn_render.hip b/vf_nerf_amd/csrc/vfn_render.hip
--- a/vf_nerf_amd/csrc/vfn_render.hip
+++ b/vf_nerf_amd/csrc/vfn_render.hip
@@ -1,5 +1,6 @@
 #include <string.h>
 #include "vfn_common.h"
+#include "vfn_aux16.h"
 
 namespace {
 
@@ -19,6 +20,7 @@
     int64_t* imax;
     int32_t *cnt, *off, *k_dev, *sel_sorted;
     float *pts_sel, *dirs_sel;
+    unsigned char* dir_aux;
     size_t bytes;
 };
 
@@ -44,6 +46,7 @@
     w.sel_sorted = c.take<int32_t>(cap);
     w.pts_sel = c.take<float>(cap * 3);
     w.dirs_sel = c.take<float>(cap * 3);
+    w.dir_aux = c.take<unsigned char>((p->sparse_colours || p->separate_launches) ? 0 : n * VFN16_DIR_ROW_BYTES);
     w.bytes = c.off;
     return w;
 }
@@ -166,6 +169,7 @@
     auto stage = [&](int which, int ray0, int nh, hipStream_t s) -> int {
         const size_t r = (size_t)ray0;
         float* dirs_h = ray_dirs + r * 3;
+        unsigned char* aux_h = rn_geom->multires == VFN16_DIR_MULTIRES ? w.dir_aux + r * VFN16_DIR_ROW_BYTES : nullptr;
         float* n_c = w.normals_c + r * sc * 3; float* c_c = w.colors_c + r * sc * 3;
         int32_t* dst_h = w.dst + r * st; int32_t* src_h = w.src + r * st;
         vfn_density_params dp = p->density;
@@ -176,11 +180,11 @@
             return vfn_internal_raygen(&rq, uv + r * 2, pose + r * (p->pose_is_quat ? 7 : 16), intrinsics + r * 16, intrinsics, t_vals,
                                        far_coarse_per_ray ? far_coarse_per_ray + r : nullptr,
                                        (p->perturb_coarse && u_coarse) ? u_coarse + r * sc : nullptr, gen_c, (long long)r * sc, p->seed, p->offset,
-                                       w.directions + r * 3, dirs_h, w.cam_loc + r * 3, w.z_c + r * sc, w.pts_c + r * sc * 3, s);
+                                       w.directions + r * 3, dirs_h, w.cam_loc + r * 3, w.z_c + r * sc, w.pts_c + r * sc * 3, s, aux_h);
         }
         case 1:
-            return vfn_vf_render_fused16_products(vf_geom, vf_packed16, rn_geom, rn_packed16, w.pts_c + r * sc * 3, dirs_h, (int64_t)nh * sc, sc, nullptr,
-                                                  products, n_c, c_c, s);
+            return vfn_internal_fused16_products_table(vf_geom, vf_packed16, rn_geom, rn_packed16, w.pts_c + r * sc * 3, dirs_h, aux_h, (int64_t)nh * sc, sc,
+                                                       nullptr, products, n_c, c_c, s);
         case 2: {
             dp.n_samples = sc;
             vfn_fine_params fp = {nh, sc, nf, p->near_fine, p->far_fine, p->fine_range, p->window_step, p->span};
@@ -191,8 +195,8 @@
                                              (int64_t)nh * sc, s);
         }
         case 3:
-            return vfn_vf_render_fused16_products(vf_geom, vf_packed16, rn_geom, rn_packed16, w.new_pts + r * nf * 3, dirs_h, (int64_t)nh * nf, nf,
-                                                  dst_h + (size_t)nh * sc, products, normals + r * st * 3, colors + r * st * 3, s);
+            return vfn_internal_fused16_products_table(vf_geom, vf_packed16, rn_geom, rn_packed16, w.new_pts + r * nf * 3, dirs_h, aux_h, (int64_t)nh * nf,
+                                                       nf, dst_h + (size_t)nh * sc, products, normals + r * st * 3, colors + r * st * 3, s);
         default:
             dp.n_samples = st;
             return vfn_internal_composite_gather(&dp, normals + r * st * 3, dirs_h, z_vals + r * st, density_scalars, colors + r * st * 3, src_h, n_c, c_c,
```

After: 2.038 million (median of 6 runs). No clear change (+0.2%).
